# zju-pi/diff-sampler

Measured on NVIDIA H100. Metric: images/sec at fixed NFE, higher is better.
Workload: dtype fp16 operands, fp32 accumulate (split-precision: fp16 hi x hi + two e4m3 correction MMAs per product); 1 GPU; EDM cifar10 U-Net, heun num_steps=10 (NFE=18), batch 512/GPU; net=cifar10, solver=heun, nfe=18, batch_per_gpu=512, global_batch=512, weights=random init (reference constructors, seed 0), init_zero layers de-zeroed, parallelism=dp1, l2=per-forward activation working set (GBs) >> 50 MB L2

## Files before the change

diff-sampler_b200/_cstructs.py:

```python
import ctypes as C

P = C.c_uint64
I32 = C.c_int32
I64 = C.c_int64
F32 = C.c_float

DS_OP_GEMM, DS_OP_GN_STATS, DS_OP_GN_APPLY, DS_OP_SOFTMAX, DS_OP_POSEMB, DS_OP_LINEAR = 1, 2, 3, 4, 5, 6
DS_OP_PREP_INPUT, DS_OP_CHANMEAN, DS_OP_MEMSET, DS_OP_LAYERNORM, DS_OP_GEGLU, DS_OP_GN_FINALIZE, DS_OP_ATTN, DS_OP_EMBED = 7, 8, 9, 10, 11, 12, 13, 14
DS_OP_OPT_PREP, DS_OP_OPT_SOFTMAX, DS_OP_OPT_REDUCE, DS_OP_OPT_KNN = 15, 16, 17, 18
DS_IO_X, DS_IO_D, DS_IO_SIGMA, DS_IO_LABELS, DS_IO_BOTTLENECK, DS_IO_CTX, DS_IO_COUNT = 0, 1, 2, 3, 4, 5, 6
DS_M_X0, DS_M_EPS, DS_M_DIV, DS_M_NONE = 0, 1, 2, 3
DS_F8_SH_A16, DS_F8_SH_LO8, DS_F8_SH_HI8 = 6, 13, 2
DS_OPT_CAP, DS_OPT_P_SHIFT, DS_OPT_BAND_NATS, DS_OPT_TAU, DS_OPT_EPS = 1024, 15, 40, 0.01, 2.0 ** -17
DS_OPT_PLAIN, DS_OPT_RESCORED, DS_OPT_UNREFINED = 0, 1, 2
DS_KNN_MAX, DS_KNN_CAND = 64, 256

SPACE_ABS, SPACE_ARENA, SPACE_WEIGHTS, SPACE_IO = 0, 1, 2, 3


def ref(space, offset):
    return (space << 60) | int(offset)


class GemmDesc(C.Structure):
    _fields_ = [
        ('a_ptr', P), ('a_dims', I64 * 4), ('a_strides', I64 * 3), ('a_box', I32 * 4), ('a_plane_n', I32),
        ('a2_ptr', P), ('a2_c', I64), ('a2_plane_n', I32), ('nkb_aux', I32),
        ('b_ptr', P), ('b_dims', I64 * 3), ('b_strides', I64 * 2), ('b_plane_batch', I32),
        ('BN', I32), ('m_tiles', I32), ('n_tiles', I32), ('num_z', I32), ('nh', I32),
        ('taps', I32), ('cpb', I32), ('npass', I32), ('a_mode', I32), ('conv_H', I32), ('conv_W', I32),
        ('a_c_per_zh', I32), ('a_n_per_zb', I32), ('a_n_per_zh', I32),
        ('b_k0', I32), ('b_k_per_zh', I32), ('b_row_per_zh', I32), ('b_z_per_zb', I32), ('b_z_per_zh', I32),
        ('m_valid', I32), ('n_valid', I32),
        ('out_f32', P), ('out_h16', P), ('o_zb', I64), ('o_zh', I64), ('ldo', I64), ('o_plane', I64),
        ('bias_n', P), ('bias_m', P), ('rowvec', P), ('rowvec_stride', I64), ('rows_per_sample', I32), ('f8', I32),
        ('residual', P), ('ldr', I64), ('scale', F32),
        ('edm_out', I32), ('edm_x', P), ('edm_coef', P), ('edm_coef_stride', I32), ('edm_C', I32), ('edm_D', P),
        ('st_quads', P),
        ('tap_dh', I32 * 9), ('tap_dw', I32 * 9), ('tap_cb', I32 * 9), ('acc_scale', F32), ('st_unit', I32),
    ]


class GnStatsDesc(C.Structure):
    _fields_ = [('src0', P), ('src1', P), ('C0', I32), ('C1', I32), ('HW', I32), ('B', I32), ('groups', I32), ('pad0', I32),
                ('sums', P)]


class GnApplyDesc(C.Structure):
    _fields_ = [('src0', P), ('src1', P), ('C0', I32), ('C1', I32), ('H', I32), ('W', I32), ('B', I32), ('groups', I32),
                ('sums', P), ('gamma', P), ('beta', P), ('eps', F32), ('silu', I32), ('ada', P), ('ada_stride', I64),
                ('resample', I32), ('nplanes', I32), ('out_act', P), ('out_raw', P), ('out_raw_f32', P), ('fmt', I32), ('pad0', I32), ('coef', P)]


class SoftmaxDesc(C.Structure):
    _fields_ = [('S', P), ('P', P), ('rows', I64), ('L', I32), ('nplanes', I32), ('pitch_in', I32), ('pitch_out', I32)]


class PosembDesc(C.Structure):
    _fields_ = [('sigma', P), ('nsig', I32), ('num_channels', I32), ('endpoint', I32), ('swap_sincos', I32),
                ('sigma_data', F32), ('mode', I32), ('coef', P), ('emb', P), ('noise_scale', F32), ('pad0', I32)]


class LinearDesc(C.Structure):
    _fields_ = [('in_', P), ('in_stride', I64), ('W', P), ('b', P), ('add', P), ('add_stride', I64), ('out', P),
                ('n_rows', I32), ('in_f', I32), ('out_f', I32), ('act', I32), ('in_scale', F32), ('pad0', I32)]


class PrepInputDesc(C.Structure):
    _fields_ = [('x', P), ('coef', P), ('coef_stride', I32), ('B', I32), ('C', I32), ('HW', I32), ('nplanes', I32),
                ('x_batch', I32), ('out', P), ('codebook', P), ('idx', P), ('n_embed', I32), ('pad0', I32)]


class ChanmeanDesc(C.Structure):
    _fields_ = [('src', P), ('out', P), ('rows', I64), ('C', I32), ('pad0', I32)]


class LayernormDesc(C.Structure):
    _fields_ = [('src', P), ('gamma', P), ('beta', P), ('out', P), ('rows', I64), ('C', I32), ('nplanes', I32), ('eps', F32), ('fmt', I32)]


class GegluDesc(C.Structure):
    _fields_ = [('src', P), ('out', P), ('rows', I64), ('I', I32), ('nplanes', I32), ('fmt', I32), ('mode', I32)]


class GnFinalizeDesc(C.Structure):
    _fields_ = [('quads0', P), ('quads1', P), ('C0', I32), ('C1', I32), ('slabs_per_sample', I32), ('B', I32), ('groups', I32),
                ('unit0', I32), ('sums', P), ('gamma', P), ('beta', P), ('ada', P), ('ada_stride', I64), ('eps', F32), ('HW', I32), ('coef', P),
                ('unit1', I32), ('pad1', I32)]


class AttnDesc(C.Structure):
    _fields_ = [('q', P), ('k', P), ('vt', P), ('out', P), ('B', I32), ('nh', I32), ('L', I32), ('Lk', I32),
                ('q_pitch', I32), ('q_c0', I32), ('k_pitch', I32), ('k_c0', I32), ('vt_pitch', I32), ('o_pitch', I32),
                ('nplanes', I32), ('scale', F32), ('causal', I32), ('pad0', I32)]


class EmbedDesc(C.Structure):
    _fields_ = [('ids', P), ('tok', P), ('pos', P), ('out', P), ('rows', I64), ('T', I32), ('C', I32), ('vocab', I32), ('pad0', I32)]


class OptPrepDesc(C.Structure):
    _fields_ = [('x', P), ('planes', P), ('xn2', P), ('B', I32), ('D', I32), ('pitch', I32), ('pad0', I32)]


class OptSoftmaxDesc(C.Structure):
    _fields_ = [('part', P), ('hy2', P), ('xn2', P), ('sigma', P), ('x', P), ('y', P), ('P', P), ('status', P), ('ldp', I64), ('ldP', I64),
                ('B', I32), ('N', I32), ('D', I32), ('nslice', I32), ('nsig', I32), ('ymax', F32)]


class OptReduceDesc(C.Structure):
    _fields_ = [('part', P), ('out', P), ('rows', I64), ('cols', I32), ('ld', I32), ('nsplit', I32), ('scale', F32)]


class OptKnnDesc(C.Structure):
    _fields_ = [('part', P), ('hy2', P), ('xn2', P), ('x', P), ('y', P), ('dist', P), ('idx', P), ('ldp', I64),
                ('B', I32), ('N', I32), ('D', I32), ('nslice', I32), ('k', I32), ('ymax', F32)]


class MemsetDesc(C.Structure):
    _fields_ = [('ptr', P), ('bytes', I64)]


class _OpUnion(C.Union):
    _fields_ = [('gemm', GemmDesc), ('gn_stats', GnStatsDesc), ('gn_apply', GnApplyDesc), ('softmax', SoftmaxDesc),
                ('posemb', PosembDesc), ('linear', LinearDesc), ('prep_input', PrepInputDesc), ('chanmean', ChanmeanDesc),
                ('memset', MemsetDesc), ('layernorm', LayernormDesc), ('geglu', GegluDesc), ('gn_finalize', GnFinalizeDesc), ('attn', AttnDesc),
                ('embed', EmbedDesc), ('opt_prep', OptPrepDesc), ('opt_softmax', OptSoftmaxDesc), ('opt_reduce', OptReduceDesc),
                ('opt_knn', OptKnnDesc)]


class PlanOp(C.Structure):
    _fields_ = [('type', I32), ('tag', I32), ('u', _OpUnion)]


SIZEOF_CHECKS = {
    0: PlanOp, DS_OP_GEMM: GemmDesc, DS_OP_GN_STATS: GnStatsDesc, DS_OP_GN_APPLY: GnApplyDesc, DS_OP_SOFTMAX: SoftmaxDesc,
    DS_OP_POSEMB: PosembDesc, DS_OP_LINEAR: LinearDesc, DS_OP_PREP_INPUT: PrepInputDesc, DS_OP_CHANMEAN: ChanmeanDesc,
    DS_OP_MEMSET: MemsetDesc, DS_OP_LAYERNORM: LayernormDesc, DS_OP_GEGLU: GegluDesc, DS_OP_GN_FINALIZE: GnFinalizeDesc, DS_OP_ATTN: AttnDesc,
    DS_OP_EMBED: EmbedDesc, DS_OP_OPT_PREP: OptPrepDesc, DS_OP_OPT_SOFTMAX: OptSoftmaxDesc, DS_OP_OPT_REDUCE: OptReduceDesc,
    DS_OP_OPT_KNN: OptKnnDesc,
}

UNION_FIELD = {
    DS_OP_GEMM: 'gemm', DS_OP_GN_STATS: 'gn_stats', DS_OP_GN_APPLY: 'gn_apply', DS_OP_SOFTMAX: 'softmax', DS_OP_POSEMB: 'posemb',
    DS_OP_LINEAR: 'linear', DS_OP_PREP_INPUT: 'prep_input', DS_OP_CHANMEAN: 'chanmean', DS_OP_MEMSET: 'memset',
    DS_OP_LAYERNORM: 'layernorm', DS_OP_GEGLU: 'geglu', DS_OP_GN_FINALIZE: 'gn_finalize', DS_OP_ATTN: 'attn', DS_OP_EMBED: 'embed',
}
OPT_UNION_FIELD = {DS_OP_OPT_PREP: 'opt_prep', DS_OP_OPT_SOFTMAX: 'opt_softmax', DS_OP_OPT_REDUCE: 'opt_reduce', DS_OP_OPT_KNN: 'opt_knn'}
ALL_UNION_FIELD = {**UNION_FIELD, **OPT_UNION_FIELD}
OP_TYPE_OF = {GemmDesc: DS_OP_GEMM, GnStatsDesc: DS_OP_GN_STATS, GnApplyDesc: DS_OP_GN_APPLY, SoftmaxDesc: DS_OP_SOFTMAX,
              PosembDesc: DS_OP_POSEMB, LinearDesc: DS_OP_LINEAR, PrepInputDesc: DS_OP_PREP_INPUT, ChanmeanDesc: DS_OP_CHANMEAN,
              MemsetDesc: DS_OP_MEMSET, LayernormDesc: DS_OP_LAYERNORM, GegluDesc: DS_OP_GEGLU, GnFinalizeDesc: DS_OP_GN_FINALIZE, AttnDesc: DS_OP_ATTN,
              EmbedDesc: DS_OP_EMBED, OptPrepDesc: DS_OP_OPT_PREP, OptSoftmaxDesc: DS_OP_OPT_SOFTMAX, OptReduceDesc: DS_OP_OPT_REDUCE,
              OptKnnDesc: DS_OP_OPT_KNN}
```

diff-sampler_b200/_lib.py:

```python
import ctypes as C
import os

import torch

from . import _cstructs as S

_HERE = os.path.dirname(os.path.abspath(__file__))
LIB_PATH = os.path.join(_HERE, 'libdiffsampler_b200.so')

EXPORTS = [
    'ds_version', 'ds_last_error', 'ds_weights_create', 'ds_weights_destroy', 'ds_unet_create', 'ds_unet_destroy',
    'ds_unet_forward', 'ds_unet_debug_read', 'ds_unet_last_launch_count', 'ds_solver_update', 'ds_dyn_threshold',
    'ds_op_launch', 'ds_sizeof', 'ds_unet_set_profiling', 'ds_unet_get_profile', 'ds_unet_op_type', 'ds_gits_cost', 'ds_unet_forward_io', 'ds_images_to_uint8', 'ds_solver_update_u8', 'ds_unet_enable_graph', 'ds_amed_predict',
    'ds_gemm_config', 'ds_op_check',
]

_lib = None


class DsError(RuntimeError):
    pass


def load():
    global _lib
    if _lib is not None:
        return _lib
    if not os.path.exists(LIB_PATH):
        raise DsError(f'{LIB_PATH} not found: build it with `python diff-sampler_b200/build.py` '
                      '(there is no CPU fallback for the CUDA path)')
    lib = C.CDLL(LIB_PATH)
    vp, cp, sz = C.c_void_p, C.c_char_p, C.c_size_t
    lib.ds_version.restype = cp
    lib.ds_last_error.restype = cp
    lib.ds_weights_create.argtypes = [vp, sz, C.POINTER(vp)]
    lib.ds_weights_destroy.argtypes = [vp]
    lib.ds_weights_destroy.restype = None
    lib.ds_unet_create.argtypes = [vp, vp, C.c_int, sz, sz, C.POINTER(vp)]
    lib.ds_unet_destroy.argtypes = [vp]
    lib.ds_unet_destroy.restype = None
    lib.ds_unet_forward.argtypes = [vp, vp, vp, vp, vp, vp, vp]
    lib.ds_unet_forward_io.argtypes = [vp, C.POINTER(vp), C.c_int, vp]
    lib.ds_unet_enable_graph.argtypes = [vp, C.POINTER(sz), C.c_int]
    lib.ds_unet_debug_read.argtypes = [vp, sz, vp, sz, vp]
    lib.ds_unet_last_launch_count.argtypes = [vp]
    lib.ds_unet_set_profiling.argtypes = [vp, C.c_int]
    lib.ds_unet_get_profile.argtypes = [vp, C.POINTER(C.c_float), C.c_int]
    lib.ds_unet_op_type.argtypes = [vp, C.c_int]
    lib.ds_solver_update.argtypes = [vp, vp, vp, vp, vp, C.POINTER(vp), C.c_int, vp, C.c_int, C.c_float, vp,
                                     C.POINTER(C.c_float), vp, C.c_int64, C.c_int, vp]
    lib.ds_solver_update_u8.argtypes = [vp, vp, vp, C.c_int, C.c_int, vp, vp, vp, C.POINTER(vp), C.c_int, vp, C.c_int, C.c_float, vp,
                                        C.POINTER(C.c_float), vp, C.c_int64, C.c_int, vp]
    lib.ds_amed_predict.argtypes = [vp, C.POINTER(C.c_int), vp, vp, vp, C.c_float, C.c_float, vp, C.c_int, vp]
    lib.ds_dyn_threshold.argtypes = [vp, vp, C.c_int, C.c_int, C.c_float, C.c_float, vp]
    lib.ds_gits_cost.argtypes = [vp, vp, vp, vp, C.c_int, C.c_int, C.c_int64, vp]
    lib.ds_images_to_uint8.argtypes = [vp, vp, C.c_int, C.c_int, C.c_int, vp]
    lib.ds_op_launch.argtypes = [C.c_int, vp, sz, vp]
    lib.ds_op_check.argtypes = [C.c_int, vp, sz]
    lib.ds_sizeof.argtypes = [C.c_int]
    lib.ds_sizeof.restype = sz
    lib.ds_gemm_config.argtypes = [vp, C.POINTER(C.c_int)]
    for which, cls in S.SIZEOF_CHECKS.items():
        got, want = C.sizeof(cls), lib.ds_sizeof(which)
        if got != want:
            raise DsError(f'struct mirror {cls.__name__}: ctypes size {got} != library size {want}')
    _lib = lib
    return lib


def check(rc, what=''):
    if rc != 0:
        msg = load().ds_last_error().decode()
        raise DsError(f'{what} failed (rc={rc}): {msg}')


def version():
    return load().ds_version().decode()


def op_launch(desc, stream=0):
    lib = load()
    check(lib.ds_op_launch(S.OP_TYPE_OF[type(desc)], C.byref(desc), C.sizeof(desc), C.c_void_p(stream)), type(desc).__name__)


def op_check(desc):
    lib = load()
    if lib.ds_op_check(S.OP_TYPE_OF[type(desc)], C.byref(desc), C.sizeof(desc)) == 0:
        return None
    return lib.ds_last_error().decode()


def gemm_config(desc):
    info = (C.c_int * 2)()
    check(load().ds_gemm_config(C.byref(desc), info), 'ds_gemm_config')
    return dict(stages=info[0], grid=info[1])


class NativePlans:

    def __init__(self, blob, device):
        self.lib = load()
        self.device = device
        self.plans = {}
        self._wh = C.c_void_p()
        with torch.cuda.device(device):
            check(self.lib.ds_weights_create(blob, len(blob), C.byref(self._wh)), 'ds_weights_create')

    def get(self, key, compile_fn, io_bytes=None):
        ent = self.plans.get(key)
        if ent is None:
            pl = compile_fn()
            h = C.c_void_p()
            with torch.cuda.device(self.device):
                check(self.lib.ds_unet_create(self._wh, C.cast(pl.ops_array, C.c_void_p), pl.n_ops, C.sizeof(S.PlanOp), pl.arena_bytes,
                                              C.byref(h)), 'ds_unet_create')
                if io_bytes is not None:
                    check(self.lib.ds_unet_enable_graph(h, (C.c_size_t * S.DS_IO_COUNT)(*io_bytes(pl)), S.DS_IO_COUNT),
                          'ds_unet_enable_graph')
            ent = self.plans[key] = (h, pl)
        return ent

    def run(self, h, io, stream):
        check(self.lib.ds_unet_forward_io(h, (C.c_void_p * S.DS_IO_COUNT)(*io), S.DS_IO_COUNT, C.c_void_p(stream)), 'ds_unet_forward_io')
        return self.lib.ds_unet_last_launch_count(h)

    def debug_read(self, key, name, numel, dtype=torch.float32):
        h, pl = self.plans[key]
        t = torch.empty(numel, dtype=dtype)
        stream = torch.cuda.current_stream(self.device).cuda_stream
        check(self.lib.ds_unet_debug_read(h, pl.arena_offsets[name], t.data_ptr(), t.numel() * t.element_size(), C.c_void_p(stream)),
              'ds_unet_debug_read')
        return t

    def __del__(self):
        try:
            for h, _ in self.plans.values():
                self.lib.ds_unet_destroy(h)
            self.lib.ds_weights_destroy(self._wh)
        except Exception:
            pass
```

diff-sampler_b200/csrc/elementwise.cu:

```cuda
#include "ops.h"
#include "operand.cuh"
#include <cuda_fp16.h>
#include <math.h>

namespace dsb {

__device__ __forceinline__ float silu_f(float v) { return __fdividef(v, 1.0f + __expf(-v)); }

__global__ void gn_stats_kernel(ds_gn_stats_desc d, int pix_per_cta) {
    __shared__ double s_sum[64];
    __shared__ double s_sq[64];
    const int tid = threadIdx.y * blockDim.x + threadIdx.x;
    if (tid < 64) { s_sum[tid] = 0.0; s_sq[tid] = 0.0; }
    __syncthreads();
    const int C = d.C0 + d.C1;
    const int cpg = C / d.groups;
    const int n = blockIdx.y;
    const int ncol4 = C / 4;
    const int p_begin = blockIdx.x * pix_per_cta;
    int p_end = p_begin + pix_per_cta;
    if (p_end > d.HW) p_end = d.HW;
    for (int col = threadIdx.x; col < ncol4; col += blockDim.x) {
        const int c = col * 4;
        const float* base;
        int pitch, cc;
        if (c < d.C0) { base = d.src0; pitch = d.C0; cc = c; }
        else { base = d.src1; pitch = d.C1; cc = c - d.C0; }
        const int gA = c / cpg;
        const int gB = (c + 3) / cpg;
        const int nA = (gA == gB) ? 4 : ((gA + 1) * cpg - c);
        float sA = 0.f, qA = 0.f, sB = 0.f, qB = 0.f;
#pragma unroll 8
        for (int p = p_begin + threadIdx.y; p < p_end; p += blockDim.y) {
            const float4 v = __ldcs(reinterpret_cast<const float4*>(base + ((long long)n * d.HW + p) * pitch + cc));
            const float e[4] = {v.x, v.y, v.z, v.w};
#pragma unroll
            for (int j = 0; j < 4; ++j) {
                if (j < nA) { sA += e[j]; qA += e[j] * e[j]; }
                else { sB += e[j]; qB += e[j] * e[j]; }
            }
        }
        atomicAdd(&s_sum[gA], (double)sA);
        atomicAdd(&s_sq[gA], (double)qA);
        if (gB != gA) {
            atomicAdd(&s_sum[gB], (double)sB);
            atomicAdd(&s_sq[gB], (double)qB);
        }
    }
    __syncthreads();
    if (tid < d.groups) {
        atomicAdd(&d.sums[((long long)n * d.groups + tid) * 2 + 0], s_sum[tid]);
        atomicAdd(&d.sums[((long long)n * d.groups + tid) * 2 + 1], s_sq[tid]);
    }
}

template <class D>
__device__ __forceinline__ float2 gn_group_stats(const D& d, int n, int g, double cnt) {
    const double s = d.sums[((long long)n * d.groups + g) * 2 + 0];
    const double q = d.sums[((long long)n * d.groups + g) * 2 + 1];
    const double mu = s / cnt;
    double var = q / cnt - mu * mu;
    if (var < 0.0) var = 0.0;
    const float rstd = (float)(1.0 / sqrt(var + (double)d.eps));
    return make_float2((float)mu, rstd);
}

template <class D>
__device__ __forceinline__ void gn_channel_coef(const D& d, int n, int C, int c, int j, float rstd, float& a, float& b) {
    float aa = rstd * __ldg(d.gamma + c + j);
    float bb = __ldg(d.beta + c + j);
    if (d.ada) {
        const float sc = d.ada[(long long)n * d.ada_stride + c + j] + 1.0f;
        const float sh = d.ada[(long long)n * d.ada_stride + C + c + j];
        aa *= sc;
        bb = bb * sc + sh;
    }
    a = aa;
    b = bb;
}

__global__ void __launch_bounds__(1024) gn_finalize_kernel(ds_gn_finalize_desc d) {
    extern __shared__ double s_cols[];
    __shared__ float s_mu[64], s_rstd[64];
    const int n = blockIdx.x;
    const int C = d.C0 + d.C1;
    if (d.quads0) {
        const int u0 = d.unit0 == 2 ? 2 : 4, u1 = d.unit1 == 2 ? 2 : 4;
        const int w0 = d.C0 / u0 * 2, w1 = d.C1 / u1 * 2;
        const int cols = w0 + w1;
        int SG = blockDim.x / cols;
        if (SG < 1) SG = 1;
        if (SG > d.slabs_per_sample) SG = d.slabs_per_sample;
        double* part = s_cols + cols;
        for (int idx = threadIdx.x; idx < cols * SG; idx += blockDim.x) {
            const int t = idx % cols, sg = idx / cols;
            const float* src = (t < w0) ? d.quads0 + (long long)n * d.slabs_per_sample * w0 + t
                                        : d.quads1 + (long long)n * d.slabs_per_sample * w1 + (t - w0);
            const int pitch = (t < w0) ? w0 : w1;
            double acc = 0.0;
#pragma unroll 4
            for (int sl = sg; sl < d.slabs_per_sample; sl += SG) acc += (double)__ldg(src + (long long)sl * pitch);
            part[(long long)sg * cols + t] = acc;
        }
        __syncthreads();
        for (int t = threadIdx.x; t < cols; t += blockDim.x) {
            double acc = 0.0;
            for (int sg = 0; sg < SG; ++sg) acc += part[(long long)sg * cols + t];
            s_cols[t] = acc;
        }
        __syncthreads();
        const int cpg = C / d.groups;
        for (int j = threadIdx.x; j < 2 * d.groups; j += blockDim.x) {
            const int g = j >> 1, k = j & 1;
            double acc = 0.0;
            int c = g * cpg;
            const int c_end = c + cpg;
            while (c < c_end) {
                if (c < d.C0) { acc += s_cols[(c / u0) * 2 + k]; c += u0; }
                else { acc += s_cols[w0 + ((c - d.C0) / u1) * 2 + k]; c += u1; }
            }
            d.sums[((long long)n * d.groups + g) * 2 + k] = acc;
        }
        __syncthreads();
    }
    if (!d.coef) return;
    const double cnt = (double)(C / d.groups) * d.HW;
    for (int g = threadIdx.x; g < d.groups; g += blockDim.x) {
        const float2 st = gn_group_stats(d, n, g, cnt);
        s_mu[g] = st.x;
        s_rstd[g] = st.y;
    }
    __syncthreads();
    const int cpg = C / d.groups;
    for (int c = threadIdx.x; c < C; c += blockDim.x) {
        const int g = c / cpg;
        float aa, bb;
        gn_channel_coef(d, n, C, c, 0, s_rstd[g], aa, bb);
        reinterpret_cast<float2*>(d.coef)[(long long)n * C + c] = make_float2(aa, fmaf(-s_mu[g], aa, bb));
    }
}

template <int RESAMPLE>
__global__ void __launch_bounds__(512) gn_apply_kernel(ds_gn_apply_desc d, int pix_per_cta, int nc8, int rows) {
    const int C = d.C0 + d.C1;
    const int n = blockIdx.y;
    const int c8 = threadIdx.x % nc8;
    const int prow = threadIdx.x / nc8;
    const int c = c8 * 8;
    const bool norm = d.sums != nullptr;
    float mean[8], a[8], b[8];
    if (norm) {
        const int cpg = C / d.groups;
// ... 487 lines not shown
    for (int o = 16; o > 0; o >>= 1) sum += __shfl_xor_sync(0xffffffffu, sum, o);
    const float mean = sum / (float)d.C;
    float sq = 0.f;
#pragma unroll
    for (int k = 0; k < MAXV; ++k) {
        const int j = lane + 32 * k;
        if (j < nv) {
            const float a = v[k].x - mean, b = v[k].y - mean, c = v[k].z - mean, e = v[k].w - mean;
            sq += a * a + b * b + c * c + e * e;
        }
    }
#pragma unroll
    for (int o = 16; o > 0; o >>= 1) sq += __shfl_xor_sync(0xffffffffu, sq, o);
    const float rstd = rsqrtf(sq / (float)d.C + d.eps);
#pragma unroll
    for (int k = 0; k < MAXV; ++k) {
        const int j = lane + 32 * k;
        if (j < nv) {
            const float4 g = *reinterpret_cast<const float4*>(d.gamma + 4 * j);
            const float4 b = *reinterpret_cast<const float4*>(d.beta + 4 * j);
            const float y[4] = {(v[k].x - mean) * rstd * g.x + b.x, (v[k].y - mean) * rstd * g.y + b.y,
                                (v[k].z - mean) * rstd * g.z + b.z, (v[k].w - mean) * rstd * g.w + b.w};
            if (FMT == 2) *reinterpret_cast<float4*>(reinterpret_cast<float*>(d.out) + row * d.C + 4 * j) = make_float4(y[0], y[1], y[2], y[3]);
            else store_operand<4>(reinterpret_cast<__half*>(d.out), d.rows * d.C, row * d.C + 4 * j, y, d.nplanes, FMT);
        }
    }
}

__global__ void embed_kernel(ds_embed_desc d) {
    const long long idx = (long long)blockIdx.x * blockDim.x + threadIdx.x;
    const int c4 = d.C / 4;
    if (idx >= d.rows * c4) return;
    const long long row = idx / c4;
    const int j = (int)(idx - row * c4) * 4;
    int id = d.ids[row];
    id = id < 0 ? 0 : (id >= d.vocab ? d.vocab - 1 : id);
    const float4 t = *reinterpret_cast<const float4*>(d.tok + (long long)id * d.C + j);
    const float4 p = *reinterpret_cast<const float4*>(d.pos + (long long)(row % d.T) * d.C + j);
    *reinterpret_cast<float4*>(d.out + row * d.C + j) = make_float4(t.x + p.x, t.y + p.y, t.z + p.z, t.w + p.w);
}

template <int MODE, int FMT>
__global__ void gate_kernel(ds_geglu_desc d) {
    const long long idx = (long long)blockIdx.x * blockDim.x + threadIdx.x;
    const int i4 = d.I / 4;
    if (idx >= d.rows * i4) return;
    float y[4];
    if (MODE == 0) {
        const long long row = idx / i4;
        const int j = (int)(idx - row * i4) * 4;
        const float4 a = *reinterpret_cast<const float4*>(d.src + row * 2 * d.I + j);
        const float4 g = *reinterpret_cast<const float4*>(d.src + row * 2 * d.I + d.I + j);
        const float av[4] = {a.x, a.y, a.z, a.w}, gv[4] = {g.x, g.y, g.z, g.w};
#pragma unroll
        for (int q = 0; q < 4; ++q) y[q] = av[q] * (0.5f * gv[q] * (1.0f + erff(gv[q] * 0.70710678118654752f)));
    } else {
        const float4 a = *reinterpret_cast<const float4*>(d.src + idx * 4);
        const float av[4] = {a.x, a.y, a.z, a.w};
#pragma unroll
        for (int q = 0; q < 4; ++q) y[q] = av[q] / (1.0f + expf(-1.702f * av[q]));
    }
    store_operand<4>(reinterpret_cast<__half*>(d.out), d.rows * d.I, idx * 4, y, d.nplanes, FMT);
}

__global__ void chanmean_kernel(ds_chanmean_desc d) {
    const long long row = (long long)blockIdx.x * (blockDim.x >> 5) + (threadIdx.x >> 5);
    if (row >= d.rows) return;
    const int lane = threadIdx.x & 31;
    float s = 0.f;
    for (int c = lane; c < d.C; c += 32) s += d.src[row * d.C + c];
#pragma unroll
    for (int o = 16; o > 0; o >>= 1) s += __shfl_xor_sync(0xffffffffu, s, o);
    if (lane == 0) d.out[row] = s / (float)d.C;
}

static inline int ok() { return cudaGetLastError() == cudaSuccess ? 0 : -1; }

}

using namespace dsb;

OpCheck dsb::gn_stats_check(const ds_gn_stats_desc& d) {
    const int C = d.C0 + d.C1;
    if (C % 4 || d.groups <= 0 || d.groups > 64 || C % d.groups || (d.C0 % 4)) return {-2, "gn_stats: channels"};
    if (C / d.groups < 2) return {-2, "gn_stats: one-channel groups"};
    return {0, nullptr};
}

extern "C" int ds_gn_stats_launch(const ds_gn_stats_desc* d, cudaStream_t stream) {
    if (const int rc = gn_stats_check(*d).rc) return rc;
    const int C = d->C0 + d->C1;
    const int ncol4 = C / 4;
    int bx = ncol4 < 256 ? ncol4 : 256;
    int by = 256 / bx; if (by < 1) by = 1;
    int pix_per_cta = 8 * by;
    if (pix_per_cta < 64) pix_per_cta = 64;
    const int min_pix = by > 8 ? by : 8;
    while (pix_per_cta > min_pix && (long long)((d->HW + pix_per_cta - 1) / pix_per_cta) * d->B < 132 * 4) pix_per_cta /= 2;
    const int chunks = (d->HW + pix_per_cta - 1) / pix_per_cta;
    gn_stats_kernel<<<dim3(chunks, d->B), dim3(bx, by), 0, stream>>>(*d, pix_per_cta);
    return ok();
}

static size_t gn_finalize_shape(const ds_gn_finalize_desc& d, int* threads) {
    *threads = 256;
    if (!d.quads0) return (size_t)(d.C0 + d.C1 + 2) * sizeof(double);
    const int u0 = d.unit0 == 2 ? 2 : 4, u1 = d.unit1 == 2 ? 2 : 4;
    const int cols = d.C0 / u0 * 2 + d.C1 / u1 * 2;
    *threads = 1024;
    const int sg = cols >= *threads ? 1 : *threads / cols;
    return (size_t)(cols + (size_t)sg * cols + 2) * sizeof(double);
}

OpCheck dsb::gn_finalize_check(const ds_gn_finalize_desc& d) {
    const int C = d.C0 + d.C1;
    if (d.groups <= 0 || d.groups > 64 || C % d.groups) return {-2, "gn_finalize: groups"};
    if (d.quads0) {
        const int u0 = d.unit0 == 2 ? 2 : 4, u1 = d.unit1 == 2 ? 2 : 4;
        const int cpg = C / d.groups;
        if (d.C0 % u0 || d.C1 % u1 || (d.C1 > 0 && !d.quads1)) return {-2, "gn_finalize: source units"};
        const int rem = d.C0 % cpg;
        if (cpg % u0 || rem % u0) return {-2, "gn_finalize: group units"};
        if (d.C1 > 0 && (cpg % u1 || (rem ? (cpg - rem) % u1 : 0))) return {-2, "gn_finalize: group units"};
    }
    if (!d.quads0 && !d.coef) return {-2, "gn_finalize: nothing to do"};
    if (d.coef && (!d.gamma || !d.beta || d.HW <= 0)) return {-2, "gn_finalize: coef inputs"};
    int threads;
    if (gn_finalize_shape(d, &threads) > 48 * 1024) return {-2, "gn_finalize: shared memory"};
    return {0, nullptr};
}

extern "C" int ds_gn_finalize_launch(const ds_gn_finalize_desc* d, cudaStream_t stream) {
    if (const int rc = gn_finalize_check(*d).rc) return rc;
    int threads;
    const size_t smem = gn_finalize_shape(*d, &threads);
    gn_finalize_kernel<<<d->B, threads, smem, stream>>>(*d);
    return ok();
}

OpCheck dsb::gn_apply_check(const ds_gn_apply_desc& d) {
    const int C = d.C0 + d.C1;
    if (C % 8 || (d.C0 % 8)) return {-2, "gn_apply: channels"};
    if (d.fmt != 0 && (d.fmt != 1 || d.resample == 3 || d.nplanes != 2)) return {-2, "gn_apply: fmt"};
    if (d.coef && d.resample != 0) return {-2, "gn_apply: coef with resample"};
    if (d.out_act && !d.sums && !d.coef) return {-2, "gn_apply: statistics"};
    if ((d.resample == 1 || d.resample == 3) && (d.H % 2 || d.W % 2)) return {-2, "gn_apply: resample parity"};
    if (d.pad0 && (d.resample != 3 || d.pad0 < C || d.pad0 % 8 || d.out_raw_f32)) return {-2, "gn_apply: phase pitch"};
    const int nc8 = C / 8;
    if (nc8 > 512) return {-2, "gn_apply: width"};
    if (d.coef && d.resample == 0 && d.sums == nullptr && nc8 > 256) return {-2, "gn_apply: coef width"};
    return {0, nullptr};
}

extern "C" int ds_gn_apply_launch(const ds_gn_apply_desc* d, cudaStream_t stream) {
    if (const int rc = gn_apply_check(*d).rc) return rc;
    const int C = d->C0 + d->C1;
    const int nc8 = C / 8;
    int rows = 256 / nc8;
    if (rows < 1) rows = 1;
    const int threads = nc8 * rows;
    const int Ho = d->resample == 1 ? d->H / 2 : (d->resample == 2 ? d->H * 2 : d->H);
    const int Wo = d->resample == 1 ? d->W / 2 : (d->resample == 2 ? d->W * 2 : d->W);
    const int npix = Ho * Wo;
    int pix_per_cta = rows * 16;
    while (pix_per_cta > rows && (long long)((npix + pix_per_cta - 1) / pix_per_cta) * d->B < 132 * 4) pix_per_cta /= 2;
    const int chunks = (npix + pix_per_cta - 1) / pix_per_cta;
    dim3 grid(chunks, d->B);
    if (d->coef && d->resample == 0 && d->sums == nullptr) {
        static int occ[64][17] = {};
        static int sms[64] = {};
        int dev = 0;
        cudaGetDevice(&dev);
        if (dev < 0 || dev >= 64) dev = 0;
        const int slot = threads / 32;
        if (!sms[dev]) cudaDeviceGetAttribute(&sms[dev], cudaDevAttrMultiProcessorCount, dev);
        if (!occ[dev][slot]) {
            int nb = 0;
            if (cudaOccupancyMaxActiveBlocksPerMultiprocessor(&nb, gn_apply_v3_kernel, threads, 0) != cudaSuccess || nb < 1) nb = 1;
            occ[dev][slot] = nb;
        }
        const int ups = (npix + rows - 1) / rows;
        const long long total_units = (long long)ups * d->B;
        long long g3 = (long long)sms[dev] * occ[dev][slot];
        const long long total_chunks = (long long)((ups + 7) / 8) * d->B;
        if (g3 > total_chunks) g3 = total_chunks;
        if (g3 < 1) g3 = 1;
        gn_apply_v3_kernel<<<(unsigned)g3, threads, 0, stream>>>(*d, nc8, rows, ups, total_units);
        return ok();
    }
    if (d->resample == 1) gn_apply_kernel<1><<<grid, threads, 0, stream>>>(*d, pix_per_cta, nc8, rows);
    else if (d->resample == 3 && d->pad0 && d->pad0 != C) gn_apply_kernel<4><<<grid, threads, 0, stream>>>(*d, pix_per_cta, nc8, rows);
    else if (d->resample == 3) gn_apply_kernel<3><<<grid, threads, 0, stream>>>(*d, pix_per_cta, nc8, rows);
    else if (d->resample == 2) gn_apply_kernel<2><<<grid, threads, 0, stream>>>(*d, pix_per_cta, nc8, rows);
    else gn_apply_v2_kernel<<<grid, threads, 0, stream>>>(*d, pix_per_cta, nc8, rows);
    return ok();
}

OpCheck dsb::embed_check(const ds_embed_desc& d) {
    if (d.C % 4 || d.rows <= 0 || d.T <= 0 || d.vocab <= 0) return {-2, "embed: shape"};
    return {0, nullptr};
}

extern "C" int ds_embed_launch(const ds_embed_desc* d, cudaStream_t stream) {
    if (const int rc = embed_check(*d).rc) return rc;
    const long long total = d->rows * (d->C / 4);
    embed_kernel<<<(unsigned)((total + 255) / 256), 256, 0, stream>>>(*d);
    return ok();
}

OpCheck dsb::layernorm_check(const ds_layernorm_desc& d) {
    if (d.C % 4 || d.C > 2048) return {-2, "layernorm: C"};
    if (d.fmt == 1 && d.nplanes != 2) return {-2, "layernorm: f8 planes"};
    return {0, nullptr};
}

extern "C" int ds_layernorm_launch(const ds_layernorm_desc* d, cudaStream_t stream) {
    if (const int rc = layernorm_check(*d).rc) return rc;
    const int wpb = 8;
    const unsigned blocks = (unsigned)((d->rows + wpb - 1) / wpb);
    if (d->fmt == 1) {
        layernorm_kernel<1><<<blocks, wpb * 32, 0, stream>>>(*d);
    } else if (d->fmt == 2) {
        layernorm_kernel<2><<<blocks, wpb * 32, 0, stream>>>(*d);
    } else {
        layernorm_kernel<0><<<blocks, wpb * 32, 0, stream>>>(*d);
    }
    return ok();
}

OpCheck dsb::geglu_check(const ds_geglu_desc& d) {
    if (d.I % 4) return {-2, "geglu: I"};
    if (d.mode == 1 && d.fmt != 0) return {-2, "geglu: quick-GELU fmt"};
    if (d.mode != 1 && d.fmt == 1 && d.nplanes != 2) return {-2, "geglu: f8 planes"};
    return {0, nullptr};
}

extern "C" int ds_geglu_launch(const ds_geglu_desc* d, cudaStream_t stream) {
    if (const int rc = geglu_check(*d).rc) return rc;
    const unsigned blocks = (unsigned)((d->rows * (d->I / 4) + 255) / 256);
    if (d->mode == 1) {
        gate_kernel<1, 0><<<blocks, 256, 0, stream>>>(*d);
    } else if (d->fmt == 1) {
        gate_kernel<0, 1><<<blocks, 256, 0, stream>>>(*d);
    } else {
        gate_kernel<0, 0><<<blocks, 256, 0, stream>>>(*d);
    }
    return ok();
}

extern "C" int ds_softmax_launch(const ds_softmax_desc* d, cudaStream_t stream) {
    const bool dense = (d->pitch_in == 0 || d->pitch_in == d->L) && (d->pitch_out == 0 || d->pitch_out == d->L) && (d->L % 4 == 0);
    if (dense && d->L <= 1024) {
        const unsigned blocks = (unsigned)((d->rows + 7) / 8);
        if (d->L <= 256) softmax_reg_kernel<2, false><<<blocks, 256, 0, stream>>>(*d);
        else softmax_reg_kernel<8, false><<<blocks, 256, 0, stream>>>(*d);
        return ok();
    }
    if (dense && d->L <= 8192) {
        if (d->L <= 4096) softmax_reg_kernel<4, true><<<(unsigned)d->rows, 256, 0, stream>>>(*d);
        else softmax_reg_kernel<8, true><<<(unsigned)d->rows, 256, 0, stream>>>(*d);
        return ok();
    }
    const int wpb = 8;
    const long long blocks = (d->rows + wpb - 1) / wpb;
    softmax_kernel<<<(unsigned)blocks, wpb * 32, 0, stream>>>(*d);
    return ok();
}

extern "C" int ds_posemb_launch(const ds_posemb_desc* d, cudaStream_t stream) {
    posemb_kernel<<<d->nsig, 128, 0, stream>>>(*d);
    return ok();
}

OpCheck dsb::linear_check(const ds_linear_desc& d) {
    if (d.in_f > 2048) return {-2, "linear: in_f"};
    return {0, nullptr};
}

extern "C" int ds_linear_launch(const ds_linear_desc* d, cudaStream_t stream) {
    if (const int rc = linear_check(*d).rc) return rc;
    const int wpb = 4;
    const int bx = (d->out_f + wpb - 1) / wpb;
    int by = d->n_rows < 16 ? d->n_rows : 16;
    if (by < 1) by = 1;
    if (d->in_f <= 256) linear_kernel<256><<<dim3(bx, by), wpb * 32, 0, stream>>>(*d);
    else if (d->in_f <= 512) linear_kernel<512><<<dim3(bx, by), wpb * 32, 0, stream>>>(*d);
    else if (d->in_f <= 1024) linear_kernel<1024><<<dim3(bx, by), wpb * 32, 0, stream>>>(*d);
    else linear_kernel<2048><<<dim3(bx, by), wpb * 32, 0, stream>>>(*d);
    return ok();
}

OpCheck dsb::prep_input_check(const ds_prep_input_desc& d) {
    if (d.C > 64) return {-2, "prep_input: C"};
    if (d.codebook && (d.C > 8 || d.n_embed < 1)) return {-2, "prep_input: codebook"};
    return {0, nullptr};
}

extern "C" int ds_prep_input_launch(const ds_prep_input_desc* d, cudaStream_t stream) {
    if (const int rc = prep_input_check(*d).rc) return rc;
    if (d->codebook) {
        const unsigned blocks = (unsigned)(((long long)d->B * d->HW + 255) / 256);
        if (d->C <= 4) vq_prep_input_kernel<4><<<blocks, 256, 0, stream>>>(*d);
        else vq_prep_input_kernel<8><<<blocks, 256, 0, stream>>>(*d);
        return ok();
    }
    const long long total = (long long)d->B * d->HW * 8;
    prep_input_kernel<<<(unsigned)((total + 255) / 256), 256, 0, stream>>>(*d);
    return ok();
}

extern "C" int ds_chanmean_launch(const ds_chanmean_desc* d, cudaStream_t stream) {
    const int wpb = 8;
    chanmean_kernel<<<(unsigned)((d->rows + wpb - 1) / wpb), wpb * 32, 0, stream>>>(*d);
    return ok();
}
```

diff-sampler_b200/csrc/engine.cu:

```cuda
#include "../../include/diffsampler_b200.h"
#include "ops.h"
#include "ptx.cuh"
#include <cuda_fp16.h>
#include <nvtx3/nvToolsExt.h>
#include <stdio.h>
#include <stdlib.h>
#include <string.h>
#include <string>
#include <vector>

namespace dsb {
struct GemmKernelParams;
int gemm_build(const ds_gemm_desc* d, GemmKernelParams* kp);
int gemm_run(const GemmKernelParams* kp, cudaStream_t stream);
size_t gemm_params_size();
void gemm_patch_edm(GemmKernelParams* kp, const float* x, float* D);
struct AttnKernelParams;
int attn_build(const ds_attn_desc* d, AttnKernelParams* kp);
int attn_run(const AttnKernelParams* kp, cudaStream_t stream);
size_t attn_params_size();
}

static thread_local std::string g_err;

struct NvtxRange {
    explicit NvtxRange(const char* name) { nvtxRangePushA(name); }
    ~NvtxRange() { nvtxRangePop(); }
};
static int fail(int code, const std::string& msg) {
    g_err = msg;
    return code;
}

struct ds_weights {
    void* dev = nullptr;
    size_t bytes = 0;
};

struct IoFix {
    int op;
    size_t field_off;
    int slot;
};

struct ds_unet {
    const ds_weights* w = nullptr;
    void* arena = nullptr;
    size_t arena_bytes = 0;
    std::vector<ds_plan_op> ops;
    std::vector<std::vector<unsigned char>> gemm_params;
    std::vector<IoFix> fixes;
    int last_launches = 0;
    bool profiling = false;
    std::vector<cudaEvent_t> ev0, ev1;
    std::vector<char> ev_used;
    bool graph_on = false;
    void* stage[DS_IO_COUNT] = {nullptr, nullptr, nullptr, nullptr, nullptr, nullptr};
    size_t stage_bytes[DS_IO_COUNT] = {0, 0, 0, 0, 0, 0};
    cudaGraphExec_t gexec[2] = {nullptr, nullptr};
    int gnodes[2] = {0, 0};
    int warm_runs = 0;
    cudaStream_t cap_stream = nullptr;
};

template <class F>
static void visit_ptrs(ds_plan_op& op, F f) {
#define P(field) f((void**)(void*)(&(field)))
    switch (op.type) {
        case DS_OP_GEMM: {
            ds_gemm_desc& g = op.u.gemm;
            P(g.a_ptr); P(g.a2_ptr); P(g.b_ptr); P(g.out_f32); P(g.out_h16); P(g.bias_n); P(g.bias_m); P(g.rowvec);
            P(g.residual); P(g.edm_x); P(g.edm_coef); P(g.edm_D); P(g.st_quads);
            break;
        }
        case DS_OP_GN_STATS: { auto& d = op.u.gn_stats; P(d.src0); P(d.src1); P(d.sums); break; }
        case DS_OP_GN_APPLY: {
            auto& d = op.u.gn_apply;
            P(d.src0); P(d.src1); P(d.sums); P(d.gamma); P(d.beta); P(d.ada); P(d.out_act); P(d.out_raw); P(d.out_raw_f32); P(d.coef);
            break;
        }
        case DS_OP_SOFTMAX: { auto& d = op.u.softmax; P(d.S); P(d.P); break; }
        case DS_OP_POSEMB: { auto& d = op.u.posemb; P(d.sigma); P(d.coef); P(d.emb); break; }
        case DS_OP_LINEAR: { auto& d = op.u.linear; P(d.in); P(d.W); P(d.b); P(d.add); P(d.out); break; }
        case DS_OP_PREP_INPUT: { auto& d = op.u.prep_input; P(d.x); P(d.coef); P(d.out); P(d.codebook); P(d.idx); break; }
        case DS_OP_CHANMEAN: { auto& d = op.u.chanmean; P(d.src); P(d.out); break; }
        case DS_OP_MEMSET: { auto& d = op.u.memset; P(d.ptr); break; }
        case DS_OP_LAYERNORM: { auto& d = op.u.layernorm; P(d.src); P(d.gamma); P(d.beta); P(d.out); break; }
        case DS_OP_GEGLU: { auto& d = op.u.geglu; P(d.src); P(d.out); break; }
        case DS_OP_GN_FINALIZE: { auto& d = op.u.gn_finalize; P(d.quads0); P(d.quads1); P(d.sums); P(d.gamma); P(d.beta); P(d.ada); P(d.coef); break; }
        case DS_OP_ATTN: { auto& d = op.u.attn; P(d.q); P(d.k); P(d.vt); P(d.out); break; }
        case DS_OP_EMBED: { auto& d = op.u.embed; P(d.ids); P(d.tok); P(d.pos); P(d.out); break; }
        case DS_OP_OPT_PREP: { auto& d = op.u.opt_prep; P(d.x); P(d.planes); P(d.xn2); break; }
        case DS_OP_OPT_SOFTMAX: { auto& d = op.u.opt_softmax; P(d.part); P(d.hy2); P(d.xn2); P(d.sigma); P(d.x); P(d.y); P(d.P); P(d.status); break; }
        case DS_OP_OPT_REDUCE: { auto& d = op.u.opt_reduce; P(d.part); P(d.out); break; }
        case DS_OP_OPT_KNN: { auto& d = op.u.opt_knn; P(d.part); P(d.hy2); P(d.xn2); P(d.x); P(d.y); P(d.dist); P(d.idx); break; }
        default: break;
    }
#undef P
}

static dsb::OpCheck check_op(const ds_plan_op& op) {
    switch (op.type) {
        case DS_OP_GEMM: return dsb::gemm_check(op.u.gemm);
        case DS_OP_GN_STATS: return dsb::gn_stats_check(op.u.gn_stats);
        case DS_OP_GN_APPLY: return dsb::gn_apply_check(op.u.gn_apply);
        case DS_OP_LINEAR: return dsb::linear_check(op.u.linear);
        case DS_OP_PREP_INPUT: return dsb::prep_input_check(op.u.prep_input);
        case DS_OP_LAYERNORM: return dsb::layernorm_check(op.u.layernorm);
        case DS_OP_GEGLU: return dsb::geglu_check(op.u.geglu);
        case DS_OP_GN_FINALIZE: return dsb::gn_finalize_check(op.u.gn_finalize);
        case DS_OP_ATTN: return dsb::attn_check(op.u.attn);
        case DS_OP_EMBED: return dsb::embed_check(op.u.embed);
        case DS_OP_OPT_PREP: return dsb::opt_prep_check(op.u.opt_prep);
        case DS_OP_OPT_SOFTMAX: return dsb::opt_softmax_check(op.u.opt_softmax);
        case DS_OP_OPT_REDUCE: return dsb::opt_reduce_check(op.u.opt_reduce);
        case DS_OP_OPT_KNN: return dsb::opt_knn_check(op.u.opt_knn);
        case DS_OP_SOFTMAX: case DS_OP_POSEMB: case DS_OP_CHANMEAN: case DS_OP_MEMSET: return {0, nullptr};
        default: return {-100, "unknown op type"};
    }
}

static int launch_op(const ds_plan_op& op, const unsigned char* gemm_kp, cudaStream_t s) {
    switch (op.type) {
        case DS_OP_GEMM:
            if (gemm_kp) return dsb::gemm_run(reinterpret_cast<const dsb::GemmKernelParams*>(gemm_kp), s);
            return ds_gemm_launch(&op.u.gemm, s);
        case DS_OP_GN_STATS: return ds_gn_stats_launch(&op.u.gn_stats, s);
        case DS_OP_GN_APPLY: return ds_gn_apply_launch(&op.u.gn_apply, s);
        case DS_OP_SOFTMAX: return ds_softmax_launch(&op.u.softmax, s);
        case DS_OP_POSEMB: return ds_posemb_launch(&op.u.posemb, s);
        case DS_OP_LINEAR: return ds_linear_launch(&op.u.linear, s);
        case DS_OP_PREP_INPUT: return ds_prep_input_launch(&op.u.prep_input, s);
        case DS_OP_CHANMEAN: return ds_chanmean_launch(&op.u.chanmean, s);
        case DS_OP_LAYERNORM: return ds_layernorm_launch(&op.u.layernorm, s);
        case DS_OP_GEGLU: return ds_geglu_launch(&op.u.geglu, s);
        case DS_OP_GN_FINALIZE: return ds_gn_finalize_launch(&op.u.gn_finalize, s);
        case DS_OP_EMBED: return ds_embed_launch(&op.u.embed, s);
        case DS_OP_OPT_PREP: return ds_opt_prep_launch(&op.u.opt_prep, s);
        case DS_OP_OPT_SOFTMAX: return ds_opt_softmax_launch(&op.u.opt_softmax, s);
        case DS_OP_OPT_REDUCE: return ds_opt_reduce_launch(&op.u.opt_reduce, s);
        case DS_OP_OPT_KNN: return ds_opt_knn_launch(&op.u.opt_knn, s);
        case DS_OP_ATTN:
            if (gemm_kp) return dsb::attn_run(reinterpret_cast<const dsb::AttnKernelParams*>(gemm_kp), s);
            return ds_attn_launch(&op.u.attn, s);
        case DS_OP_MEMSET:
            return cudaMemsetAsync(op.u.memset.ptr, 0, (size_t)op.u.memset.bytes, s) == cudaSuccess ? 0 : -1;
        default: return -100;
    }
}

extern "C" {

const char* ds_version(void) { return "diffsampler_b200 0.1 (sm_90a, wgmma/TMA)"; }
const char* ds_last_error(void) { return g_err.c_str(); }

int ds_weights_create(const void* host_blob, size_t bytes, ds_weights** out) {
    if (!host_blob || !out) return fail(-1, "ds_weights_create: null argument");
    ds_weights* w = new ds_weights();
    if (cudaMalloc(&w->dev, bytes ? bytes : 16) != cudaSuccess) {
        delete w;
        return fail(-2, std::string("ds_weights_create: cudaMalloc failed: ") + cudaGetErrorString(cudaGetLastError()));
    }
    if (cudaMemcpy(w->dev, host_blob, bytes, cudaMemcpyHostToDevice) != cudaSuccess) {
        cudaFree(w->dev);
        delete w;
        return fail(-3, "ds_weights_create: cudaMemcpy failed");
    }
    w->bytes = bytes;
    *out = w;
    return 0;
}

void ds_weights_destroy(ds_weights* w) {
    if (!w) return;
    cudaFree(w->dev);
    delete w;
}

int ds_unet_create(const ds_weights* w, const void* plan_ops, int n_ops, size_t op_size, size_t arena_bytes, ds_unet** out) {
    if (!w || !plan_ops || !out) return fail(-1, "ds_unet_create: null argument");
    if (op_size != sizeof(ds_plan_op)) {
        char buf[128];
        snprintf(buf, sizeof buf, "ds_unet_create: ds_plan_op size mismatch (caller %zu, library %zu)", op_size, sizeof(ds_plan_op));
        return fail(-4, buf);
    }
    for (int i = 0; i < n_ops; ++i) {
        const ds_plan_op& op = reinterpret_cast<const ds_plan_op*>(plan_ops)[i];
        const dsb::OpCheck c = check_op(op);
        if (c.rc) {
            char buf[160];
            snprintf(buf, sizeof buf, "ds_unet_create: op %d (type %d tag %d) refused (rc %d): %s", i, op.type, op.tag, c.rc, c.rule);
            return fail(-6, buf);
        }
    }
    ds_unet* u = new ds_unet();
    u->w = w;
    u->arena_bytes = arena_bytes;
    if (cudaMalloc(&u->arena, arena_bytes ? arena_bytes : 16) != cudaSuccess) {
        delete u;
        return fail(-2, std::string("ds_unet_create: cudaMalloc(arena) failed: ") + cudaGetErrorString(cudaGetLastError()));
    }
    cudaMemset(u->arena, 0, arena_bytes);
    u->ops.assign(reinterpret_cast<const ds_plan_op*>(plan_ops), reinterpret_cast<const ds_plan_op*>(plan_ops) + n_ops);
    u->gemm_params.resize(n_ops);
    int bad = 0;
    for (int i = 0; i < n_ops; ++i) {
        ds_plan_op& op = u->ops[i];
        visit_ptrs(op, [&](void** field) {
            const uint64_t ref = reinterpret_cast<uint64_t>(*field);
            const uint64_t space = ref >> 60;
            const uint64_t off = ref & ((1ull << 60) - 1);
            if (space == 0) return;
            if (space == 1) {
                if (off >= arena_bytes) bad = i + 1;
                *field = static_cast<char*>(u->arena) + off;
            } else if (space == 2) {
                if (off >= w->bytes) bad = i + 1;
                *field = static_cast<char*>(w->dev) + off;
            } else if (space == 3) {
                IoFix fx;
                fx.op = i;
                fx.field_off = reinterpret_cast<char*>(field) - reinterpret_cast<char*>(&op);
                fx.slot = (int)off;
                u->fixes.push_back(fx);
                *field = nullptr;
            } else {
                bad = i + 1;
            }
        });
    }
    if (bad) {
        char buf[96];
        snprintf(buf, sizeof buf, "ds_unet_create: bad pointer reference in op %d", bad - 1);
        ds_unet_destroy(u);
        return fail(-5, buf);
    }
    for (int i = 0; i < n_ops; ++i) {
        const int type = u->ops[i].type;
        if (type != DS_OP_GEMM && type != DS_OP_ATTN) continue;
        u->gemm_params[i].resize((type == DS_OP_GEMM ? dsb::gemm_params_size() : dsb::attn_params_size()) + 64);
        unsigned char* p = u->gemm_params[i].data();
        unsigned char* al = reinterpret_cast<unsigned char*>((reinterpret_cast<uintptr_t>(p) + 63) & ~uintptr_t(63));
        int rc = type == DS_OP_GEMM ? dsb::gemm_build(&u->ops[i].u.gemm, reinterpret_cast<dsb::GemmKernelParams*>(al))
                                    : dsb::attn_build(&u->ops[i].u.attn, reinterpret_cast<dsb::AttnKernelParams*>(al));
        if (rc) {
            char buf[96];
            snprintf(buf, sizeof buf, "ds_unet_create: %s failed (rc %d) for op %d tag %d", type == DS_OP_GEMM ? "gemm_build" : "attn_build", rc, i,
                     u->ops[i].tag);
            ds_unet_destroy(u);
            return fail(-6, buf);
        }
    }
    *out = u;
    return 0;
}

void ds_unet_destroy(ds_unet* u) {
    if (!u) return;
    for (auto e : u->ev0) cudaEventDestroy(e);
    for (auto e : u->ev1) cudaEventDestroy(e);
    for (int v = 0; v < 2; ++v) if (u->gexec[v]) cudaGraphExecDestroy(u->gexec[v]);
    for (int k = 0; k < DS_IO_COUNT; ++k) if (u->stage[k]) cudaFree(u->stage[k]);
    if (u->cap_stream) cudaStreamDestroy(u->cap_stream);
    cudaFree(u->arena);
    delete u;
}

int ds_unet_forward_io(ds_unet* u, const void* const* io_in, int n_io, void* stream);

int ds_unet_forward(ds_unet* u, const float* x, const float* sigma, const float* labels, float* out_D, float* out_bottleneck,
                    void* stream) {
    const void* io[DS_IO_COUNT] = {x, out_D, sigma, labels, out_bottleneck, nullptr};
    return ds_unet_forward_io(u, io, DS_IO_COUNT, stream);
}

static int run_ops(ds_unet* u, const void* const* io, cudaStream_t s, bool profiling) {
    for (const IoFix& fx : u->fixes) {
        if (fx.slot < 0 || fx.slot >= DS_IO_COUNT) return fail(-7, "ds_unet_forward: bad io slot");
        void** field = reinterpret_cast<void**>(reinterpret_cast<char*>(&u->ops[fx.op]) + fx.field_off);
        *field = const_cast<void*>(io[fx.slot]);
    }
    int launches = 0;
    for (size_t i = 0; i < u->ops.size(); ++i) {
        ds_plan_op& op = u->ops[i];
        const unsigned char* kp = nullptr;
        if (op.type == DS_OP_GEMM || op.type == DS_OP_ATTN) {
            unsigned char* p = u->gemm_params[i].data();
            unsigned char* al = reinterpret_cast<unsigned char*>((reinterpret_cast<uintptr_t>(p) + 63) & ~uintptr_t(63));
            if (op.type == DS_OP_GEMM && op.u.gemm.edm_out)
                dsb::gemm_patch_edm(reinterpret_cast<dsb::GemmKernelParams*>(al), op.u.gemm.edm_x, op.u.gemm.edm_D);
            kp = al;
        }
        if (op.type == DS_OP_CHANMEAN && op.u.chanmean.out == nullptr) continue;
        if (profiling) { cudaEventRecord(u->ev0[i], s); u->ev_used[i] = 1; }
        int rc = launch_op(op, kp, s);
        if (profiling) cudaEventRecord(u->ev1[i], s);
        if (rc) {
            char buf[160];
            snprintf(buf, sizeof buf, "ds_unet_forward: op %zu (type %d tag %d) failed rc=%d cuda=%s", i, op.type, op.tag, rc,
                     cudaGetErrorString(cudaGetLastError()));
            return fail(-8, buf);
        }
        ++launches;
    }
    return launches;
}

static int build_graph(ds_unet* u, int variant, const void* const* staged_io) {
    if (!u->cap_stream && cudaStreamCreateWithFlags(&u->cap_stream, cudaStreamNonBlocking) != cudaSuccess)
        return fail(-20, "ds_unet_forward: cannot create the capture stream");
    if (cudaStreamBeginCapture(u->cap_stream, cudaStreamCaptureModeThreadLocal) != cudaSuccess)
        return fail(-21, std::string("ds_unet_forward: cudaStreamBeginCapture failed: ") + cudaGetErrorString(cudaGetLastError()));
    const int n = run_ops(u, staged_io, u->cap_stream, false);
    cudaGraph_t g = nullptr;
    const cudaError_t e = cudaStreamEndCapture(u->cap_stream, &g);
    if (n < 0 || e != cudaSuccess || !g) {
        if (g) cudaGraphDestroy(g);
        if (n < 0) return n;
        return fail(-22, std::string("ds_unet_forward: stream capture failed: ") + cudaGetErrorString(e));
    }
    cudaGraphExec_t ex = nullptr;
    const cudaError_t ei = cudaGraphInstantiate(&ex, g, 0);
    cudaGraphDestroy(g);
    if (ei != cudaSuccess) return fail(-23, std::string("ds_unet_forward: cudaGraphInstantiate failed: ") + cudaGetErrorString(ei));
    u->gexec[variant] = ex;
    u->gnodes[variant] = n;
    return 0;
}

int ds_unet_forward_io(ds_unet* u, const void* const* io_in, int n_io, void* stream) {
    if (!u) return fail(-1, "ds_unet_forward: null handle");
    NvtxRange nvtx_range("ds_unet_forward");
    cudaStream_t s = static_cast<cudaStream_t>(stream);
    const void* io[DS_IO_COUNT] = {nullptr, nullptr, nullptr, nullptr, nullptr, nullptr};
    for (int k = 0; k < n_io && k < DS_IO_COUNT; ++k) io[k] = io_in[k];
    if (!u->graph_on || u->profiling) {
        const int n = run_ops(u, io, s, u->profiling);
        if (n < 0) return n;
        u->last_launches = n;
        return 0;
    }
    static const bool is_input[DS_IO_COUNT] = {true, false, true, true, false, true};
    const void* staged[DS_IO_COUNT];
    for (int k = 0; k < DS_IO_COUNT; ++k) {
        staged[k] = (io[k] && u->stage[k]) ? u->stage[k] : nullptr;
        if (io[k] && !u->stage[k]) return fail(-24, "ds_unet_forward: io slot used without a staging buffer (ds_unet_enable_graph sizes)");
        if (io[k] && is_input[k] &&
            cudaMemcpyAsync(u->stage[k], io[k], u->stage_bytes[k], cudaMemcpyDeviceToDevice, s) != cudaSuccess)
            return fail(-25, "ds_unet_forward: staging copy failed");
    }
    const int variant = io[DS_IO_BOTTLENECK] ? 1 : 0;
    int launches = 0;
    if (!u->gexec[variant]) {
        if (u->warm_runs < 1) {
            launches = run_ops(u, staged, s, false);
            if (launches < 0) return launches;
            ++u->warm_runs;
        } else {
            const int rc = build_graph(u, variant, staged);
            if (rc) return rc;
        }
    }
    if (u->gexec[variant]) {
        if (cudaGraphLaunch(u->gexec[variant], s) != cudaSuccess)
            return fail(-26, std::string("ds_unet_forward: cudaGraphLaunch failed: ") + cudaGetErrorString(cudaGetLastError()));
        launches = u->gnodes[variant];
    }
    for (int k = 0; k < DS_IO_COUNT; ++k)
        if (io[k] && !is_input[k] &&
            cudaMemcpyAsync(const_cast<void*>(io[k]), u->stage[k], u->stage_bytes[k], cudaMemcpyDeviceToDevice, s) != cudaSuccess)
            return fail(-25, "ds_unet_forward: staging copy failed");
    u->last_launches = launches;
    return 0;
}

int ds_unet_enable_graph(ds_unet* u, const size_t* io_bytes, int n_io) {
    if (!u || !io_bytes) return fail(-1, "ds_unet_enable_graph: null argument");
    if (u->graph_on) return 0;
    for (int k = 0; k < n_io && k < DS_IO_COUNT; ++k) {
        if (!io_bytes[k]) continue;
        if (cudaMalloc(&u->stage[k], io_bytes[k]) != cudaSuccess)
            return fail(-2, std::string("ds_unet_enable_graph: cudaMalloc failed: ") + cudaGetErrorString(cudaGetLastError()));
        u->stage_bytes[k] = io_bytes[k];
    }
    u->graph_on = true;
    return 0;
}

int ds_unet_debug_read(ds_unet* u, size_t arena_offset, void* host_dst, size_t bytes, void* stream) {
    if (!u || arena_offset + bytes > u->arena_bytes) return fail(-1, "ds_unet_debug_read: out of range");
    cudaStream_t s = static_cast<cudaStream_t>(stream);
    if (cudaStreamSynchronize(s) != cudaSuccess) return fail(-2, std::string("ds_unet_debug_read: ") + cudaGetErrorString(cudaGetLastError()));
    if (cudaMemcpy(host_dst, static_cast<char*>(u->arena) + arena_offset, bytes, cudaMemcpyDeviceToHost) != cudaSuccess)
        return fail(-3, "ds_unet_debug_read: memcpy failed");
    return 0;
}

int ds_unet_last_launch_count(const ds_unet* u) { return u ? u->last_launches : 0; }

int ds_unet_set_profiling(ds_unet* u, int enable) {
    if (!u) return fail(-1, "ds_unet_set_profiling: null handle");
    if (enable && u->ev0.empty()) {
        u->ev0.resize(u->ops.size());
        u->ev1.resize(u->ops.size());
        u->ev_used.assign(u->ops.size(), 0);
        for (size_t i = 0; i < u->ops.size(); ++i) {
            cudaEventCreate(&u->ev0[i]);
            cudaEventCreate(&u->ev1[i]);
        }
    }
    u->profiling = enable != 0;
    return 0;
}

int ds_unet_get_profile(ds_unet* u, float* ms_per_op, int n) {
    if (!u || u->ev0.empty()) return fail(-1, "ds_unet_get_profile: profiling was not enabled");
    if (cudaDeviceSynchronize() != cudaSuccess) return fail(-2, "ds_unet_get_profile: sync failed");
    for (int i = 0; i < n && i < (int)u->ops.size(); ++i) {
        float ms = 0.f;
        if (u->ev_used[i]) cudaEventElapsedTime(&ms, u->ev0[i], u->ev1[i]);
        ms_per_op[i] = ms;
    }
    return (int)u->ops.size();
}

int ds_unet_op_type(const ds_unet* u, int i) { return (u && i >= 0 && i < (int)u->ops.size()) ? u->ops[i].type : -1; }

static int solver_update_impl(float* out_x, float* out_m, unsigned char* out_u8, int u8_C, int u8_HW, const float* xb, const float* xs,
                              const float* D, const float* const* hist, int nhist, const float* thr, int mode, float t, const float* t_dev,
                              const float* coef6, const float* coef_dev, int64_t n_per_sample, int B, void* stream) {
    if (!xb || nhist < 0 || nhist > 4) return fail(-1, "ds_solver_update: bad argument");
    NvtxRange nvtx_range("ds_solver_update");
    ds_update_desc d;
    memset(&d, 0, sizeof d);
    d.out_x = out_x; d.out_m = out_m; d.xb = xb; d.xs = xs; d.D = D;
    for (int k = 0; k < nhist; ++k) d.h[k] = hist[k];
    d.thr = thr; d.coef_dev = coef_dev; d.t_dev = t_dev;
    if (coef6) for (int k = 0; k < 6; ++k) d.coef[k] = coef6[k];
    d.t = t; d.mode = mode; d.nhist = nhist; d.B = B; d.n_per_sample = n_per_sample;
    d.out_u8 = out_u8; d.u8_C = u8_C; d.u8_HW = u8_HW;
    if ((mode == DS_M_X0 || mode == DS_M_EPS) && !D) return fail(-1, "ds_solver_update: mode needs D");
    int rc = ds_update_launch(&d, static_cast<cudaStream_t>(stream));
    if (rc) return fail(rc, std::string("ds_solver_update: launch failed: ") + cudaGetErrorString(cudaGetLastError()));
    return 0;
}

int ds_solver_update(float* out_x, float* out_m, const float* xb, const float* xs, const float* D, const float* const* hist, int nhist,
                     const float* thr, int mode, float t, const float* t_dev, const float* coef6, const float* coef_dev,
                     int64_t n_per_sample, int B, void* stream) {
    return solver_update_impl(out_x, out_m, nullptr, 0, 0, xb, xs, D, hist, nhist, thr, mode, t, t_dev, coef6, coef_dev, n_per_sample, B, stream);
}

int ds_solver_update_u8(float* out_x, float* out_m, unsigned char* out_u8, int C, int HW, const float* xb, const float* xs, const float* D,
                        const float* const* hist, int nhist, const float* thr, int mode, float t, const float* t_dev, const float* coef6,
                        const float* coef_dev, int64_t n_per_sample, int B, void* stream) {
    if (!out_u8 || C <= 0 || HW <= 0) return fail(-1, "ds_solver_update_u8: bad image geometry");
    return solver_update_impl(out_x, out_m, out_u8, C, HW, xb, xs, D, hist, nhist, thr, mode, t, t_dev, coef6, coef_dev, n_per_sample, B, stream);
}

int ds_dyn_threshold(const float* x0, float* thr, int B, int row_len, float q, float floor_val, void* stream) {
    ds_threshold_desc d;
    d.x0 = x0; d.thr = thr; d.B = B; d.row_len = row_len; d.q = q; d.floor_val = floor_val;
    int rc = ds_threshold_launch(&d, static_cast<cudaStream_t>(stream));
    if (rc) return fail(rc, std::string("ds_dyn_threshold: launch failed: ") + cudaGetErrorString(cudaGetLastError()));
    return 0;
}

size_t ds_sizeof(int which) {
    switch (which) {
        case 0: return sizeof(ds_plan_op);
        case DS_OP_GEMM: return sizeof(ds_gemm_desc);
        case DS_OP_GN_STATS: return sizeof(ds_gn_stats_desc);
        case DS_OP_GN_APPLY: return sizeof(ds_gn_apply_desc);
        case DS_OP_SOFTMAX: return sizeof(ds_softmax_desc);
        case DS_OP_POSEMB: return sizeof(ds_posemb_desc);
        case DS_OP_LINEAR: return sizeof(ds_linear_desc);
        case DS_OP_PREP_INPUT: return sizeof(ds_prep_input_desc);
        case DS_OP_CHANMEAN: return sizeof(ds_chanmean_desc);
        case DS_OP_MEMSET: return sizeof(ds_memset_desc);
        case DS_OP_LAYERNORM: return sizeof(ds_layernorm_desc);
        case DS_OP_GEGLU: return sizeof(ds_geglu_desc);
        case DS_OP_GN_FINALIZE: return sizeof(ds_gn_finalize_desc);
        case DS_OP_ATTN: return sizeof(ds_attn_desc);
        case DS_OP_EMBED: return sizeof(ds_embed_desc);
        case DS_OP_OPT_PREP: return sizeof(ds_opt_prep_desc);
        case DS_OP_OPT_SOFTMAX: return sizeof(ds_opt_softmax_desc);
        case DS_OP_OPT_REDUCE: return sizeof(ds_opt_reduce_desc);
        case DS_OP_OPT_KNN: return sizeof(ds_opt_knn_desc);
        default: return 0;
    }
}

int ds_gits_cost(const float* traj, const float* eps, const float* t_steps, double* out, int N, int B, int64_t n_per_sample, void* stream) {
    ds_gits_cost_desc d;
    d.traj = traj; d.eps = eps; d.t = t_steps; d.out = out; d.N = N; d.B = B; d.n = n_per_sample;
    int rc = ds_gits_cost_launch(&d, static_cast<cudaStream_t>(stream));
    if (rc) return fail(rc, std::string("ds_gits_cost: launch failed: ") + cudaGetErrorString(cudaGetLastError()));
    return 0;
}

int ds_amed_predict(const float* weights, const int* dims6, const float* bottleneck, const float* t_cur, const float* t_next,
                    float scale_dir, float scale_time, float* out4, int B, void* stream) {
    if (!weights || !dims6 || !t_cur || !t_next || !out4) return fail(-1, "ds_amed_predict: null argument");
    NvtxRange nvtx_range("ds_amed_predict");
    int rc = ds_amed_predict_launch(weights, dims6, bottleneck, t_cur, t_next, scale_dir, scale_time, out4, B, static_cast<cudaStream_t>(stream));
    if (rc) return fail(rc, std::string("ds_amed_predict: launch failed: ") + cudaGetErrorString(cudaGetLastError()));
    return 0;
}

int ds_images_to_uint8(const float* images, unsigned char* out, int B, int C, int HW, void* stream) {
    if (!images || !out) return fail(-1, "ds_images_to_uint8: null argument");
    int rc = ds_to_uint8_launch(images, out, B, C, HW, static_cast<cudaStream_t>(stream));
    if (rc) return fail(rc, std::string("ds_images_to_uint8: launch failed: ") + cudaGetErrorString(cudaGetLastError()));
    return 0;
}

int ds_op_launch(int op_type, const void* desc, size_t desc_size, void* stream) {
    ds_plan_op op;
    memset(&op, 0, sizeof op);
    op.type = op_type;
    if (desc_size > sizeof(op.u)) return fail(-1, "ds_op_launch: descriptor too large");
    memcpy(&op.u, desc, desc_size);
    int rc = launch_op(op, nullptr, static_cast<cudaStream_t>(stream));
    if (rc) {
        char buf[128];
        snprintf(buf, sizeof buf, "ds_op_launch: op type %d failed rc=%d cuda=%s", op_type, rc, cudaGetErrorString(cudaGetLastError()));
        return fail(rc, buf);
    }
    return 0;
}

int ds_op_check(int op_type, const void* desc, size_t desc_size) {
    ds_plan_op op;
    memset(&op, 0, sizeof op);
    op.type = op_type;
    if (desc_size > sizeof(op.u)) return fail(-1, "ds_op_check: descriptor too large");
    memcpy(&op.u, desc, desc_size);
    const dsb::OpCheck c = check_op(op);
// ... 5 lines not shown
```

diff-sampler_b200/csrc/gemm_tc.cu:

```cuda
#include "ops.h"
#include "ptx.cuh"
#include <cuda_fp16.h>
#include <stdio.h>
#include <stdlib.h>
#include <string.h>

namespace dsb {

static constexpr int kMaxStages = 8;
static constexpr int kATileBytes = 128 * 128;
static constexpr int kThreads = 384;
static constexpr int kStgPitch = 64;
static constexpr int kStgBytes = 2 * 64 * kStgPitch * 4;
static constexpr int kSmemLimit = 227 * 1024;

struct alignas(64) GemmKernelParams {
    CUtensorMap tmA, tmA2, tmB;
    CUtensorMap tmA8, tmA2_8, tmB8;
    int f8, cpb8, nkb8_main, nkb8_aux, a8_plane_n;
    float acc_scale;
    int BN, m_tiles, n_tiles, num_z, nh;
    int taps, cpb, nkb_main, nkb_aux, npass;
    int a_mode, conv_H, conv_W, a_bn_dummy;
    int a_plane_n, a2_plane_n, b_plane_batch;
    int a_c_per_zh, a_n_per_zb, a_n_per_zh;
    int b_k0, b_k_per_zh, b_row_per_zh, b_z_per_zb, b_z_per_zh;
    int m_valid, n_valid;
    int num_stages;
    float* out_f32;
    __half* out_h16;
    long long o_zb, o_zh, ldo, o_plane;
    const float* bias_n;
    const float* bias_m;
    const float* rowvec;
    long long rowvec_stride;
    int rows_per_sample;
    const float* residual;
    long long ldr;
    float scale;
    int edm_out;
    const float* edm_x;
    const float* edm_coef;
    int edm_coef_stride;
    int edm_C;
    float* edm_D;
    float* st_quads;
    int st_unit;
    int tap_dh[9], tap_dw[9], tap_cb[9];
    int f8_last_steps;
};

struct SmemCtl {
    uint64_t full[kMaxStages];
    uint64_t empty[kMaxStages];
};

template <int N>
__device__ __forceinline__ void warp_sum_levels(float* v, int lane, int off) {
    if constexpr (N >= 1) {
        const bool up = (lane & off) != 0;
#pragma unroll
        for (int i = 0; i < N; ++i) {
            const float send = up ? v[i] : v[i + N];
            const float keep = up ? v[i + N] : v[i];
            v[i] = keep + __shfl_xor_sync(0xffffffffu, send, off);
        }
        warp_sum_levels<N / 2>(v, lane, off >> 1);
    } else {
        for (; off >= 1; off >>= 1) v[0] += __shfl_xor_sync(0xffffffffu, v[0], off);
    }
}
template <int NV>
__device__ __forceinline__ void warp_sum_multi(float (&v)[NV], int lane) {
    static_assert(NV == 32 || NV == 16 || NV == 8, "NV");
    warp_sum_levels<NV / 2>(v, lane, 16);
}

template <int W>
__device__ __forceinline__ void epilogue_chunk(const GemmKernelParams& p, const float* v, long long grow_in_z, int col0, bool row_ok,
                                               int zb, int zh) {
    const bool warp_rows_ok = __all_sync(0xffffffffu, row_ok);
    if (!row_ok) return;
    float r[W];
#pragma unroll
    for (int j = 0; j < W; ++j) r[j] = v[j] * p.acc_scale;
    const bool full = (col0 + W <= p.n_valid);
    if (p.bias_n) {
        if (full) {
#pragma unroll
            for (int j = 0; j < W; j += 4) {
                const float4 t = __ldg(reinterpret_cast<const float4*>(p.bias_n + col0 + j));
                r[j] += t.x; r[j + 1] += t.y; r[j + 2] += t.z; r[j + 3] += t.w;
            }
        } else {
#pragma unroll
            for (int j = 0; j < W; ++j)
                if (col0 + j < p.n_valid) r[j] += __ldg(p.bias_n + col0 + j);
        }
    }
    if (p.bias_m) {
        const float bm = __ldg(p.bias_m + grow_in_z);
#pragma unroll
        for (int j = 0; j < W; ++j) r[j] += bm;
    }
    if (p.rowvec) {
        const long long s = (p.rowvec_stride == 0) ? 0 : (grow_in_z / p.rows_per_sample) * p.rowvec_stride;
        const float* rv = p.rowvec + s + col0;
        if (full) {
#pragma unroll
            for (int j = 0; j < W; j += 4) {
                const float4 t = __ldg(reinterpret_cast<const float4*>(rv + j));
                r[j] += t.x; r[j + 1] += t.y; r[j + 2] += t.z; r[j + 3] += t.w;
            }
        } else {
#pragma unroll
            for (int j = 0; j < W; ++j)
                if (col0 + j < p.n_valid) r[j] += __ldg(rv + j);
        }
    }
    if (p.residual) {
        const float* rs = p.residual + grow_in_z * p.ldr + col0;
        if (full) {
#pragma unroll
            for (int j = 0; j < W; j += 4) {
                const float4 t = *reinterpret_cast<const float4*>(rs + j);
                r[j] += t.x; r[j + 1] += t.y; r[j + 2] += t.z; r[j + 3] += t.w;
            }
        } else {
#pragma unroll
            for (int j = 0; j < W; ++j)
                if (col0 + j < p.n_valid) r[j] += rs[j];
        }
    }
#pragma unroll
    for (int j = 0; j < W; ++j) r[j] *= p.scale;

    if (p.st_quads) {
        const int lane = threadIdx.x & 31;
        if (p.st_unit == 2) {
            float q[W];
#pragma unroll
            for (int j = 0; j < W; j += 2) {
                q[j] = r[j] + r[j + 1];
                q[j + 1] = fmaf(r[j], r[j], r[j + 1] * r[j + 1]);
            }
            warp_sum_multi<W>(q, lane);
            constexpr int kShift = (W == 32) ? 0 : 1;
            const int vi = lane >> kShift;
            if ((lane & ((1 << kShift) - 1)) == 0 && col0 + 2 * (vi >> 1) < p.n_valid)
                p.st_quads[(grow_in_z >> 5) * (long long)p.n_valid + col0 + vi] = q[0];
        } else {
            float q[W / 2];
#pragma unroll
            for (int j = 0; j < W; j += 4) {
                q[j / 2] = (r[j] + r[j + 1]) + (r[j + 2] + r[j + 3]);
                q[j / 2 + 1] = fmaf(r[j], r[j], r[j + 1] * r[j + 1]) + fmaf(r[j + 2], r[j + 2], r[j + 3] * r[j + 3]);
            }
            warp_sum_multi<W / 2>(q, lane);
            constexpr int kShift = (W == 32) ? 1 : 2;
            const int vi = lane >> kShift;
            if ((lane & ((1 << kShift) - 1)) == 0 && col0 + 4 * (vi >> 1) < p.n_valid)
                p.st_quads[((grow_in_z >> 5) * (long long)(p.n_valid >> 2)) * 2 + (col0 >> 1) + vi] = q[0];
        }
    }

    if (p.edm_out) {
        const int HW = p.rows_per_sample;
        const long long n = grow_in_z / HW;
        const long long hw = grow_in_z % HW;
        if (p.edm_out == 2) {
#pragma unroll
            for (int j = 0; j < W; ++j) {
                const int c = col0 + j;
                if (c < p.edm_C) p.edm_D[(n * p.edm_C + c) * HW + hw] = r[j];
            }
            return;
        }
        const float cskip = __ldg(p.edm_coef + n * p.edm_coef_stride + 0);
        const float cout = __ldg(p.edm_coef + n * p.edm_coef_stride + 1);
#pragma unroll
        for (int j = 0; j < W; ++j) {
            const int c = col0 + j;
            if (c < p.edm_C) {
                const long long idx = (n * p.edm_C + c) * HW + hw;
                p.edm_D[idx] = cskip * __ldg(p.edm_x + idx) + cout * r[j];
            }
        }
        return;
    }

    const long long obase = (long long)zb * p.o_zb + (long long)zh * p.o_zh + grow_in_z * p.ldo + col0;
    const int odd = threadIdx.x & 1;
    if (p.out_f32) {
        float* o = p.out_f32 + obase;
        if (full && warp_rows_ok) {
            float* oe = o - odd * p.ldo + odd * 4;
#pragma unroll
            for (int j = 0; j < W; j += 8) {
                float x[4];
#pragma unroll
                for (int k = 0; k < 4; ++k) x[k] = __shfl_xor_sync(0xffffffffu, odd ? r[j + k] : r[j + 4 + k], 1);
                const float4 s1 = odd ? make_float4(x[0], x[1], x[2], x[3]) : make_float4(r[j], r[j + 1], r[j + 2], r[j + 3]);
// ... 270 lines not shown
                    ah0 = 0;
                    an0 = tc.zb * p.a_n_per_zb + tc.zh * p.a_n_per_zh;
                }
                const int a_c_off = tc.zh * p.a_c_per_zh;
                const int b_k_off = p.b_k0 + tc.zh * p.b_k_per_zh;
                const int b_row = tc.nt * BN + tc.zh * p.b_row_per_zh;
                const int b_z = tc.zb * p.b_z_per_zb + tc.zh * p.b_z_per_zh;
                producer_tile(p, smem, ctl, ring, block_bytes, aw0, ah0, an0, a_c_off, b_k_off, b_row, b_z);
            }
        }
    } else {
        asm volatile("setmaxnreg.inc.sync.aligned.u32 232;");
        const int cw = wg - 1;
        float* my_stg = stg + cw * 64 * kStgPitch;
        RingPos ring{0, 0u};
        for (int tile = blockIdx.x; tile < total_tiles; tile += gridDim.x) {
            const TileCoord tc = tile_coord(p, tile);
            float acc[BN / 2];
            mma_tile<BN>(p, smem, ctl, ring, block_bytes, cw, acc);
            epilogue_tile<BN>(p, my_stg, cw, tc, acc);
        }
    }
}

typedef CUresult (*EncodeTiledFn)(CUtensorMap*, CUtensorMapDataType, cuuint32_t, void*, const cuuint64_t*, const cuuint64_t*,
                                  const cuuint32_t*, const cuuint32_t*, CUtensorMapInterleave, CUtensorMapSwizzle,
                                  CUtensorMapL2promotion, CUtensorMapFloatOOBfill);

static EncodeTiledFn get_encode_fn() {
    static EncodeTiledFn fn = nullptr;
    if (!fn) {
        void* p = nullptr;
        cudaDriverEntryPointQueryResult q;
        if (cudaGetDriverEntryPoint("cuTensorMapEncodeTiled", &p, cudaEnableDefault, &q) != cudaSuccess || q != cudaDriverEntryPointSuccess)
            return nullptr;
        fn = reinterpret_cast<EncodeTiledFn>(p);
    }
    return fn;
}

static int encode_map_typed(CUtensorMap* m, const void* ptr, int rank, const int64_t* dims, const int64_t* strides_bytes,
                            const int32_t* box, bool bytes8) {
    EncodeTiledFn fn = get_encode_fn();
    if (!fn) return -1;
    cuuint64_t gd[5];
    cuuint64_t gs[4];
    cuuint32_t bx[5];
    cuuint32_t es[5];
    for (int i = 0; i < rank; ++i) { gd[i] = (cuuint64_t)dims[i]; bx[i] = (cuuint32_t)box[i]; es[i] = 1; }
    for (int i = 0; i + 1 < rank; ++i) gs[i] = (cuuint64_t)strides_bytes[i];
    CUresult r = fn(m, bytes8 ? CU_TENSOR_MAP_DATA_TYPE_UINT8 : CU_TENSOR_MAP_DATA_TYPE_FLOAT16, (cuuint32_t)rank, const_cast<void*>(ptr), gd, gs, bx, es, CU_TENSOR_MAP_INTERLEAVE_NONE,
                    CU_TENSOR_MAP_SWIZZLE_128B, CU_TENSOR_MAP_L2_PROMOTION_L2_256B, CU_TENSOR_MAP_FLOAT_OOB_FILL_NONE);
    if (r != CUDA_SUCCESS) {
        fprintf(stderr, "[dsb] cuTensorMapEncodeTiled failed: %d (rank %d dims %lld %lld %lld %lld box %d %d %d %d)\n", (int)r, rank,
                (long long)dims[0], (long long)dims[1], (long long)dims[2], rank > 3 ? (long long)dims[3] : 0LL, box[0], box[1], box[2],
                rank > 3 ? box[3] : 0);
        return -2;
    }
    return 0;
}

int encode_map(CUtensorMap* m, const void* ptr, int rank, const int64_t* dims, const int64_t* strides_bytes, const int32_t* box) {
    return encode_map_typed(m, ptr, rank, dims, strides_bytes, box, false);
}

OpCheck gemm_check(const ds_gemm_desc& d) {
    if (d.BN < 16 || d.BN > 256 || (d.BN % 16) != 0) return {-10, "gemm: BN"};
    if (d.a_box[0] != 64 || d.a_box[1] * d.a_box[2] * d.a_box[3] != 128) return {-11, "gemm: a_box"};
    if (d.npass != 1 && d.npass != 3) return {-12, "gemm: npass"};
    for (int i = 0; i < 4; ++i) if (d.a_dims[i] > (int64_t(1) << 32)) return {-1, "gemm: A tensor map"};
    for (int i = 0; i < 3; ++i) if (d.a_strides[i] % 16 || d.a_strides[i] >= (int64_t(1) << 40)) return {-1, "gemm: A tensor map"};
    if (d.st_unit != 0 && d.st_unit != 2 && d.st_unit != 4) return {-14, "gemm: st_unit"};
    if (d.f8 & 1) {
        if (d.a_mode != 0 || d.num_z != 1 || d.npass != 3 || d.a_plane_n <= 0) return {-16, "gemm: f8"};
        for (int t = 0; t < 9; ++t) if (d.tap_cb[t]) return {-16, "gemm: f8 with tap_cb"};
        if (d.a_dims[0] % 64 || d.a2_c % 64) return {-16, "gemm: f8 channel remainder"};
    }
    if (d.taps != 1 && d.taps != 9) return {-15, "gemm: taps"};
    if (d.a_mode == 0 && d.conv_W > 128 && (d.conv_W % 128 != 0 || d.a_box[1] != 128)) return {-13, "gemm: row segment"};
    if (d.st_quads && (d.num_z != 1 || d.m_valid % 32 != 0 || d.n_valid % (d.st_unit == 2 ? 2 : 4) != 0 || d.edm_out != 0))
        return {-14, "gemm: st_quads"};
    return {0, nullptr};
}

int gemm_build(const ds_gemm_desc* d, GemmKernelParams* kp) {
    memset(kp, 0, sizeof(*kp));
    if (const int rc = gemm_check(*d).rc) return rc;
    if (encode_map(&kp->tmA, d->a_ptr, 4, d->a_dims, d->a_strides, d->a_box)) return -1;
    if (d->a2_c > 0) {
        int64_t dims2[4] = {d->a2_c, d->a_dims[1], d->a_dims[2], d->a_dims[3]};
        int64_t st2[3] = {d->a2_c * 2, d->a2_c * 2 * d->a_dims[1], d->a2_c * 2 * d->a_dims[1] * d->a_dims[2]};
        if (encode_map(&kp->tmA2, d->a2_ptr, 4, dims2, st2, d->a_box)) return -2;
    }
    int32_t bbox[3] = {64, d->BN, 1};
    if (encode_map(&kp->tmB, d->b_ptr, 3, d->b_dims, d->b_strides, bbox)) return -3;

    kp->BN = d->BN; kp->m_tiles = d->m_tiles; kp->n_tiles = d->n_tiles; kp->num_z = d->num_z; kp->nh = d->nh > 0 ? d->nh : 1;
    kp->taps = d->taps; kp->cpb = d->cpb; kp->nkb_main = d->taps * d->cpb; kp->nkb_aux = d->a2_c > 0 ? (int)((d->a2_c + 63) / 64) : 0;
    kp->npass = d->npass; kp->a_mode = d->a_mode; kp->conv_H = d->conv_H; kp->conv_W = d->conv_W;
    kp->a_plane_n = d->a_plane_n; kp->a2_plane_n = d->a2_plane_n; kp->b_plane_batch = d->b_plane_batch;
    kp->a_c_per_zh = d->a_c_per_zh; kp->a_n_per_zb = d->a_n_per_zb; kp->a_n_per_zh = d->a_n_per_zh;
    kp->b_k0 = d->b_k0; kp->b_k_per_zh = d->b_k_per_zh; kp->b_row_per_zh = d->b_row_per_zh;
    kp->b_z_per_zb = d->b_z_per_zb; kp->b_z_per_zh = d->b_z_per_zh;
    kp->m_valid = d->m_valid; kp->n_valid = d->n_valid;
    kp->out_f32 = d->out_f32; kp->out_h16 = reinterpret_cast<__half*>(d->out_h16);
    kp->o_zb = d->o_zb; kp->o_zh = d->o_zh; kp->ldo = d->ldo; kp->o_plane = d->o_plane;
    kp->bias_n = d->bias_n; kp->bias_m = d->bias_m; kp->rowvec = d->rowvec; kp->rowvec_stride = d->rowvec_stride;
    kp->rows_per_sample = d->rows_per_sample > 0 ? d->rows_per_sample : 1;
    kp->residual = d->residual; kp->ldr = d->ldr; kp->scale = d->scale;
    kp->edm_out = d->edm_out; kp->edm_x = d->edm_x; kp->edm_coef = d->edm_coef; kp->edm_coef_stride = d->edm_coef_stride;
    kp->edm_C = d->edm_C; kp->edm_D = d->edm_D;
    kp->st_quads = d->st_quads;
    kp->st_unit = d->st_unit == 2 ? 2 : 4;
    kp->acc_scale = d->acc_scale == 0.f ? 1.f : d->acc_scale;
    if (d->f8 & 1) {
        const int64_t C = d->a_dims[0], Wd = d->a_dims[1], Hd = d->a_dims[2], Bn = d->a_plane_n;
        const int32_t box8[4] = {128, d->a_box[1], d->a_box[2], d->a_box[3]};
        const int64_t dims8[4] = {C, Wd, Hd, 2 * Bn};
        const int64_t st8[3] = {C, Wd * C, Hd * Wd * C};
        const char* a8 = static_cast<const char*>(d->a_ptr) + Bn * Hd * Wd * C * 2;
        if (encode_map_typed(&kp->tmA8, a8, 4, dims8, st8, box8, true)) return -17;
        kp->f8 = 1;
        kp->f8_last_steps = (d->cpb & 1) ? 2 : 4;
        kp->a8_plane_n = (int)Bn;
        kp->cpb8 = (d->cpb + 1) / 2;
        kp->nkb8_main = d->taps * kp->cpb8;
        kp->nkb8_aux = 0;
        if (d->a2_c > 0) {
            const int64_t C2 = d->a2_c;
            const int64_t dims28[4] = {C2, Wd, Hd, 2 * Bn};
            const int64_t st28[3] = {C2, Wd * C2, Hd * Wd * C2};
            const char* a28 = static_cast<const char*>(d->a2_ptr) + Bn * Hd * Wd * C2 * 2;
            if (encode_map_typed(&kp->tmA2_8, a28, 4, dims28, st28, box8, true)) return -18;
            kp->nkb8_aux = (int)((C2 + 127) / 128);
        }
        const int64_t ktot8 = (int64_t)(kp->nkb8_main + kp->nkb8_aux) * 128;
        const int64_t rows = d->b_dims[1];
        const int64_t bd8[3] = {ktot8, rows, 2};
        const int64_t bs8[2] = {ktot8, rows * ktot8};
        const int32_t bbox8[3] = {128, d->BN, 1};
        const char* b8 = static_cast<const char*>(d->b_ptr) + rows * d->b_dims[0] * 2;
        if (encode_map_typed(&kp->tmB8, b8, 3, bd8, bs8, bbox8, true)) return -19;
    }
    for (int t = 0; t < 9; ++t) { kp->tap_dh[t] = d->tap_dh[t]; kp->tap_dw[t] = d->tap_dw[t]; kp->tap_cb[t] = d->tap_cb[t]; }
    const int stage_bytes = kATileBytes + d->BN * 128;
    int ns = (kSmemLimit - 1024 - kStgBytes - (int)sizeof(SmemCtl)) / stage_bytes;
    if (ns > kMaxStages) ns = kMaxStages;
    kp->num_stages = ns;
    return 0;
}

size_t gemm_params_size() { return sizeof(GemmKernelParams); }
void gemm_patch_edm(GemmKernelParams* kp, const float* x, float* D) { kp->edm_x = x; kp->edm_D = D; }

static int g_num_sms[64] = {};
static bool g_attr_set[64][17] = {};

template <int BN>
static int gemm_launch(const GemmKernelParams* kp, cudaStream_t stream, int slot) {
    if (!g_attr_set[slot][BN / 16]) {
        if (cudaFuncSetAttribute(gemm_tc_kernel<BN>, cudaFuncAttributeMaxDynamicSharedMemorySize, kSmemLimit) != cudaSuccess) return -20;
        g_attr_set[slot][BN / 16] = true;
    }
    const size_t smem = (size_t)kp->num_stages * (kATileBytes + BN * 128) + kStgBytes + sizeof(SmemCtl) + 1024;
    const int tiles = kp->num_z * kp->m_tiles * kp->n_tiles;
    const int grid = tiles < g_num_sms[slot] ? tiles : g_num_sms[slot];
    if (grid <= 0) return 0;
    gemm_tc_kernel<BN><<<grid, kThreads, smem, stream>>>(*kp);
    return cudaGetLastError() == cudaSuccess ? 0 : -21;
}

int gemm_run(const GemmKernelParams* kp, cudaStream_t stream) {
    int dev = 0;
    cudaGetDevice(&dev);
    const int slot = (dev < 0 || dev >= 64) ? 0 : dev;
    if (!g_num_sms[slot]) cudaDeviceGetAttribute(&g_num_sms[slot], cudaDevAttrMultiProcessorCount, slot);
    switch (kp->BN / 16) {
        case 1: return gemm_launch<16>(kp, stream, slot);
        case 2: return gemm_launch<32>(kp, stream, slot);
        case 3: return gemm_launch<48>(kp, stream, slot);
        case 4: return gemm_launch<64>(kp, stream, slot);
        case 5: return gemm_launch<80>(kp, stream, slot);
        case 6: return gemm_launch<96>(kp, stream, slot);
        case 7: return gemm_launch<112>(kp, stream, slot);
        case 8: return gemm_launch<128>(kp, stream, slot);
        case 9: return gemm_launch<144>(kp, stream, slot);
        case 10: return gemm_launch<160>(kp, stream, slot);
        case 11: return gemm_launch<176>(kp, stream, slot);
        case 12: return gemm_launch<192>(kp, stream, slot);
        case 13: return gemm_launch<208>(kp, stream, slot);
        case 14: return gemm_launch<224>(kp, stream, slot);
        case 15: return gemm_launch<240>(kp, stream, slot);
        case 16: return gemm_launch<256>(kp, stream, slot);
        default: return -10;
    }
}

}

extern "C" int ds_gemm_launch(const ds_gemm_desc* d, cudaStream_t stream) {
    dsb::GemmKernelParams kp;
    int rc = dsb::gemm_build(d, &kp);
    if (rc) return rc;
    return dsb::gemm_run(&kp, stream);
}

extern "C" int ds_gemm_config(const void* desc, int* info) {
    dsb::GemmKernelParams kp;
    int rc = dsb::gemm_build(static_cast<const ds_gemm_desc*>(desc), &kp);
    if (rc) return rc;
    int dev = 0, sms = 0;
    cudaGetDevice(&dev);
    if (cudaDeviceGetAttribute(&sms, cudaDevAttrMultiProcessorCount, dev) != cudaSuccess) return -20;
    const int tiles = kp.num_z * kp.m_tiles * kp.n_tiles;
    info[0] = kp.num_stages;
    info[1] = tiles < sms ? tiles : sms;
    return 0;
}
```

diff-sampler_b200/csrc/ops.h:

```cpp
#pragma once
#include <stdint.h>
#include <cuda_runtime.h>

#ifdef __cplusplus
extern "C" {
#endif

enum { DS_F8_SH_A16 = 6, DS_F8_SH_LO8 = 13, DS_F8_SH_HI8 = 2 };
typedef struct ds_gemm_desc {
    const void* a_ptr;
    int64_t a_dims[4];
    int64_t a_strides[3];
    int32_t a_box[4];
    int32_t a_plane_n;
    const void* a2_ptr;
    int64_t a2_c;
    int32_t a2_plane_n;
    int32_t nkb_aux;
    const void* b_ptr;
    int64_t b_dims[3];
    int64_t b_strides[2];
    int32_t b_plane_batch;
    int32_t BN;
    int32_t m_tiles, n_tiles, num_z, nh;
// ... 210 lines not shown
    const float* t_dev;
    float coef[6];
    float t;
    int32_t mode;
    int32_t nhist;
    int32_t B;
    int64_t n_per_sample;
    unsigned char* out_u8;
    int32_t u8_C, u8_HW;
} ds_update_desc;

typedef struct ds_threshold_desc {
    const float* x0;
    float* thr;
    int32_t B;
    int32_t row_len;
    float q;
    float floor_val;
} ds_threshold_desc;

typedef struct ds_gits_cost_desc {
    const float* traj;
    const float* eps;
    const float* t;
    double* out;
    int32_t N, B;
    int64_t n;
} ds_gits_cost_desc;

int ds_gits_cost_launch(const ds_gits_cost_desc* d, cudaStream_t stream);

typedef struct ds_opt_prep_desc {
    const float* x;
    void* planes;
    double* xn2;
    int32_t B, D;
    int32_t pitch, pad0;
} ds_opt_prep_desc;

enum { DS_OPT_CAP = 1024, DS_OPT_P_SHIFT = 15, DS_OPT_BAND_NATS = 40 };
#define DS_OPT_TAU 0.01f
#define DS_OPT_EPS 7.62939453125e-06
enum { DS_OPT_PLAIN = 0, DS_OPT_RESCORED = 1, DS_OPT_UNREFINED = 2 };
typedef struct ds_opt_softmax_desc {
    float* part;
    const double* hy2;
    const double* xn2;
    const float* sigma;
    const float* x;
    const float* y;
    void* P;
    int32_t* status;
    int64_t ldp, ldP;
    int32_t B, N, D, nslice;
    int32_t nsig;
    float ymax;
} ds_opt_softmax_desc;

typedef struct ds_opt_reduce_desc {
    const float* part;
    float* out;
    int64_t rows;
    int32_t cols, ld;
    int32_t nsplit;
    float scale;
} ds_opt_reduce_desc;

enum { DS_KNN_MAX = 64, DS_KNN_CAND = 256 };
typedef struct ds_opt_knn_desc {
    float* part;
    const double* hy2;
    const double* xn2;
    const float* x;
    const float* y;
    float* dist;
    int32_t* idx;
    int64_t ldp;
    int32_t B, N, D, nslice;
    int32_t k;
    float ymax;
} ds_opt_knn_desc;

int ds_opt_prep_launch(const ds_opt_prep_desc* d, cudaStream_t stream);
int ds_opt_softmax_launch(const ds_opt_softmax_desc* d, cudaStream_t stream);
int ds_opt_reduce_launch(const ds_opt_reduce_desc* d, cudaStream_t stream);
int ds_opt_knn_launch(const ds_opt_knn_desc* d, cudaStream_t stream);
int ds_amed_predict_launch(const float* w, const int* dims6, const float* bott, const float* t_cur, const float* t_next, float scale_dir,
                           float scale_time, float* out, int B, cudaStream_t stream);
int ds_to_uint8_launch(const float* x, unsigned char* out, int B, int Cc, int HW, cudaStream_t stream);
int ds_update_launch(const ds_update_desc* d, cudaStream_t stream);
int ds_threshold_launch(const ds_threshold_desc* d, cudaStream_t stream);
int ds_gn_stats_launch(const ds_gn_stats_desc* d, cudaStream_t stream);
int ds_gn_apply_launch(const ds_gn_apply_desc* d, cudaStream_t stream);
int ds_gn_finalize_launch(const ds_gn_finalize_desc* d, cudaStream_t stream);
int ds_attn_launch(const ds_attn_desc* d, cudaStream_t stream);
int ds_softmax_launch(const ds_softmax_desc* d, cudaStream_t stream);
int ds_posemb_launch(const ds_posemb_desc* d, cudaStream_t stream);
int ds_linear_launch(const ds_linear_desc* d, cudaStream_t stream);
int ds_prep_input_launch(const ds_prep_input_desc* d, cudaStream_t stream);
int ds_chanmean_launch(const ds_chanmean_desc* d, cudaStream_t stream);
int ds_layernorm_launch(const ds_layernorm_desc* d, cudaStream_t stream);
int ds_geglu_launch(const ds_geglu_desc* d, cudaStream_t stream);
int ds_embed_launch(const ds_embed_desc* d, cudaStream_t stream);

enum { DS_OP_GEMM = 1, DS_OP_GN_STATS = 2, DS_OP_GN_APPLY = 3, DS_OP_SOFTMAX = 4, DS_OP_POSEMB = 5, DS_OP_LINEAR = 6,
       DS_OP_PREP_INPUT = 7, DS_OP_CHANMEAN = 8, DS_OP_MEMSET = 9, DS_OP_LAYERNORM = 10, DS_OP_GEGLU = 11,
       DS_OP_GN_FINALIZE = 12, DS_OP_ATTN = 13, DS_OP_EMBED = 14, DS_OP_OPT_PREP = 15, DS_OP_OPT_SOFTMAX = 16,
       DS_OP_OPT_REDUCE = 17, DS_OP_OPT_KNN = 18 };
enum { DS_IO_X = 0, DS_IO_D = 1, DS_IO_SIGMA = 2, DS_IO_LABELS = 3, DS_IO_BOTTLENECK = 4, DS_IO_CTX = 5, DS_IO_COUNT = 6 };

typedef struct ds_memset_desc {
    void* ptr;
    int64_t bytes;
} ds_memset_desc;

typedef struct ds_plan_op {
    int32_t type;
    int32_t tag;
    union {
        ds_gemm_desc gemm;
        ds_gn_stats_desc gn_stats;
        ds_gn_apply_desc gn_apply;
        ds_softmax_desc softmax;
        ds_posemb_desc posemb;
        ds_linear_desc linear;
        ds_prep_input_desc prep_input;
        ds_chanmean_desc chanmean;
        ds_memset_desc memset;
        ds_layernorm_desc layernorm;
        ds_geglu_desc geglu;
        ds_gn_finalize_desc gn_finalize;
        ds_attn_desc attn;
        ds_embed_desc embed;
        ds_opt_prep_desc opt_prep;
        ds_opt_softmax_desc opt_softmax;
        ds_opt_reduce_desc opt_reduce;
        ds_opt_knn_desc opt_knn;
    } u;
} ds_plan_op;

#ifdef __cplusplus
}

namespace dsb {
struct OpCheck {
    int rc;
    const char* rule;
};
OpCheck gemm_check(const ds_gemm_desc& d);
OpCheck attn_check(const ds_attn_desc& d);
OpCheck gn_stats_check(const ds_gn_stats_desc& d);
OpCheck gn_finalize_check(const ds_gn_finalize_desc& d);
OpCheck gn_apply_check(const ds_gn_apply_desc& d);
OpCheck embed_check(const ds_embed_desc& d);
OpCheck layernorm_check(const ds_layernorm_desc& d);
OpCheck geglu_check(const ds_geglu_desc& d);
OpCheck linear_check(const ds_linear_desc& d);
OpCheck prep_input_check(const ds_prep_input_desc& d);
OpCheck opt_prep_check(const ds_opt_prep_desc& d);
OpCheck opt_softmax_check(const ds_opt_softmax_desc& d);
OpCheck opt_reduce_check(const ds_opt_reduce_desc& d);
OpCheck opt_knn_check(const ds_opt_knn_desc& d);
}
#endif
```

diff-sampler_b200/gemm_desc.py:

```python
from . import _cstructs as S

H16 = 2


NUM_SMS = 132


def _tile_cost(bn):
    return 690.0 + bn


def pick_bn(n):
    for bn in (32, 64):
        if n <= bn:
            return bn, 1
    best = None
    for bn in range(256, 63, -16):
        tiles = -(-n // bn)
        key = (tiles * _tile_cost(bn), tiles * bn - n, -bn)
        if best is None or key < best[0]:
            best = (key, bn, tiles)
    return best[1], best[2]


def fill_bn(n, m_tiles, num_z=1):
    bn, tiles = pick_bn(n)
    if m_tiles * tiles * num_z >= 4 * NUM_SMS or bn <= 64:
        return bn, tiles
    best = None
    for cand in range(256, 63, -16):
        nt = -(-n // cand)
        waves = -(-(m_tiles * nt * num_z) // NUM_SMS)
        key = (waves * _tile_cost(cand), nt * cand - n, -cand)
        if best is None or key < best[0]:
            best = (key, cand, nt)
    return best[1], best[2]


def padded_rows(n):
    bn, tiles = pick_bn(n)
    return bn * tiles


def split_planes_rows(n_valid, bn):
    tiles = -(-n_valid // bn)
    return tiles, tiles * bn


def conv_box(H, W):
    if W > 128:
        assert W % 128 == 0, f'unsupported width {W}'
        return 128, 1, 1
    assert 128 % W == 0, f'unsupported width {W}'
    bw = W
    bh = min(H, 128 // W)
    bn = 128 // (bw * bh)
    assert bw * bh * bn == 128
    return bw, bh, bn


def conv_gemm(a_ptr, Bn, H, W, C, w_ptr, Cout, *, taps=9, npass=3, a_planes=2, w_planes=2, a2_ptr=0, C2=0,
              out_f32=0, out_h16=0, o_planes=2, ldo=None, bias=0, rowvec=0, rowvec_stride=0, residual=0, ldr=None, scale=1.0,
              edm=None, nchw_out=None, bn=None, s2d=False, f8=False, acc_scale=1.0):
    assert C % 8 == 0 and C2 % 8 == 0
    cpad, c2pad = -(-C // 64) * 64, -(-C2 // 64) * 64
    if f8:
        assert npass == 3 and not s2d
        a_planes = w_planes = 1
    elif npass == 3:
        assert a_planes == 2 and w_planes == 2
    d = S.GemmDesc()
    bw, bh, bnn = conv_box(H, W)
    BN, n_tiles = (bn, -(-Cout // bn)) if bn else fill_bn(Cout, -(-(Bn * H * W) // 128))
    cout_pad = padded_rows(Cout)
    ktot = taps * cpad + c2pad
    d.a_ptr = a_ptr
    cphys = 4 * cpad if s2d else C
    d.a_dims[:] = [cphys, W, H, a_planes * Bn]
    d.a_strides[:] = [cphys * H16, W * cphys * H16, H * W * cphys * H16]
    d.a_box[:] = [64, bw, bh, bnn]
    d.a_plane_n = Bn
    d.a2_ptr = a2_ptr
    d.a2_c = C2
    d.a2_plane_n = Bn
    d.nkb_aux = c2pad // 64
    d.b_ptr = w_ptr
    d.b_dims[:] = [ktot, cout_pad, w_planes]
    d.b_strides[:] = [ktot * H16, cout_pad * ktot * H16]
    d.b_plane_batch = 1
    d.BN = BN
    d.m_tiles = -(-(Bn * H * W) // 128)
    d.n_tiles = n_tiles
    d.num_z = 1
    d.nh = 1
    d.taps = taps
    d.cpb = cpad // 64
    d.npass = npass
    d.a_mode = 0
    d.conv_H, d.conv_W = H, W
    if taps == 9:
        for t in range(9):
            kh, kw = t // 3, t % 3
            if s2d:
                sh, ph = [(-1, 1), (0, 0), (0, 1)][kh]
                sw, pw = [(-1, 1), (0, 0), (0, 1)][kw]
                d.tap_dh[t], d.tap_dw[t], d.tap_cb[t] = sh, sw, (ph * 2 + pw) * cpad
            else:
                d.tap_dh[t], d.tap_dw[t], d.tap_cb[t] = kh - 1, kw - 1, 0
    d.m_valid = Bn * H * W
    d.n_valid = Cout
    d.out_f32 = out_f32
    d.out_h16 = out_h16
    d.ldo = ldo if ldo is not None else Cout
    d.o_plane = (Bn * H * W * d.ldo) if (out_h16 and o_planes == 2) else 0
    d.bias_n = bias
    d.rowvec = rowvec
    d.rowvec_stride = rowvec_stride
    d.rows_per_sample = H * W
    d.residual = residual
    d.ldr = ldr if ldr is not None else Cout
    d.scale = scale
    d.f8 = 1 if f8 else 0
    d.acc_scale = acc_scale
    if edm is not None:
        d.edm_out = 1
        d.edm_x, d.edm_coef, d.edm_coef_stride, d.edm_C, d.edm_D = edm
    if nchw_out is not None:
        d.edm_out = 2
        d.edm_C, d.edm_D = nchw_out
    return d, dict(BN=BN, n_tiles=n_tiles, cout_pad=cout_pad, ktot=ktot)


def rows_gemm(a_ptr, a_rows, a_pitch, a_batches, b_ptr, b_rows, b_pitch, b_batches, K, *, num_z, nh=1, m_valid, n_valid,
              npass=3, a_planes=2, b_planes=2, a_c_per_zh=0, a_n_per_zb=0, a_n_per_zh=0, b_k0=0, b_k_per_zh=0, b_row_per_zh=0,
              b_z_per_zb=0, b_z_per_zh=0, out_f32=0, out_h16=0, o_zb=0, o_zh=0, ldo=0, o_plane=0, bias_n=0, bias_m=0,
              residual=0, ldr=0, scale=1.0, bn=None, a_k_valid=None, b_k_valid=None):
    assert K % 64 == 0
    d = S.GemmDesc()
    BN, n_tiles = (bn, -(-n_valid // bn)) if bn else fill_bn(n_valid, -(-m_valid // 128), num_z)
    d.a_ptr = a_ptr
    d.a_dims[:] = [a_k_valid or a_pitch, a_rows, 1, a_planes * a_batches]
    d.a_strides[:] = [a_pitch * H16, a_rows * a_pitch * H16, a_rows * a_pitch * H16]
    d.a_box[:] = [64, 128, 1, 1]
    d.a_plane_n = a_batches
    d.b_ptr = b_ptr
    d.b_dims[:] = [b_k_valid or b_pitch, b_rows, b_planes * b_batches]
    d.b_strides[:] = [b_pitch * H16, b_rows * b_pitch * H16]
    d.b_plane_batch = b_batches
    d.BN = BN
    d.m_tiles = -(-m_valid // 128)
    d.n_tiles = n_tiles
    d.num_z = num_z
    d.nh = nh
    d.taps = 1
    d.cpb = K // 64
    d.npass = npass
    d.a_mode = 1
    d.conv_H = d.conv_W = 1
    d.a_c_per_zh, d.a_n_per_zb, d.a_n_per_zh = a_c_per_zh, a_n_per_zb, a_n_per_zh
    d.b_k0, d.b_k_per_zh, d.b_row_per_zh, d.b_z_per_zb, d.b_z_per_zh = b_k0, b_k_per_zh, b_row_per_zh, b_z_per_zb, b_z_per_zh
    d.m_valid, d.n_valid = m_valid, n_valid
    d.out_f32, d.out_h16 = out_f32, out_h16
    d.o_zb, d.o_zh, d.ldo, d.o_plane = o_zb, o_zh, ldo, o_plane
    d.bias_n, d.bias_m = bias_n, bias_m
    d.rows_per_sample = 1
    d.residual, d.ldr = residual, ldr
    d.scale = scale
    return d, dict(BN=BN, n_tiles=n_tiles)


def pack_conv_weight(weight, skip_weight=None, cin_pad=None, bn=None):
    import torch
    cout, cin, kh, kw = weight.shape
    cin_pad = cin_pad or -(-cin // 64) * 64
    w = torch.zeros(cout, kh, kw, cin_pad, dtype=torch.float32)
    w[..., :cin] = weight.detach().float().permute(0, 2, 3, 1)
    w = w.reshape(cout, kh * kw * cin_pad)
    if skip_weight is not None:
        c2 = skip_weight.shape[1]
        c2_pad = -(-c2 // 64) * 64
        sk = torch.zeros(cout, c2_pad, dtype=torch.float32)
        sk[:, :c2] = skip_weight.detach().float().reshape(cout, c2)
        w = torch.cat([w, sk], dim=1)
    BN, n_tiles = (bn, -(-cout // bn)) if bn else pick_bn(cout)
    cout_pad = BN * n_tiles
    wp = torch.zeros(cout_pad, w.shape[1], dtype=torch.float32)
    wp[:cout] = w
    hi = wp.half()
    lo = (wp - hi.float()).half()
    return torch.stack([hi, lo]).contiguous()


def describe(d):
    m, n, z = int(d.m_valid), int(d.n_valid), max(int(d.num_z), 1)
    k_main = int(d.taps) * int(d.cpb) * 64
    k_aux = int(d.a2_c)
    k = k_main + k_aux
    flops = 2.0 * m * n * k * z
    a_bytes = 4 * m * (int(d.cpb) * 64 + k_aux) * z if d.a_mode == 0 else 4 * m * k * z
    w_bytes = 4 * n * k * (z if d.a_mode == 1 else 1)
    out_bytes = m * n * z * ((4 if d.out_f32 else 0) + (4 if d.out_h16 and d.o_plane else (2 if d.out_h16 else 0)))
    if d.edm_out:
        out_bytes = 2 * 4 * m * int(d.edm_C)
    res_bytes = 4 * m * n * z if d.residual else 0
    if d.a_mode == 0:
        label = f"conv{'3x3' if d.taps == 9 else '1x1'} {int(d.cpb) * 64}{'+' + str(k_aux) if k_aux else ''}->{n} @{int(d.conv_H)}x{int(d.conv_W)} x{m // max(int(d.conv_H) * int(d.conv_W), 1)}"
    else:
        label = f'gemm {m}x{n}x{k} z{z}'
    return dict(label=label + (' f8' if d.f8 & 1 else ''), flops=flops, bytes=float(a_bytes + w_bytes + out_bytes + res_bytes),
                m=m, n=n, k=k, z=z, f8=bool(d.f8 & 1))


E4M3_MAX = 448.0


def _e4m3_bytes(x, shift):
    import torch
    return (x * 2.0 ** shift).clamp(-E4M3_MAX, E4M3_MAX).to(torch.float8_e4m3fn).view(torch.uint8)


def f8_weight_shift(*weights):
    import math
    wmax = max(float(w.detach().abs().max()) for w in weights if w is not None)
    b1 = int(math.floor(math.log2(E4M3_MAX / wmax))) if wmax > 0 else 0
    return S.DS_F8_SH_LO8 + b1


def pack_conv_weight_f8(weight, skip_weight=None, bn=None):
    import torch
    cout, cin, kh, kw = weight.shape
    Sh = f8_weight_shift(weight, skip_weight)
    b, b1, b2 = Sh - S.DS_F8_SH_A16, Sh - S.DS_F8_SH_LO8, Sh - S.DS_F8_SH_HI8
    BN, n_tiles = (bn, -(-cout // bn)) if bn else pick_bn(cout)
    cout_pad = BN * n_tiles

    def kmajor(t, pad):
        cp = -(-cin // pad) * pad
        w = torch.zeros(cout, kh, kw, cp, dtype=torch.float32)
        w[..., :cin] = t.permute(0, 2, 3, 1)
        w = w.reshape(cout, kh * kw * cp)
        return w

    def with_skip(main, skip, pad):
        w = kmajor(main, pad)
        if skip is not None:
            c2 = skip.shape[1]
            c2p = -(-c2 // pad) * pad
            sk = torch.zeros(cout, c2p, dtype=torch.float32)
            sk[:, :c2] = skip.reshape(cout, c2)
            w = torch.cat([w, sk], dim=1)
        out = torch.zeros(cout_pad, w.shape[1], dtype=torch.float32)
        out[:cout] = w
        return out

    wf = weight.detach().float()
    sf = skip_weight.detach().float() if skip_weight is not None else None
    hi16 = lambda t: (t * 2.0 ** b).clamp(-65504.0, 65504.0).half()
    w_hi = hi16(wf)
    s_hi = hi16(sf) if sf is not None else None
    w_hi_f = w_hi.float() / 2.0 ** b
    s_hi_f = s_hi.float() / 2.0 ** b if sf is not None else None
    plane16 = with_skip(w_hi.float(), s_hi.float() if sf is not None else None, 64).half()
    hi8 = _e4m3_bytes(with_skip(w_hi_f, s_hi_f, 128), b1)
    lo8 = _e4m3_bytes(with_skip(wf - w_hi_f, (sf - s_hi_f) if sf is not None else None, 128), b2)
    blob = torch.cat([plane16.contiguous().view(torch.uint8).reshape(-1), hi8.reshape(-1), lo8.reshape(-1)]).contiguous()
    return blob, Sh


def act_planes_f8(x):
    import torch
    hi = (x * 2.0 ** S.DS_F8_SH_A16).clamp(-65504.0, 65504.0).half()
    hf = hi.float() / 2.0 ** S.DS_F8_SH_A16
    lo8 = _e4m3_bytes(x - hf, S.DS_F8_SH_LO8)
    hi8 = _e4m3_bytes(hf, S.DS_F8_SH_HI8)
    return torch.cat([hi.contiguous().view(torch.uint8).reshape(-1), lo8.reshape(-1), hi8.reshape(-1)]).contiguous()


def decode_act_planes_f8(buf, shape):
    import torch
    n = 1
    for d in shape:
        n *= d
    hi = buf[:2 * n].view(torch.float16).float().reshape(shape) / 2.0 ** S.DS_F8_SH_A16
    lo8 = buf[2 * n:3 * n].view(torch.float8_e4m3fn).float().reshape(shape) / 2.0 ** S.DS_F8_SH_LO8
    hi8 = buf[3 * n:4 * n].view(torch.float8_e4m3fn).float().reshape(shape) / 2.0 ** S.DS_F8_SH_HI8
    return hi, lo8, hi8


def decode_conv_weight_f8(blob, shift, cout, cin, taps, c2=0, bn=None):
    import torch
    BN, n_tiles = (bn, -(-cout // bn)) if bn else pick_bn(cout)
    cout_pad = BN * n_tiles
# ... 21 lines not shown
```

diff-sampler_b200/net.py:

```python
import ctypes as C
from collections import OrderedDict

import torch

from . import _lib
from . import edm_nets
from . import plan as planner

PRECISIONS = {'fp16x3': 3, 'fp16': 1, 'fp16f8': 3}


def default_precision():
    import os
    p = os.environ.get('DSB_PRECISION', 'fp16x3')
    if p not in PRECISIONS:
        raise ValueError(f'DSB_PRECISION={p!r}: expected one of {sorted(PRECISIONS)}')
    return p


def default_cuda_graph():
    import os
    return os.environ.get('DSB_CUDA_GRAPH', '1') != '0'


class B200Net:
    def __init__(self, params, img_resolution, img_channels, label_dim=0, sigma_min=0.002, sigma_max=80.0, sigma_data=0.5,
                 precision=None, device='cuda', fuse_stats=True, flash_attn=True, f8_min_channels=None, cuda_graph=None, spec=None):
        self.device = torch.device(device)
        precision = precision or default_precision()
        if self.device.type != 'cuda':
            raise _lib.DsError('B200Net needs a CUDA device (no CPU fallback)')
        self.lib = _lib.load()
        self.img_resolution, self.img_channels, self.label_dim = img_resolution, img_channels, label_dim
        self.sigma_min, self.sigma_max, self.sigma_data = sigma_min, sigma_max, sigma_data
        self.precision = precision
        self.npass = PRECISIONS[precision]
        self.f8 = precision == 'fp16f8'
        if f8_min_channels is None:
            import os
            f8_min_channels = int(os.environ.get('DSB_F8_MIN_CHANNELS', '0'))
        self.f8_min_channels = int(f8_min_channels)
        self.fuse_stats = bool(fuse_stats)
        self.flash_attn = bool(flash_attn)
        self.cuda_graph = default_cuda_graph() if cuda_graph is None else bool(cuda_graph)
        self.spec = spec if spec is not None else edm_nets.spec_from_params(params, img_resolution, img_channels, label_dim)
        self.spec.sigma_data = sigma_data
        self.wb, self.winfo = planner.pack_weights(self.spec, params, f8=self.f8, f8_min_channels=self.f8_min_channels)
        blob = self.wb.bytes()
        self.native = _lib.NativePlans(blob, self.device)
        self.weight_bytes = len(blob)
        self.launches_last_forward = 0
        self.total_launches = 0

    @classmethod
    def from_config(cls, name, seed=0, dezero=False, **kw):
        params, cfg = edm_nets.init_params(name, seed=seed)
        if dezero:
            edm_nets.dezero_(params, cfg['kind'], seed=seed)
        return cls(params, cfg['img_resolution'], cfg['img_channels'], cfg.get('label_dim', 0), **kw)

    @classmethod
    def from_reference(cls, net, **kw):
        sd = OrderedDict((k, v) for k, v in net.state_dict().items() if 'resample_filter' not in k)
        return cls(sd, net.img_resolution, net.img_channels, net.label_dim, sigma_min=float(net.sigma_min),
                   sigma_max=float(net.sigma_max), sigma_data=float(getattr(net, 'sigma_data', 0.5)), **kw)

    @classmethod
    def from_pickle(cls, f, key='ema', **kw):
        from . import checkpoint
        params, meta = checkpoint.load_edm_pickle(f, key=key)
        kw.setdefault('sigma_min', 0.002)
        kw.setdefault('sigma_max', 80.0)
        kw.setdefault('sigma_data', meta['sigma_data'])
        net = cls(params, meta['img_resolution'], meta['img_channels'], meta['label_dim'], **kw)
        net.checkpoint_meta = meta
        return net

    @classmethod
    def from_cm(cls, net, setting=None, **kw):
        from . import cm_net
        if getattr(net, 'label_dim', 0):
            raise ValueError('label_dim: class-conditional CM nets are not lowered')
        spec, params = cm_net.convert(net.state_dict(), setting, prefix='model.')
        if int(net.img_resolution) != spec.img_resolution:
            raise ValueError(f'img_resolution={net.img_resolution} does not match the settings ({spec.img_resolution})')
        return cls(params, spec.img_resolution, spec.img_channels, 0, sigma_min=float(net.sigma_min), sigma_max=float(net.sigma_max),
                   sigma_data=float(net.sigma_data), spec=spec, **kw)

    @classmethod
    def from_cm_checkpoint(cls, f, setting=None, **kw):
        from . import cm_net
        sd = torch.load(f, map_location='cpu', weights_only=True)
        spec, params = cm_net.convert(sd, setting)
        for k, v in (('sigma_min', 0.002), ('sigma_max', 80.0), ('sigma_data', 0.5)):
            kw.setdefault(k, v)
        return cls(params, spec.img_resolution, spec.img_channels, 0, spec=spec, **kw)

    @property
    def _plans(self):
        return self.native.plans

    def _plan(self, B, nsig, nlab):
        img = B * self.img_channels * self.img_resolution ** 2 * 4
        return self.native.get((B, nsig, nlab),
                               lambda: planner.compile_plan(self.spec, self.wb, self.winfo, B, nsig, nlab, npass=self.npass,
                                                            fuse_stats=self.fuse_stats, flash_attn=self.flash_attn, f8=self.f8),
                               (lambda pl: (img, img, nsig * 4, nlab * self.label_dim * 4, B * 64 * 4, 0)) if self.cuda_graph else None)

    def __call__(self, x, sigma, class_labels=None, out=None, bottleneck=None, **_):
        if x.device.type != 'cuda':
            raise _lib.DsError('B200Net: input must live on the CUDA device (no CPU fallback)')
        x = x.to(torch.float32).contiguous()
        B = x.shape[0]
        sig = torch.as_tensor(sigma, dtype=torch.float32, device=x.device).reshape(-1)
        if not sig.is_contiguous():
            sig = sig.contiguous()
        if sig.numel() not in (1, B):
            raise ValueError(f'sigma must have 1 or {B} elements, got {sig.numel()}')
        nsig = sig.numel() if sig.numel() == B and B > 1 else 1
        lab = None
        nlab = 0
        if self.label_dim:
            if class_labels is None:
                lab = torch.zeros([1, self.label_dim], device=x.device)
            else:
                lab = class_labels.to(torch.float32).reshape(-1, self.label_dim).contiguous()
            nlab = lab.shape[0]
            if nlab not in (1, B):
                raise ValueError('class_labels batch mismatch')
        h, pl = self._plan(B, nsig, nlab)
        if out is None:
            out = torch.empty_like(x)
        stream = torch.cuda.current_stream(x.device).cuda_stream
        self.launches_last_forward = self.native.run(h, (x.data_ptr(), out.data_ptr(), sig.data_ptr(), lab.data_ptr() if lab is not None else None,
                                                         bottleneck.data_ptr() if bottleneck is not None else None, None), stream)
        self.total_launches += self.launches_last_forward
        return out

    def profile_forward(self, x, sigma, class_labels=None):
        B = x.shape[0]
        self(x, sigma, class_labels)
        sig = torch.as_tensor(sigma).reshape(-1)
        nsig = sig.numel() if sig.numel() == B and B > 1 else 1
        nlab = 0 if not self.label_dim else (1 if class_labels is None else class_labels.reshape(-1, self.label_dim).shape[0])
        h, pl = self._plan(B, nsig, nlab)
        _lib.check(self.lib.ds_unet_set_profiling(h, 1), 'ds_unet_set_profiling')
        self(x, sigma, class_labels)
        buf = (C.c_float * pl.n_ops)()
        n = self.lib.ds_unet_get_profile(h, buf, pl.n_ops)
        self.lib.ds_unet_set_profiling(h, 0)
        out = {}
        for i in range(n):
            t = self.lib.ds_unet_op_type(h, i)
            c, ms = out.get(t, (0, 0.0))
            out[t] = (c + 1, ms + buf[i])
        self.last_profile = ([float(buf[i]) for i in range(n)], pl)
        return out

    def round_sigma(self, sigma):
        return torch.as_tensor(sigma)

    def debug_read(self, B, nsig, nlab, name, numel, dtype=torch.float32):
        self._plan(B, nsig, nlab)
        return self.native.debug_read((B, nsig, nlab), name, numel, dtype)

    def eval(self):
        return self

    def to(self, *_a, **_k):
        return self

    def requires_grad_(self, *_a, **_k):
        return self
```

diff-sampler_b200/plan.py:

```python
import math

import torch

from . import _cstructs as S
from . import gemm_desc as G

ALIGN = 1024
F4, H2 = 4, 2
NPL = 2


def _groups(c):
    return min(32, c // 4)


def _align(n, a=ALIGN):
    return (n + a - 1) // a * a


def io(slot):
    return S.ref(S.SPACE_IO, slot)


class WeightBlob:
    def __init__(self):
        self.chunks = []
        self.off = {}
        self.size = 0

    def add(self, name, t):
        t = t.detach().contiguous().cpu()
        raw = t.numpy().tobytes() if t.dtype != torch.float16 else t.view(torch.int16).numpy().tobytes()
        o = _align(self.size)
        if o > self.size:
            self.chunks.append(b'\0' * (o - self.size))
        self.chunks.append(raw)
        self.size = o + len(raw)
        self.off[name] = o
        return o

    def add_gemm(self, key, w, skip_w=None, bias=None, f8=False):
        if w.dim() == 2:
            w = w.reshape(w.shape[0], w.shape[1], 1, 1)
        packed, shift = G.pack_conv_weight_f8(w, skip_w) if f8 else (G.pack_conv_weight(w, skip_w), None)
        self.add(key + ':w', packed)
        if bias is not None:
            self.add(key + ':b', bias)
        return packed, shift

    def add_norm(self, key, P, src=None):
        src = src or key
        self.add(key + ':g', P(src + '.weight'))
        self.add(key + ':b', P(src + '.bias'))

    def ref(self, name, extra=0):
        return S.ref(S.SPACE_WEIGHTS, self.off[name] + extra)

    def bytes(self):
        return b''.join(self.chunks)


def _resolve(R, x):
    if x is None:
        return 0
    if isinstance(x, str):
        return R(x)
    if isinstance(x, tuple):
        return R(*x)
    return x


class Plan:
    def __init__(self, ops_array, n_ops, arena_bytes, arena_offsets, meta):
        self.ops_array = ops_array
        self.n_ops = n_ops
        self.arena_bytes = arena_bytes
        self.arena_offsets = arena_offsets
        self.meta = meta


class PlanBuilder:

    def __init__(self, wb, B, npass=3, tag=0):
        self.wb, self.B, self.npass, self.tag = wb, B, npass, tag
        self.sizes = {}
        self.ops = []
        self._slots = self._n_slots = 0

    def need(self, name, nbytes):
        self.sizes[name] = max(self.sizes.get(name, 0), int(nbytes))
        return name

    def emit(self, build):
        self.ops.append((len(self.ops) if self.tag is None else self.tag, build))

    def finish(self, **meta):
        offsets, total = {}, 0
        for name, nbytes in self.sizes.items():
            offsets[name] = total
            total += _align(nbytes)

        def R(name, extra=0):
            return S.ref(S.SPACE_ARENA, offsets[name] + int(extra))
        arr = (S.PlanOp * len(self.ops))()
        for op, (tag, build) in zip(arr, self.ops):
            desc = build(R)
            op.type = S.OP_TYPE_OF[type(desc)]
            op.tag = tag
            setattr(op.u, S.ALL_UNION_FIELD[op.type], desc)
        meta.update(n_ops=len(self.ops), n_gemm=sum(1 for op in arr if op.type == S.DS_OP_GEMM))
        return Plan(arr, len(self.ops), total, offsets, meta)

    def stats(self, n_slots):
        nbytes = n_slots * self.B * 32 * 2 * 8
        self.need('stats', nbytes)
        self.emit(lambda R: S.MemsetDesc(ptr=R('stats'), bytes=nbytes))
        self._n_slots = n_slots

    def stats_slot(self):
        assert self._slots < self._n_slots
        self._slots += 1
        return (self._slots - 1) * self.B * 32 * 2 * 8

    def gn_stats(self, slot, parts, hw, groups=32):
        (n0, c0), (n1, c1) = parts[0], (parts[1] if len(parts) > 1 else (None, 0))
        self.emit(lambda R: S.GnStatsDesc(src0=R(n0), src1=_resolve(R, n1), C0=c0, C1=c1, HW=hw, B=self.B, groups=groups,
                                          sums=R('stats', slot)))

    def gn_apply(self, parts, H, norm, eps, out, *, W=None, B=None, groups=32, slot=None, coef=False, silu=1, ada=None, ada_stride=0,
                 resample=0, raw=None, raw_f32=None, fmt=0, phase_pitch=0):
        (n0, c0), (n1, c1) = parts[0], (parts[1] if len(parts) > 1 else (None, 0))
        assert norm is None or (c0 + c1) % groups == 0
        Wt = self.wb.ref
        self.emit(lambda R: S.GnApplyDesc(
            src0=_resolve(R, n0), src1=_resolve(R, n1), C0=c0, C1=c1, H=H, W=W or H, B=B or self.B, groups=groups,
            sums=R('stats', slot) if slot is not None and not coef else 0, coef=R('gncoef') if coef else 0,
            gamma=Wt(norm + ':g') if norm else 0, beta=Wt(norm + ':b') if norm else 0, eps=eps, silu=silu,
            ada=_resolve(R, ada), ada_stride=ada_stride, resample=resample, nplanes=NPL, out_act=_resolve(R, out),
            out_raw=_resolve(R, raw), out_raw_f32=_resolve(R, raw_f32), fmt=fmt, pad0=phase_pitch))

    def group_norm(self, parts, H, norm, eps, out, **apply_kw):
        slot = self.stats_slot()
        self.gn_stats(slot, parts, H * H)
        self.gn_apply(parts, H, norm, eps, out, slot=slot, **apply_kw)

    def to_planes(self, src, C, H, W, B, dst, fmt=0, resample=0, groups=32, phase_pitch=0):
        self.gn_apply([(src, C)], H, None, 0.0, None, W=W, B=B, groups=groups, silu=0, resample=resample, raw=dst, fmt=fmt,
                      phase_pitch=phase_pitch)

    def vt_gemm(self, w, src, C, N, L, pitch, bias=None):
        W = self.wb.ref
        K = -(-C // 64) * 64
        self.emit(lambda R: G.rows_gemm(W(w), N, C, 1, R(src), L, C, self.B, K, num_z=self.B, nh=1, m_valid=N, n_valid=L,
                                        npass=self.npass, b_z_per_zb=1, out_h16=R('vt'), o_zb=N * pitch, ldo=pitch,
                                        o_plane=self.B * N * pitch, bias_m=W(bias) if bias else 0)[0])

    def attention(self, fused, q, k, out, nh, L, Lk, d, scale, vt_pitch, causal=0, s_pitch=None, pairs=False):
        B, C = self.B, nh * d
        qp, kc0 = (2 * C, C) if q == k else (C, 0)
        if fused:
            self.emit(lambda R: S.AttnDesc(q=R(q), k=R(k), vt=R('vt'), out=R(out), B=B, nh=nh, L=L, Lk=Lk, q_pitch=qp, q_c0=0,
                                           k_pitch=qp, k_c0=kc0, vt_pitch=vt_pitch, o_pitch=C, nplanes=NPL, scale=scale, causal=causal,
                                           pad0=32 if pairs else 0))
            return
        sp = s_pitch or Lk
        self.need('S', B * nh * L * sp * F4)
        self.need('P', NPL * B * nh * L * vt_pitch * H2)
        self.emit(lambda R: G.rows_gemm(R(q), L, qp, B, R(k), Lk, qp, B, d, num_z=B * nh, nh=nh, m_valid=L, n_valid=Lk, npass=self.npass,
                                        a_c_per_zh=d, a_n_per_zb=1, b_k0=kc0, b_k_per_zh=d, b_z_per_zb=1, out_f32=R('S'),
                                        o_zb=nh * L * sp, o_zh=L * sp, ldo=sp, scale=scale)[0])
        self.emit(lambda R: S.SoftmaxDesc(S=R('S'), P=R('P'), rows=B * nh * L, L=Lk, nplanes=NPL, pitch_in=s_pitch or 0,
                                          pitch_out=0 if vt_pitch == Lk else vt_pitch))
        self.emit(lambda R: G.rows_gemm(R('P'), L, vt_pitch, B * nh, R('vt'), C, vt_pitch, B, vt_pitch, num_z=B * nh, nh=nh, m_valid=L,
                                        n_valid=d, npass=self.npass, a_n_per_zb=nh, a_n_per_zh=1, b_row_per_zh=d, b_z_per_zb=1,
                                        out_h16=R(out), o_zb=L * C, o_zh=d, ldo=C, o_plane=B * L * C, a_k_valid=Lk, b_k_valid=Lk)[0])


def _qkv_split(w, b, heads):
    c3 = w.shape[0]
    cc = c3 // 3
    d = cc // heads
    idx = torch.arange(c3).reshape(heads, d, 3)
    qi, ki, vi = idx[:, :, 0].reshape(-1), idx[:, :, 1].reshape(-1), idx[:, :, 2].reshape(-1)
    w2 = w.reshape(c3, -1)
    return torch.cat([w2[qi], w2[ki]]), torch.cat([b[qi], b[ki]]), w2[vi], b[vi]


def pack_weights(spec, params, f8=False, f8_min_channels=0):
    pf = spec.prefix
    P = lambda k: params[pf + k].detach().float().cpu()
    has = lambda k: (pf + k) in params
    wb = WeightBlob()
    info = {}

    def add_conv(key, w, skip_w=None, bias=None, as_f8=False):
        packed, shift = wb.add_gemm(key, w, skip_w, bias, f8=as_f8)
        info[key] = dict(cout=w.shape[0], f8_shift=shift) if as_f8 else dict(cout=w.shape[0], cout_pad=packed.shape[1], ktot=packed.shape[2])

    add_conv(spec.stem, P(spec.stem + '.weight'), bias=P(spec.stem + '.bias'))
    aff_w, aff_b = [], []
    for b in spec.enc + spec.dec:
        n = b.name
        wb.add_norm(n + '.norm0', P)
        blk_f8 = f8 and min(b.cin, b.cout) >= f8_min_channels
        add_conv(n + '.conv0', P(n + '.conv0.weight'), bias=P(n + '.conv0.bias'), as_f8=blk_f8)
        wb.add_norm(n + '.norm1', P)
        bias1 = P(n + '.conv1.bias')
        skip_w = None
        if b.skip == 'conv':
            skip_w = P(n + '.skip.weight')
            bias1 = bias1 + P(n + '.skip.bias')
        add_conv(n + '.conv1', P(n + '.conv1.weight'), skip_w, bias=bias1, as_f8=blk_f8)
        aff_w.append(P(n + '.affine.weight'))
        aff_b.append(P(n + '.affine.bias'))
        if b.heads:
            wb.add_norm(n + '.norm2', P)
            wqk, bqk, wv, bv = _qkv_split(P(n + '.qkv.weight'), P(n + '.qkv.bias'), b.heads)
            add_conv(n + '.qk', wqk.reshape(wqk.shape[0], wqk.shape[1], 1, 1), bias=bqk)
            wb.add(n + '.v:w', G.split_planes(wv))
            wb.add(n + '.v:b', bv)
            add_conv(n + '.proj', P(n + '.proj.weight'), bias=P(n + '.proj.bias'))
    wb.add('affine:w', torch.cat(aff_w, dim=0))
    wb.add('affine:w16', G.split_planes(torch.cat(aff_w, dim=0)))
    wb.add('affine:b', torch.cat(aff_b, dim=0))
    for k in ('map_layer0', 'map_layer1'):
        wb.add(k + ':w', P(k + '.weight'))
        wb.add(k + ':b', P(k + '.bias'))
    if spec.label_dim:
        wb.add('map_label:w', P('map_label.weight'))
        if has('map_label.bias'):
            wb.add('map_label:b', P('map_label.bias'))
    wb.add_norm(spec.head_norm, P)
    add_conv(spec.head_conv, P(spec.head_conv + '.weight'), bias=P(spec.head_conv + '.bias'),
             as_f8=f8 and P(spec.head_conv + '.weight').shape[1] >= f8_min_channels)
    return wb, info


def compile_plan(spec, wb, winfo, B, nsig, nlab, npass=3, fuse_stats=True, flash_attn=True, f8=False):
    assert nsig in (1, B) and nlab in (0, 1, B)
    assert not f8 or npass == 3

    def is_f8(key):
        return f8 and 'f8_shift' in winfo[key]

    def f8_args(key):
        return dict(f8=True, acc_scale=2.0 ** -winfo[key]['f8_shift']) if is_f8(key) else {}
    pb = PlanBuilder(wb, B, npass)
    emit, W = pb.emit, wb.ref
    nE = max(nsig, nlab, 1)
    R0 = spec.img_resolution

    prod_of = {}
    quads_of = {}
    unit_of = {}

    def emit_producer(name, cout, m_rows, build):
        pid = len(pb.ops)
        prod_of[name] = (pid, cout, m_rows)

        def materialise(R):
            d = build(R)
            if pid in quads_of:
                d.st_quads = R(quads_of[pid])
                d.st_unit = unit_of[pid]
            return d
        emit(materialise)

    def need_stats(slot, parts, hw, norm=None, eps=0.0, ada=None, ada_stride=0):
        assert len(parts) <= 2
        c_total = sum(c for _, c in parts)
        g = _groups(c_total)
        cpg = c_total // g
        (n0, c0), (n1, c1) = parts[0], (parts[1] if len(parts) > 1 else (None, 0))
        rem = c0 % cpg if n1 else 0
        pieces = [cpg] + ([rem, cpg - rem] if rem else [])
        unit = 4 if all(p % 4 == 0 for p in pieces) else (2 if all(p % 2 == 0 for p in pieces) else 0)
        fusable = (fuse_stats and hw % 32 == 0 and unit and all(c % unit == 0 for _, c in parts)
                   and all(name in prod_of and prod_of[name][1] == c for name, c in parts))
        want_coef = norm is not None and c_total <= 2048
        if want_coef:
            pb.need('gncoef', B * c_total * 2 * F4)

        def coef_args(R):
            if not want_coef:
                return {}
            return dict(gamma=W(norm + ':g'), beta=W(norm + ':b'), ada=_resolve(R, ada), ada_stride=ada_stride, eps=eps, HW=hw,
                        coef=R('gncoef'))
        if not fusable:
            pb.gn_stats(slot, parts, hw, groups=g)
            if want_coef:
                emit(lambda R: S.GnFinalizeDesc(quads0=0, quads1=0, C0=c0, C1=c1, slabs_per_sample=0, B=B, groups=g, sums=R('stats', slot),
                                                **coef_args(R)))
            return want_coef
        bufs, pids = [], []
        for name, c in parts:
            pid, cout, m_rows = prod_of[name]
            unit_of[pid] = min(unit_of.get(pid, 4), unit)
            quads_of[pid] = pb.need('quads:' + name, (m_rows // 32) * (cout // unit_of[pid]) * 2 * F4)
            bufs.append(quads_of[pid])
            pids.append(pid)
        emit(lambda R: S.GnFinalizeDesc(quads0=R(bufs[0]), quads1=R(bufs[1]) if len(bufs) > 1 else 0, C0=c0, C1=c1,
                                        slabs_per_sample=hw // 32, B=B, groups=g, sums=R('stats', slot), unit0=unit_of[pids[0]],
                                        unit1=unit_of[pids[1]] if len(pids) > 1 else 4, **coef_args(R)))
        return want_coef

    def group_norm(parts, H, norm, eps, silu, fmt=0, ada=None):
        slot = pb.stats_slot()
        ada_stride = aff_stride if ada else 0
        coef = need_stats(slot, parts, H * H, norm, eps, ada, ada_stride)
        pb.gn_apply(parts, H, norm, eps, 'act', groups=_groups(sum(c for _, c in parts)), slot=slot, coef=coef, silu=silu, ada=ada,
                    ada_stride=ada_stride, fmt=fmt)

    pb.need('coef', nsig * 4 * F4)
    pb.need('emb0', nsig * spec.noise_channels * F4)
    pb.need('e1', nE * spec.emb_channels * F4)
    pb.need('e2', nE * spec.emb_channels * F4)
    pb.need('e3', nE * spec.emb_channels * F4)
    pb.need('aff', nE * spec.aff_total * F4)
    pb.stats(2 * len(spec.enc + spec.dec) + sum(1 for b in spec.enc + spec.dec if b.heads) + 1)
    emit(lambda R: S.PosembDesc(sigma=io(S.DS_IO_SIGMA), nsig=nsig, num_channels=spec.noise_channels,
                                endpoint=1 if spec.kind == 'song' else 0, swap_sincos=1 if spec.kind == 'song' else 0,
                                sigma_data=spec.sigma_data, coef=R('coef'), emb=R('emb0'),
                                noise_scale=0.0 if spec.noise_scale == 1 else spec.noise_scale))
    nc, ec = spec.noise_channels, spec.emb_channels
    if spec.kind == 'song':
        src, src_rows = 'emb0', nsig
        if spec.label_dim and nlab:
            pb.need('emb0b', nE * nc * F4)
            emit(lambda R: S.LinearDesc(in_=io(S.DS_IO_LABELS), in_stride=spec.label_dim if nlab > 1 else 0, W=W('map_label:w'),
                                        b=W('map_label:b'), add=R('emb0'), add_stride=nc if nsig > 1 else 0, out=R('emb0b'),
                                        n_rows=nE, in_f=spec.label_dim, out_f=nc, act=0, in_scale=math.sqrt(spec.label_dim)))
            src, src_rows = 'emb0b', nE
        emit(lambda R: S.LinearDesc(in_=R(src), in_stride=nc if src_rows > 1 else 0, W=W('map_layer0:w'), b=W('map_layer0:b'),
                                    out=R('e1'), n_rows=src_rows, in_f=nc, out_f=ec, act=1, in_scale=1.0))
        emit(lambda R: S.LinearDesc(in_=R('e1'), in_stride=ec if src_rows > 1 else 0, W=W('map_layer1:w'), b=W('map_layer1:b'),
                                    out=R('e2'), n_rows=src_rows, in_f=ec, out_f=ec, act=1, in_scale=1.0))
        emb_buf, emb_rows = 'e2', src_rows
    else:
        with_label = bool(spec.label_dim and nlab)
        emit(lambda R: S.LinearDesc(in_=R('emb0'), in_stride=nc if nsig > 1 else 0, W=W('map_layer0:w'), b=W('map_layer0:b'),
                                    out=R('e1'), n_rows=nsig, in_f=nc, out_f=ec, act=1, in_scale=1.0))
        emit(lambda R: S.LinearDesc(in_=R('e1'), in_stride=ec if nsig > 1 else 0, W=W('map_layer1:w'), b=W('map_layer1:b'),
                                    out=R('e2'), n_rows=nsig, in_f=ec, out_f=ec, act=0 if with_label else 1, in_scale=1.0))
        emb_buf, emb_rows = 'e2', nsig
        if with_label:
            emit(lambda R: S.LinearDesc(in_=io(S.DS_IO_LABELS), in_stride=spec.label_dim if nlab > 1 else 0, W=W('map_label:w'), b=0,
                                        add=R('e2'), add_stride=ec if nsig > 1 else 0, out=R('e3'), n_rows=nE, in_f=spec.label_dim,
                                        out_f=ec, act=1, in_scale=1.0))
            emb_buf, emb_rows = 'e3', nE
    if emb_rows >= 32 and ec % 64 == 0:
        pb.need('emb_planes', NPL * emb_rows * ec * H2)
        pb.to_planes(emb_buf, ec, emb_rows, 1, 1, 'emb_planes', groups=1)
        emit(lambda R: G.rows_gemm(R('emb_planes'), emb_rows, ec, 1, W('affine:w16'), spec.aff_total, ec, 1, ec, num_z=1, nh=1,
                                   m_valid=emb_rows, n_valid=spec.aff_total, npass=npass, out_f32=R('aff'), ldo=spec.aff_total,
                                   bias_n=W('affine:b'))[0])
    else:
        emit(lambda R: S.LinearDesc(in_=R(emb_buf), in_stride=ec if emb_rows > 1 else 0, W=W('affine:w'), b=W('affine:b'), out=R('aff'),
                                    n_rows=emb_rows, in_f=ec, out_f=spec.aff_total, act=0, in_scale=1.0))
    aff_stride = spec.aff_total if emb_rows > 1 else 0

    HW0 = R0 * R0
    pb.need('in_planes', NPL * B * HW0 * 64 * H2)
    emit(lambda R: S.PrepInputDesc(x=io(S.DS_IO_X), coef=R('coef'), coef_stride=4 if nsig > 1 else 0, B=B, C=spec.img_channels,
                                   HW=HW0, nplanes=NPL, out=R('in_planes')))
    pb.need('x:' + spec.stem, B * HW0 * spec.stem_cout * F4)
    emit_producer('x:' + spec.stem, spec.stem_cout, B * HW0, lambda R: G.conv_gemm(R('in_planes'), B, R0, R0, 64, W(spec.stem + ':w'), spec.stem_cout, taps=9,
                                                          npass=npass, out_f32=R('x:' + spec.stem), bias=W(spec.stem + ':b'))[0])

    def lower_block(b, x0, c0, x1, c1):
        pb.tag += 1
        n = b.name
        Hi, Ho = b.res_in, b.res_out
        cin, cout = b.cin, b.cout
        assert c0 + c1 == cin
        resample = 1 if b.down else (2 if b.up else 0)
        Mo = B * Ho * Ho
        parts = [(x0, c0)] + ([(x1, c1)] if x1 else [])
        s0 = pb.stats_slot()
        k0 = need_stats(s0, parts, Hi * Hi, n + '.norm0' if resample == 0 else None, b.eps)
        pb.need('act', NPL * Mo * max(cin, cout) * H2)
        want_raw = b.skip == 'conv'
        want_rawf = b.skip == 'resample'
        if want_raw:
            pb.need('raw', NPL * Mo * cin * H2)
        if want_rawf:
            pb.need('rawf', Mo * cin * F4)
        pb.gn_apply(parts, Hi, n + '.norm0', b.eps, 'act', groups=_groups(cin), slot=s0, coef=k0, resample=resample,
                    raw='raw' if want_raw else None, raw_f32='rawf' if want_rawf else None, fmt=1 if is_f8(n + '.conv0') else 0)
        pb.need('y', Mo * cout * F4)
        emit_producer('y', cout, Mo, lambda R: G.conv_gemm(R('act'), B, Ho, Ho, cin, W(n + '.conv0:w'), cout, taps=9, npass=npass, out_f32=R('y'),
                                                 bias=W(n + '.conv0:b'), rowvec=0 if b.adaptive_scale else R('aff', b.aff_off * F4),
                                                 rowvec_stride=aff_stride, **f8_args(n + '.conv0'))[0])
        group_norm([('y', cout)], Ho, n + '.norm1', b.eps, 1, fmt=1 if is_f8(n + '.conv1') else 0,
                   ada=('aff', b.aff_off * F4) if b.adaptive_scale else None)
        xout = pb.need('x:' + n, Mo * cout * F4)
        mid = pb.need('xmid', Mo * cout * F4) if b.heads else xout
        if b.skip == 'identity':
            assert x1 is None
            res_name = x0
        elif b.skip == 'resample':
            res_name = 'rawf'
        else:
            res_name = None
        emit_producer(mid, cout, Mo, lambda R: G.conv_gemm(R('act'), B, Ho, Ho, cout, W(n + '.conv1:w'), cout, taps=9, npass=npass,
                                                 a2_ptr=R('raw') if want_raw else 0, C2=cin if want_raw else 0, out_f32=R(mid),
                                                 bias=W(n + '.conv1:b'), residual=R(res_name) if res_name else 0, ldr=cout,
                                                 scale=b.skip_scale, **f8_args(n + '.conv1'))[0])
        if b.heads:
            nh = b.heads
            d = cout // nh
            L = Ho * Ho
            group_norm([(mid, cout)], Ho, n + '.norm2', b.eps, 0)
            pb.need('qk', NPL * B * L * 2 * cout * H2)
            pb.need('vt', NPL * B * cout * L * H2)
            pb.need('o', NPL * B * L * cout * H2)
            emit(lambda R: G.conv_gemm(R('act'), B, Ho, Ho, cout, W(n + '.qk:w'), 2 * cout, taps=1, npass=npass, out_h16=R('qk'),
                                       bias=W(n + '.qk:b'))[0])
            pb.vt_gemm(n + '.v:w', 'act', cout, cout, L, L, bias=n + '.v:b')
            pb.attention(flash_attn and d == 64 and L % 8 == 0, 'qk', 'qk', 'o', nh, L, L, d, 1.0 / math.sqrt(d), L)
            emit_producer(xout, cout, Mo, lambda R: G.conv_gemm(R('o'), B, Ho, Ho, cout, W(n + '.proj:w'), cout, taps=1, npass=npass, out_f32=R(xout),
                                                      bias=W(n + '.proj:b'), residual=R(mid), ldr=cout, scale=b.skip_scale)[0])
        if n == spec.bottleneck_block:
            emit(lambda R: S.ChanmeanDesc(src=R(xout), out=io(S.DS_IO_BOTTLENECK), rows=B * Ho * Ho, C=cout))
        return xout

    skips = [('x:' + spec.stem, spec.stem_cout)]
    cur, cur_c = 'x:' + spec.stem, spec.stem_cout
    for b in spec.enc:
        cur = lower_block(b, cur, cur_c, None, 0)
        cur_c = b.cout
        skips.append((cur, cur_c))
    for b in spec.dec:
        if b.concat:
            sk, sc = skips.pop()
            assert sc == b.concat
            cur = lower_block(b, cur, cur_c, sk, sc)
        else:
            cur = lower_block(b, cur, cur_c, None, 0)
        cur_c = b.cout
    pb.tag += 1
    pb.need('act', NPL * B * HW0 * cur_c * H2)
    fin_c = cur_c
    group_norm([(cur, fin_c)], R0, spec.head_norm, spec.head_eps, 1, fmt=1 if is_f8(spec.head_conv) else 0)
    emit(lambda R: G.conv_gemm(R('act'), B, R0, R0, fin_c, W(spec.head_conv + ':w'), spec.img_channels, taps=9, npass=npass,
                               bias=W(spec.head_conv + ':b'),
                               edm=(io(S.DS_IO_X), R('coef'), 4 if nsig > 1 else 0, spec.img_channels, io(S.DS_IO_D)),
                               **f8_args(spec.head_conv))[0])
    return pb.finish(B=B, nsig=nsig, nlab=nlab, npass=npass, f8=bool(f8))
```

include/diffsampler_b200.h:

```cpp
#ifndef DIFFSAMPLER_B200_H
#define DIFFSAMPLER_B200_H

#include <stddef.h>
#include <stdint.h>

#ifdef __cplusplus
extern "C" {
#endif

const char* ds_version(void);
const char* ds_last_error(void);

typedef struct ds_weights ds_weights;
typedef struct ds_unet ds_unet;

int ds_weights_create(const void* host_blob, size_t bytes, ds_weights** out);
void ds_weights_destroy(ds_weights* w);

int ds_unet_create(const ds_weights* w, const void* plan_ops, int n_ops, size_t op_size, size_t arena_bytes, ds_unet** out);
void ds_unet_destroy(ds_unet* u);

int ds_unet_forward(ds_unet* u, const float* x, const float* sigma, const float* labels, float* out_D,
                    float* out_bottleneck, void* stream);

int ds_unet_forward_io(ds_unet* u, const void* const* io, int n_io, void* stream);

int ds_unet_enable_graph(ds_unet* u, const size_t* io_bytes, int n_io);

int ds_unet_debug_read(ds_unet* u, size_t arena_offset, void* host_dst, size_t bytes, void* stream);
int ds_unet_last_launch_count(const ds_unet* u);

int ds_unet_set_profiling(ds_unet* u, int enable);
int ds_unet_get_profile(ds_unet* u, float* ms_per_op, int n);
int ds_unet_op_type(const ds_unet* u, int i);

int ds_solver_update(float* out_x, float* out_m, const float* xb, const float* xs, const float* D,
                     const float* const* hist, int nhist, const float* thr, int mode, float t, const float* t_dev,
                     const float* coef6, const float* coef_dev, int64_t n_per_sample, int B, void* stream);

int ds_solver_update_u8(float* out_x, float* out_m, unsigned char* out_u8, int C, int HW, const float* xb, const float* xs, const float* D,
                        const float* const* hist, int nhist, const float* thr, int mode, float t, const float* t_dev,
                        const float* coef6, const float* coef_dev, int64_t n_per_sample, int B, void* stream);

int ds_dyn_threshold(const float* x0, float* thr, int B, int row_len, float q, float floor_val, void* stream);

int ds_gits_cost(const float* traj, const float* eps, const float* t_steps, double* out, int N, int B, int64_t n_per_sample, void* stream);

int ds_amed_predict(const float* weights, const int* dims6, const float* bottleneck, const float* t_cur, const float* t_next,
                    float scale_dir, float scale_time, float* out4, int B, void* stream);

int ds_images_to_uint8(const float* images, unsigned char* out, int B, int C, int HW, void* stream);

int ds_op_launch(int op_type, const void* desc, size_t desc_size, void* stream);
int ds_op_check(int op_type, const void* desc, size_t desc_size);
size_t ds_sizeof(int which);
int ds_gemm_config(const void* desc, int* info);

#ifdef __cplusplus
}
#endif
#endif
```

Baseline: 296.4 images/s.

## Split batch into two concurrent lanes with GEMM SM reserve and priorities

Lowers the U-Net plan as two half-batch op lists that run on two captured streams, so one lane's memory-bound normalization and elementwise ops overlap with the other lane's GEMMs. During capture GEMMs are limited to fewer SMs via an SM reserve, non-GEMM kernel nodes get high graph-node priority, and gn_apply drops its persistent grid sizing when running beside a lane. IO refs now carry byte offsets so each lane addresses its half of the inputs. The costs are smaller per-lane GEMMs with lower tile efficiency, extra event dependencies, and a plan builder whose lane setup is only partly visible.

```diff
diff --git a/diff-sampler_b200/_cstructs.py b/diff-sampler_b200/_cstructs.py
--- a/diff-sampler_b200/_cstructs.py
+++ b/diff-sampler_b200/_cstructs.py
@@ -16,6 +16,7 @@
 DS_KNN_MAX, DS_KNN_CAND = 64, 256
 
 SPACE_ABS, SPACE_ARENA, SPACE_WEIGHTS, SPACE_IO = 0, 1, 2, 3
+IO_SLOT_BITS = 8
 
 
 def ref(space, offset):
diff --git a/diff-sampler_b200/_lib.py b/diff-sampler_b200/_lib.py
--- a/diff-sampler_b200/_lib.py
+++ b/diff-sampler_b200/_lib.py
@@ -12,7 +12,7 @@
     'ds_version', 'ds_last_error', 'ds_weights_create', 'ds_weights_destroy', 'ds_unet_create', 'ds_unet_destroy',
     'ds_unet_forward', 'ds_unet_debug_read', 'ds_unet_last_launch_count', 'ds_solver_update', 'ds_dyn_threshold',
     'ds_op_launch', 'ds_sizeof', 'ds_unet_set_profiling', 'ds_unet_get_profile', 'ds_unet_op_type', 'ds_gits_cost', 'ds_unet_forward_io', 'ds_images_to_uint8', 'ds_solver_update_u8', 'ds_unet_enable_graph', 'ds_amed_predict',
-    'ds_gemm_config', 'ds_op_check',
+    'ds_gemm_config', 'ds_op_check', 'ds_unet_set_lanes',
 ]
 
 _lib = None
@@ -42,6 +42,7 @@
     lib.ds_unet_forward.argtypes = [vp, vp, vp, vp, vp, vp, vp]
     lib.ds_unet_forward_io.argtypes = [vp, C.POINTER(vp), C.c_int, vp]
     lib.ds_unet_enable_graph.argtypes = [vp, C.POINTER(sz), C.c_int]
+    lib.ds_unet_set_lanes.argtypes = [vp, C.c_int, C.c_int]
     lib.ds_unet_debug_read.argtypes = [vp, sz, vp, sz, vp]
     lib.ds_unet_last_launch_count.argtypes = [vp]
     lib.ds_unet_set_profiling.argtypes = [vp, C.c_int]
@@ -114,6 +115,8 @@
             with torch.cuda.device(self.device):
                 check(self.lib.ds_unet_create(self._wh, C.cast(pl.ops_array, C.c_void_p), pl.n_ops, C.sizeof(S.PlanOp), pl.arena_bytes,
                                               C.byref(h)), 'ds_unet_create')
+                if pl.meta.get('lanes', 1) > 1:
+                    check(self.lib.ds_unet_set_lanes(h, pl.meta['lanes'], pl.meta['gemm_sm_reserve']), 'ds_unet_set_lanes')
                 if io_bytes is not None:
                     check(self.lib.ds_unet_enable_graph(h, (C.c_size_t * S.DS_IO_COUNT)(*io_bytes(pl)), S.DS_IO_COUNT),
                           'ds_unet_enable_graph')
diff --git a/diff-sampler_b200/csrc/elementwise.cu b/diff-sampler_b200/csrc/elementwise.cu
--- a/diff-sampler_b200/csrc/elementwise.cu
+++ b/diff-sampler_b200/csrc/elementwise.cu
@@ -1,3 +1,4 @@
+#include <climits>
 #include "ops.h"
 #include "operand.cuh"
 #include <cuda_fp16.h>
@@ -791,7 +792,7 @@
     return {0, nullptr};
 }
 
-extern "C" int ds_gn_apply_launch(const ds_gn_apply_desc* d, cudaStream_t stream) {
+int dsb::gn_apply_run(const ds_gn_apply_desc* d, cudaStream_t stream, bool persistent) {
     if (const int rc = gn_apply_check(*d).rc) return rc;
     const int C = d->C0 + d->C1;
     const int nc8 = C / 8;
@@ -820,7 +821,7 @@
         }
         const int ups = (npix + rows - 1) / rows;
         const long long total_units = (long long)ups * d->B;
-        long long g3 = (long long)sms[dev] * occ[dev][slot];
+        long long g3 = persistent ? (long long)sms[dev] * occ[dev][slot] : LLONG_MAX;
         const long long total_chunks = (long long)((ups + 7) / 8) * d->B;
         if (g3 > total_chunks) g3 = total_chunks;
         if (g3 < 1) g3 = 1;
@@ -834,6 +835,8 @@
     else gn_apply_v2_kernel<<<grid, threads, 0, stream>>>(*d, pix_per_cta, nc8, rows);
     return ok();
 }
+
+extern "C" int ds_gn_apply_launch(const ds_gn_apply_desc* d, cudaStream_t stream) { return dsb::gn_apply_run(d, stream, true); }
 
 OpCheck dsb::embed_check(const ds_embed_desc& d) {
     if (d.C % 4 || d.rows <= 0 || d.T <= 0 || d.vocab <= 0) return {-2, "embed: shape"};
diff --git a/diff-sampler_b200/csrc/engine.cu b/diff-sampler_b200/csrc/engine.cu
--- a/diff-sampler_b200/csrc/engine.cu
+++ b/diff-sampler_b200/csrc/engine.cu
@@ -15,6 +15,8 @@
 int gemm_run(const GemmKernelParams* kp, cudaStream_t stream);
 size_t gemm_params_size();
 void gemm_patch_edm(GemmKernelParams* kp, const float* x, float* D);
+void gemm_set_sm_reserve(GemmKernelParams* kp, int sms);
+bool is_gemm_kernel(const void* func);
 struct AttnKernelParams;
 int attn_build(const ds_attn_desc* d, AttnKernelParams* kp);
 int attn_run(const AttnKernelParams* kp, cudaStream_t stream);
@@ -41,6 +43,7 @@
     int op;
     size_t field_off;
     int slot;
+    size_t byte_off;
 };
 
 struct ds_unet {
@@ -61,6 +64,10 @@
     int gnodes[2] = {0, 0};
     int warm_runs = 0;
     cudaStream_t cap_stream = nullptr;
+    int lanes = 1;
+    int gemm_sm_reserve = 0;
+    cudaStream_t lane_stream = nullptr;
+    cudaEvent_t lane_ev[3] = {nullptr, nullptr, nullptr};
 };
 
 template <class F>
@@ -120,13 +127,13 @@
     }
 }
 
-static int launch_op(const ds_plan_op& op, const unsigned char* gemm_kp, cudaStream_t s) {
+static int launch_op(const ds_plan_op& op, const unsigned char* gemm_kp, cudaStream_t s, bool beside_lane = false) {
     switch (op.type) {
         case DS_OP_GEMM:
             if (gemm_kp) return dsb::gemm_run(reinterpret_cast<const dsb::GemmKernelParams*>(gemm_kp), s);
             return ds_gemm_launch(&op.u.gemm, s);
         case DS_OP_GN_STATS: return ds_gn_stats_launch(&op.u.gn_stats, s);
-        case DS_OP_GN_APPLY: return ds_gn_apply_launch(&op.u.gn_apply, s);
+        case DS_OP_GN_APPLY: return dsb::gn_apply_run(&op.u.gn_apply, s, !beside_lane);
         case DS_OP_SOFTMAX: return ds_softmax_launch(&op.u.softmax, s);
         case DS_OP_POSEMB: return ds_posemb_launch(&op.u.posemb, s);
         case DS_OP_LINEAR: return ds_linear_launch(&op.u.linear, s);
@@ -221,7 +228,8 @@
                 IoFix fx;
                 fx.op = i;
                 fx.field_off = reinterpret_cast<char*>(field) - reinterpret_cast<char*>(&op);
-                fx.slot = (int)off;
+                fx.slot = (int)(off & 0xff);
+                fx.byte_off = (size_t)(off >> 8);
                 u->fixes.push_back(fx);
                 *field = nullptr;
             } else {
@@ -262,6 +270,8 @@
     for (int v = 0; v < 2; ++v) if (u->gexec[v]) cudaGraphExecDestroy(u->gexec[v]);
     for (int k = 0; k < DS_IO_COUNT; ++k) if (u->stage[k]) cudaFree(u->stage[k]);
     if (u->cap_stream) cudaStreamDestroy(u->cap_stream);
+    if (u->lane_stream) cudaStreamDestroy(u->lane_stream);
+    for (auto e : u->lane_ev) if (e) cudaEventDestroy(e);
     cudaFree(u->arena);
     delete u;
 }
@@ -274,44 +284,86 @@
     return ds_unet_forward_io(u, io, DS_IO_COUNT, stream);
 }
 
-static int run_ops(ds_unet* u, const void* const* io, cudaStream_t s, bool profiling) {
+static unsigned char* op_params(ds_unet* u, size_t i) {
+    unsigned char* p = u->gemm_params[i].data();
+    return reinterpret_cast<unsigned char*>((reinterpret_cast<uintptr_t>(p) + 63) & ~uintptr_t(63));
+}
+
+static int run_op(ds_unet* u, size_t i, cudaStream_t s, bool profiling, bool beside_lane = false) {
+    ds_plan_op& op = u->ops[i];
+    const unsigned char* kp = nullptr;
+    if (op.type == DS_OP_GEMM || op.type == DS_OP_ATTN) {
+        unsigned char* al = op_params(u, i);
+        if (op.type == DS_OP_GEMM && op.u.gemm.edm_out)
+            dsb::gemm_patch_edm(reinterpret_cast<dsb::GemmKernelParams*>(al), op.u.gemm.edm_x, op.u.gemm.edm_D);
+        kp = al;
+    }
+    if (op.type == DS_OP_CHANMEAN && op.u.chanmean.out == nullptr) return 0;
+    if (profiling) { cudaEventRecord(u->ev0[i], s); u->ev_used[i] = 1; }
+    int rc = launch_op(op, kp, s, beside_lane);
+    if (profiling) cudaEventRecord(u->ev1[i], s);
+    if (rc) {
+        char buf[160];
+        snprintf(buf, sizeof buf, "ds_unet_forward: op %zu (type %d tag %d) failed rc=%d cuda=%s", i, op.type, op.tag, rc,
+                 cudaGetErrorString(cudaGetLastError()));
+        return fail(-8, buf);
+    }
+    return 1;
+}
+
+static int run_ops(ds_unet* u, const void* const* io, cudaStream_t s, bool profiling, cudaStream_t s2 = nullptr) {
     for (const IoFix& fx : u->fixes) {
         if (fx.slot < 0 || fx.slot >= DS_IO_COUNT) return fail(-7, "ds_unet_forward: bad io slot");
         void** field = reinterpret_cast<void**>(reinterpret_cast<char*>(&u->ops[fx.op]) + fx.field_off);
-        *field = const_cast<void*>(io[fx.slot]);
+        *field = io[fx.slot] ? static_cast<char*>(const_cast<void*>(io[fx.slot])) + fx.byte_off : nullptr;
     }
     int launches = 0;
-    for (size_t i = 0; i < u->ops.size(); ++i) {
-        ds_plan_op& op = u->ops[i];
-        const unsigned char* kp = nullptr;
-        if (op.type == DS_OP_GEMM || op.type == DS_OP_ATTN) {
-            unsigned char* p = u->gemm_params[i].data();
-            unsigned char* al = reinterpret_cast<unsigned char*>((reinterpret_cast<uintptr_t>(p) + 63) & ~uintptr_t(63));
-            if (op.type == DS_OP_GEMM && op.u.gemm.edm_out)
-                dsb::gemm_patch_edm(reinterpret_cast<dsb::GemmKernelParams*>(al), op.u.gemm.edm_x, op.u.gemm.edm_D);
-            kp = al;
-        }
-        if (op.type == DS_OP_CHANMEAN && op.u.chanmean.out == nullptr) continue;
-        if (profiling) { cudaEventRecord(u->ev0[i], s); u->ev_used[i] = 1; }
-        int rc = launch_op(op, kp, s);
-        if (profiling) cudaEventRecord(u->ev1[i], s);
-        if (rc) {
-            char buf[160];
-            snprintf(buf, sizeof buf, "ds_unet_forward: op %zu (type %d tag %d) failed rc=%d cuda=%s", i, op.type, op.tag, rc,
-                     cudaGetErrorString(cudaGetLastError()));
-            return fail(-8, buf);
-        }
-        ++launches;
-    }
+    if (!s2) {
+        for (size_t i = 0; i < u->ops.size(); ++i) {
+            const int rc = run_op(u, i, s, profiling);
+            if (rc < 0) return rc;
+            launches += rc;
+        }
+        return launches;
+    }
+    const size_t n = u->ops.size() / 2;
+    cudaEvent_t* ev = u->lane_ev;
+    if (cudaEventRecord(ev[0], s) != cudaSuccess || cudaStreamWaitEvent(s2, ev[0], 0) != cudaSuccess)
+        return fail(-27, "ds_unet_forward: cannot fork the second lane");
+    for (size_t i = 0; i < n; ++i) {
+        const int r0 = run_op(u, i, s, false, true);
+        if (r0 < 0) return r0;
+        if (cudaEventRecord(ev[1], s) != cudaSuccess || cudaStreamWaitEvent(s2, ev[1], 0) != cudaSuccess)
+            return fail(-27, "ds_unet_forward: cannot order the lanes");
+        const int r1 = run_op(u, n + i, s2, false, true);
+        if (r1 < 0) return r1;
+        launches += r0 + r1;
+    }
+    if (cudaEventRecord(ev[2], s2) != cudaSuccess || cudaStreamWaitEvent(s, ev[2], 0) != cudaSuccess)
+        return fail(-27, "ds_unet_forward: cannot join the second lane");
     return launches;
+}
+
+static void set_gemm_sm_reserve(ds_unet* u, int sms) {
+    for (size_t i = 0; i < u->ops.size(); ++i)
+        if (u->ops[i].type == DS_OP_GEMM) dsb::gemm_set_sm_reserve(reinterpret_cast<dsb::GemmKernelParams*>(op_params(u, i)), sms);
 }
 
 static int build_graph(ds_unet* u, int variant, const void* const* staged_io) {
     if (!u->cap_stream && cudaStreamCreateWithFlags(&u->cap_stream, cudaStreamNonBlocking) != cudaSuccess)
         return fail(-20, "ds_unet_forward: cannot create the capture stream");
+    const bool two = u->lanes == 2;
+    if (two && !u->lane_stream) {
+        if (cudaStreamCreateWithFlags(&u->lane_stream, cudaStreamNonBlocking) != cudaSuccess)
+            return fail(-20, "ds_unet_forward: cannot create the lane stream");
+        for (auto& e : u->lane_ev)
+            if (cudaEventCreateWithFlags(&e, cudaEventDisableTiming) != cudaSuccess) return fail(-20, "ds_unet_forward: cannot create the lane events");
+    }
     if (cudaStreamBeginCapture(u->cap_stream, cudaStreamCaptureModeThreadLocal) != cudaSuccess)
         return fail(-21, std::string("ds_unet_forward: cudaStreamBeginCapture failed: ") + cudaGetErrorString(cudaGetLastError()));
-    const int n = run_ops(u, staged_io, u->cap_stream, false);
+    if (two) set_gemm_sm_reserve(u, u->gemm_sm_reserve);
+    const int n = run_ops(u, staged_io, u->cap_stream, false, two ? u->lane_stream : nullptr);
+    if (two) set_gemm_sm_reserve(u, 0);
     cudaGraph_t g = nullptr;
     const cudaError_t e = cudaStreamEndCapture(u->cap_stream, &g);
     if (n < 0 || e != cudaSuccess || !g) {
@@ -319,8 +371,27 @@
         if (n < 0) return n;
         return fail(-22, std::string("ds_unet_forward: stream capture failed: ") + cudaGetErrorString(e));
     }
+    if (two) {
+        int least = 0, greatest = 0;
+        cudaDeviceGetStreamPriorityRange(&least, &greatest);
+        size_t nn = 0;
+        cudaGraphGetNodes(g, nullptr, &nn);
+        std::vector<cudaGraphNode_t> nodes(nn);
+        cudaGraphGetNodes(g, nodes.data(), &nn);
+        for (cudaGraphNode_t node : nodes) {
+            cudaGraphNodeType t;
+            cudaKernelNodeParams kn;
+            if (cudaGraphNodeGetType(node, &t) != cudaSuccess || t != cudaGraphNodeTypeKernel) continue;
+            if (cudaGraphKernelNodeGetParams(node, &kn) != cudaSuccess || dsb::is_gemm_kernel(kn.func)) continue;
+            cudaLaunchAttributeValue v;
+            memset(&v, 0, sizeof v);
+            v.priority = greatest;
+            cudaGraphKernelNodeSetAttribute(node, cudaLaunchAttributePriority, &v);
+        }
+        cudaGetLastError();
+    }
     cudaGraphExec_t ex = nullptr;
-    const cudaError_t ei = cudaGraphInstantiate(&ex, g, 0);
+    const cudaError_t ei = cudaGraphInstantiate(&ex, g, two ? cudaGraphInstantiateFlagUseNodePriority : 0);
     cudaGraphDestroy(g);
     if (ei != cudaSuccess) return fail(-23, std::string("ds_unet_forward: cudaGraphInstantiate failed: ") + cudaGetErrorString(ei));
     u->gexec[variant] = ex;
@@ -384,6 +455,21 @@
         u->stage_bytes[k] = io_bytes[k];
     }
     u->graph_on = true;
+    return 0;
+}
+
+int ds_unet_set_lanes(ds_unet* u, int lanes, int gemm_sm_reserve) {
+    if (!u) return fail(-1, "ds_unet_set_lanes: null handle");
+    if (lanes != 1 && lanes != 2) return fail(-1, "ds_unet_set_lanes: lanes must be 1 or 2");
+    if (gemm_sm_reserve < 0) return fail(-1, "ds_unet_set_lanes: negative SM reserve");
+    if (u->gexec[0] || u->gexec[1]) return fail(-1, "ds_unet_set_lanes: the graph is already captured");
+    const size_t n = u->ops.size() / lanes;
+    if (n * lanes != u->ops.size()) return fail(-1, "ds_unet_set_lanes: op count is not a multiple of the lane count");
+    for (size_t i = 0; i < n; ++i)
+        for (int l = 1; l < lanes; ++l)
+            if (u->ops[l * n + i].type != u->ops[i].type) return fail(-1, "ds_unet_set_lanes: the lanes' op lists differ");
+    u->lanes = lanes;
+    u->gemm_sm_reserve = gemm_sm_reserve;
     return 0;
 }
 
diff --git a/diff-sampler_b200/csrc/gemm_tc.cu b/diff-sampler_b200/csrc/gemm_tc.cu
--- a/diff-sampler_b200/csrc/gemm_tc.cu
+++ b/diff-sampler_b200/csrc/gemm_tc.cu
@@ -48,6 +48,7 @@
     int st_unit;
     int tap_dh[9], tap_dw[9], tap_cb[9];
     int f8_last_steps;
+    int sm_reserve;
 };
 
 struct SmemCtl {
@@ -624,6 +625,18 @@
 
 size_t gemm_params_size() { return sizeof(GemmKernelParams); }
 void gemm_patch_edm(GemmKernelParams* kp, const float* x, float* D) { kp->edm_x = x; kp->edm_D = D; }
+void gemm_set_sm_reserve(GemmKernelParams* kp, int sms) { kp->sm_reserve = sms; }
+
+bool is_gemm_kernel(const void* func) {
+    static const void* const k[] = {
+        (const void*)gemm_tc_kernel<16>, (const void*)gemm_tc_kernel<32>, (const void*)gemm_tc_kernel<48>, (const void*)gemm_tc_kernel<64>,
+        (const void*)gemm_tc_kernel<80>, (const void*)gemm_tc_kernel<96>, (const void*)gemm_tc_kernel<112>, (const void*)gemm_tc_kernel<128>,
+        (const void*)gemm_tc_kernel<144>, (const void*)gemm_tc_kernel<160>, (const void*)gemm_tc_kernel<176>, (const void*)gemm_tc_kernel<192>,
+        (const void*)gemm_tc_kernel<208>, (const void*)gemm_tc_kernel<224>, (const void*)gemm_tc_kernel<240>, (const void*)gemm_tc_kernel<256>};
+    for (const void* f : k)
+        if (f == func) return true;
+    return false;
+}
 
 static int g_num_sms[64] = {};
 static bool g_attr_set[64][17] = {};
@@ -636,7 +649,8 @@
     }
     const size_t smem = (size_t)kp->num_stages * (kATileBytes + BN * 128) + kStgBytes + sizeof(SmemCtl) + 1024;
     const int tiles = kp->num_z * kp->m_tiles * kp->n_tiles;
-    const int grid = tiles < g_num_sms[slot] ? tiles : g_num_sms[slot];
+    const int sms = g_num_sms[slot] - kp->sm_reserve > 0 ? g_num_sms[slot] - kp->sm_reserve : 1;
+    const int grid = tiles < sms ? tiles : sms;
     if (grid <= 0) return 0;
     gemm_tc_kernel<BN><<<grid, kThreads, smem, stream>>>(*kp);
     return cudaGetLastError() == cudaSuccess ? 0 : -21;
diff --git a/diff-sampler_b200/csrc/ops.h b/diff-sampler_b200/csrc/ops.h
--- a/diff-sampler_b200/csrc/ops.h
+++ b/diff-sampler_b200/csrc/ops.h
@@ -386,6 +386,7 @@
 OpCheck gn_stats_check(const ds_gn_stats_desc& d);
 OpCheck gn_finalize_check(const ds_gn_finalize_desc& d);
 OpCheck gn_apply_check(const ds_gn_apply_desc& d);
+int gn_apply_run(const ds_gn_apply_desc* d, cudaStream_t stream, bool persistent);
 OpCheck embed_check(const ds_embed_desc& d);
 OpCheck layernorm_check(const ds_layernorm_desc& d);
 OpCheck geglu_check(const ds_geglu_desc& d);
diff --git a/diff-sampler_b200/gemm_desc.py b/diff-sampler_b200/gemm_desc.py
--- a/diff-sampler_b200/gemm_desc.py
+++ b/diff-sampler_b200/gemm_desc.py
@@ -61,7 +61,7 @@
 
 def conv_gemm(a_ptr, Bn, H, W, C, w_ptr, Cout, *, taps=9, npass=3, a_planes=2, w_planes=2, a2_ptr=0, C2=0,
               out_f32=0, out_h16=0, o_planes=2, ldo=None, bias=0, rowvec=0, rowvec_stride=0, residual=0, ldr=None, scale=1.0,
-              edm=None, nchw_out=None, bn=None, s2d=False, f8=False, acc_scale=1.0):
+              edm=None, nchw_out=None, bn=None, s2d=False, f8=False, acc_scale=1.0, lanes=1):
     assert C % 8 == 0 and C2 % 8 == 0
     cpad, c2pad = -(-C // 64) * 64, -(-C2 // 64) * 64
     if f8:
@@ -71,7 +71,7 @@
         assert a_planes == 2 and w_planes == 2
     d = S.GemmDesc()
     bw, bh, bnn = conv_box(H, W)
-    BN, n_tiles = (bn, -(-Cout // bn)) if bn else fill_bn(Cout, -(-(Bn * H * W) // 128))
+    BN, n_tiles = (bn, -(-Cout // bn)) if bn else fill_bn(Cout, -(-(lanes * Bn * H * W) // 128))
     cout_pad = padded_rows(Cout)
     ktot = taps * cpad + c2pad
     d.a_ptr = a_ptr
@@ -134,10 +134,11 @@
 def rows_gemm(a_ptr, a_rows, a_pitch, a_batches, b_ptr, b_rows, b_pitch, b_batches, K, *, num_z, nh=1, m_valid, n_valid,
               npass=3, a_planes=2, b_planes=2, a_c_per_zh=0, a_n_per_zb=0, a_n_per_zh=0, b_k0=0, b_k_per_zh=0, b_row_per_zh=0,
               b_z_per_zb=0, b_z_per_zh=0, out_f32=0, out_h16=0, o_zb=0, o_zh=0, ldo=0, o_plane=0, bias_n=0, bias_m=0,
-              residual=0, ldr=0, scale=1.0, bn=None, a_k_valid=None, b_k_valid=None):
+              residual=0, ldr=0, scale=1.0, bn=None, a_k_valid=None, b_k_valid=None, lanes=1):
     assert K % 64 == 0
     d = S.GemmDesc()
-    BN, n_tiles = (bn, -(-n_valid // bn)) if bn else fill_bn(n_valid, -(-m_valid // 128), num_z)
+    BN, n_tiles = (bn, -(-n_valid // bn)) if bn else fill_bn(n_valid, -(-(m_valid * (lanes if num_z == 1 else 1)) // 128),
+                                                                    num_z * (lanes if num_z > 1 else 1))
     d.a_ptr = a_ptr
     d.a_dims[:] = [a_k_valid or a_pitch, a_rows, 1, a_planes * a_batches]
     d.a_strides[:] = [a_pitch * H16, a_rows * a_pitch * H16, a_rows * a_pitch * H16]
diff --git a/diff-sampler_b200/net.py b/diff-sampler_b200/net.py
--- a/diff-sampler_b200/net.py
+++ b/diff-sampler_b200/net.py
@@ -104,7 +104,8 @@
         img = B * self.img_channels * self.img_resolution ** 2 * 4
         return self.native.get((B, nsig, nlab),
                                lambda: planner.compile_plan(self.spec, self.wb, self.winfo, B, nsig, nlab, npass=self.npass,
-                                                            fuse_stats=self.fuse_stats, flash_attn=self.flash_attn, f8=self.f8),
+                                                            fuse_stats=self.fuse_stats, flash_attn=self.flash_attn, f8=self.f8,
+                                                            lanes=planner.lane_count(self.spec, B)),
                                (lambda pl: (img, img, nsig * 4, nlab * self.label_dim * 4, B * 64 * 4, 0)) if self.cuda_graph else None)
 
     def __call__(self, x, sigma, class_labels=None, out=None, bottleneck=None, **_):
diff --git a/diff-sampler_b200/plan.py b/diff-sampler_b200/plan.py
--- a/diff-sampler_b200/plan.py
+++ b/diff-sampler_b200/plan.py
@@ -18,8 +18,8 @@
     return (n + a - 1) // a * a
 
 
-def io(slot):
-    return S.ref(S.SPACE_IO, slot)
+def io(slot, byte_offset=0):
+    return S.ref(S.SPACE_IO, slot | int(byte_offset) << S.IO_SLOT_BITS)
 
 
 class WeightBlob:
@@ -81,8 +81,8 @@
 
 class PlanBuilder:
 
-    def __init__(self, wb, B, npass=3, tag=0):
-        self.wb, self.B, self.npass, self.tag = wb, B, npass, tag
+    def __init__(self, wb, B, npass=3, tag=0, lanes=1):
+        self.wb, self.B, self.npass, self.tag, self.lanes = wb, B, npass, tag, lanes
         self.sizes = {}
         self.ops = []
         self._slots = self._n_slots = 0
@@ -95,21 +95,7 @@
         self.ops.append((len(self.ops) if self.tag is None else self.tag, build))
 
     def finish(self, **meta):
-        offsets, total = {}, 0
-        for name, nbytes in self.sizes.items():
-            offsets[name] = total
-            total += _align(nbytes)
-
-        def R(name, extra=0):
-            return S.ref(S.SPACE_ARENA, offsets[name] + int(extra))
-        arr = (S.PlanOp * len(self.ops))()
-        for op, (tag, build) in zip(arr, self.ops):
-            desc = build(R)
-            op.type = S.OP_TYPE_OF[type(desc)]
-            op.tag = tag
-            setattr(op.u, S.ALL_UNION_FIELD[op.type], desc)
-        meta.update(n_ops=len(self.ops), n_gemm=sum(1 for op in arr if op.type == S.DS_OP_GEMM))
-        return Plan(arr, len(self.ops), total, offsets, meta)
+        return finish_lanes([self], **meta)
 
     def stats(self, n_slots):
         nbytes = n_slots * self.B * 32 * 2 * 8
@@ -153,7 +139,7 @@
         K = -(-C // 64) * 64
         self.emit(lambda R: G.rows_gemm(W(w), N, C, 1, R(src), L, C, self.B, K, num_z=self.B, nh=1, m_valid=N, n_valid=L,
                                         npass=self.npass, b_z_per_zb=1, out_h16=R('vt'), o_zb=N * pitch, ldo=pitch,
-                                        o_plane=self.B * N * pitch, bias_m=W(bias) if bias else 0)[0])
+                                        o_plane=self.B * N * pitch, bias_m=W(bias) if bias else 0, lanes=self.lanes)[0])
 
     def attention(self, fused, q, k, out, nh, L, Lk, d, scale, vt_pitch, causal=0, s_pitch=None, pairs=False):
         B, C = self.B, nh * d
@@ -168,12 +154,35 @@
         self.need('P', NPL * B * nh * L * vt_pitch * H2)
         self.emit(lambda R: G.rows_gemm(R(q), L, qp, B, R(k), Lk, qp, B, d, num_z=B * nh, nh=nh, m_valid=L, n_valid=Lk, npass=self.npass,
                                         a_c_per_zh=d, a_n_per_zb=1, b_k0=kc0, b_k_per_zh=d, b_z_per_zb=1, out_f32=R('S'),
-                                        o_zb=nh * L * sp, o_zh=L * sp, ldo=sp, scale=scale)[0])
+                                        o_zb=nh * L * sp, o_zh=L * sp, ldo=sp, scale=scale, lanes=self.lanes)[0])
         self.emit(lambda R: S.SoftmaxDesc(S=R('S'), P=R('P'), rows=B * nh * L, L=Lk, nplanes=NPL, pitch_in=s_pitch or 0,
                                           pitch_out=0 if vt_pitch == Lk else vt_pitch))
         self.emit(lambda R: G.rows_gemm(R('P'), L, vt_pitch, B * nh, R('vt'), C, vt_pitch, B, vt_pitch, num_z=B * nh, nh=nh, m_valid=L,
                                         n_valid=d, npass=self.npass, a_n_per_zb=nh, a_n_per_zh=1, b_row_per_zh=d, b_z_per_zb=1,
-                                        out_h16=R(out), o_zb=L * C, o_zh=d, ldo=C, o_plane=B * L * C, a_k_valid=Lk, b_k_valid=Lk)[0])
+                                        out_h16=R(out), o_zb=L * C, o_zh=d, ldo=C, o_plane=B * L * C, a_k_valid=Lk, b_k_valid=Lk,
+                                        lanes=self.lanes)[0])
+
+
+def finish_lanes(builders, **meta):
+    offsets, total, ops = {}, 0, []
+    for lane, pb in enumerate(builders):
+        own = {}
+        for name, nbytes in pb.sizes.items():
+            own[name] = total
+            total += _align(nbytes)
+
+        def R(name, extra=0, own=own):
+            return S.ref(S.SPACE_ARENA, own[name] + int(extra))
+        ops += [(tag, build, R) for tag, build in pb.ops]
+        offsets.update({(f'lane{lane}:' if lane else '') + name: off for name, off in own.items()})
+    arr = (S.PlanOp * len(ops))()
+    for op, (tag, build, R) in zip(arr, ops):
+        desc = build(R)
+        op.type = S.OP_TYPE_OF[type(desc)]
+        op.tag = tag
+        setattr(op.u, S.ALL_UNION_FIELD[op.type], desc)
+    meta.update(n_ops=len(ops), n_gemm=sum(1 for op in arr if op.type == S.DS_OP_GEMM))
+    return Plan(arr, len(ops), total, offsets, meta)
 
 
 def _qkv_split(w, b, heads):
@@ -236,19 +245,44 @@
     return wb, info
 
 
-def compile_plan(spec, wb, winfo, B, nsig, nlab, npass=3, fuse_stats=True, flash_attn=True, f8=False):
+LANE_MIN_BATCH = 256
+LANE_GEMM_SM_RESERVE = 16
+
+
+def lane_count(spec, B):
+    return 2 if spec.kind in ('song', 'adm') and B >= LANE_MIN_BATCH and B % 4 == 0 else 1
+
+
+def compile_plan(spec, wb, winfo, B, nsig, nlab, npass=3, fuse_stats=True, flash_attn=True, f8=False, lanes=1):
     assert nsig in (1, B) and nlab in (0, 1, B)
     assert not f8 or npass == 3
+    if lanes == 1:
+        return _lower(spec, wb, winfo, B, nsig, nlab, npass, fuse_stats, flash_attn, f8).finish(B=B, nsig=nsig, nlab=nlab, npass=npass,
+                                                                                              f8=bool(f8))
+    assert B % lanes == 0
+    Bl = B // lanes
+    pbs = [_lower(spec, wb, winfo, Bl, Bl if nsig == B else 1, Bl if nlab == B else nlab, npass, fuse_stats, flash_attn, f8, lanes, l * Bl)
+           for l in range(lanes)]
+    assert len({len(pb.ops) for pb in pbs}) == 1
+    return finish_lanes(pbs, B=B, nsig=nsig, nlab=nlab, npass=npass, f8=bool(f8), lanes=lanes, gemm_sm_reserve=LANE_GEMM_SM_RESERVE)
+
+
+def _lower(spec, wb, winfo, B, nsig, nlab, npass, fuse_stats, flash_attn, f8, lanes=1, b0=0):
+    def io_at(slot, per_sample):
+        return io(slot, b0 * per_sample)
 
     def is_f8(key):
         return f8 and 'f8_shift' in winfo[key]
 
     def f8_args(key):
         return dict(f8=True, acc_scale=2.0 ** -winfo[key]['f8_shift']) if is_f8(key) else {}
-    pb = PlanBuilder(wb, B, npass)
+    pb = PlanBuilder(wb, B, npass, lanes=lanes)
     emit, W = pb.emit, wb.ref
+    conv_gemm = lambda *a, **k: G.conv_gemm(*a, lanes=lanes, **k)
+    rows_gemm = lambda *a, **k: G.rows_gemm(*a, lanes=lanes, **k)
     nE = max(nsig, nlab, 1)
     R0 = spec.img_resolution
+    img_bytes = spec.img_channels * R0 * R0 * F4
 
     prod_of = {}
     quads_of = {}
@@ -318,18 +352,20 @@
     pb.need('e3', nE * spec.emb_channels * F4)
     pb.need('aff', nE * spec.aff_total * F4)
     pb.stats(2 * len(spec.enc + spec.dec) + sum(1 for b in spec.enc + spec.dec if b.heads) + 1)
-    emit(lambda R: S.PosembDesc(sigma=io(S.DS_IO_SIGMA), nsig=nsig, num_channels=spec.noise_channels,
+    emit(lambda R: S.PosembDesc(sigma=io_at(S.DS_IO_SIGMA, 4 if nsig > 1 else 0), nsig=nsig, num_channels=spec.noise_channels,
                                 endpoint=1 if spec.kind == 'song' else 0, swap_sincos=1 if spec.kind == 'song' else 0,
                                 sigma_data=spec.sigma_data, coef=R('coef'), emb=R('emb0'),
                                 noise_scale=0.0 if spec.noise_scale == 1 else spec.noise_scale))
     nc, ec = spec.noise_channels, spec.emb_channels
+    lab_stride = spec.label_dim if nlab > 1 else 0
+    labels = io_at(S.DS_IO_LABELS, lab_stride * F4)
     if spec.kind == 'song':
         src, src_rows = 'emb0', nsig
         if spec.label_dim and nlab:
             pb.need('emb0b', nE * nc * F4)
-            emit(lambda R: S.LinearDesc(in_=io(S.DS_IO_LABELS), in_stride=spec.label_dim if nlab > 1 else 0, W=W('map_label:w'),
-                                        b=W('map_label:b'), add=R('emb0'), add_stride=nc if nsig > 1 else 0, out=R('emb0b'),
-                                        n_rows=nE, in_f=spec.label_dim, out_f=nc, act=0, in_scale=math.sqrt(spec.label_dim)))
+            emit(lambda R: S.LinearDesc(in_=labels, in_stride=lab_stride, W=W('map_label:w'), b=W('map_label:b'), add=R('emb0'),
+                                        add_stride=nc if nsig > 1 else 0, out=R('emb0b'), n_rows=nE, in_f=spec.label_dim, out_f=nc, act=0,
+                                        in_scale=math.sqrt(spec.label_dim)))
             src, src_rows = 'emb0b', nE
         emit(lambda R: S.LinearDesc(in_=R(src), in_stride=nc if src_rows > 1 else 0, W=W('map_layer0:w'), b=W('map_layer0:b'),
                                     out=R('e1'), n_rows=src_rows, in_f=nc, out_f=ec, act=1, in_scale=1.0))
@@ -344,14 +380,14 @@
                                     out=R('e2'), n_rows=nsig, in_f=ec, out_f=ec, act=0 if with_label else 1, in_scale=1.0))
         emb_buf, emb_rows = 'e2', nsig
         if with_label:
-            emit(lambda R: S.LinearDesc(in_=io(S.DS_IO_LABELS), in_stride=spec.label_dim if nlab > 1 else 0, W=W('map_label:w'), b=0,
+            emit(lambda R: S.LinearDesc(in_=labels, in_stride=lab_stride, W=W('map_label:w'), b=0,
                                         add=R('e2'), add_stride=ec if nsig > 1 else 0, out=R('e3'), n_rows=nE, in_f=spec.label_dim,
                                         out_f=ec, act=1, in_scale=1.0))
             emb_buf, emb_rows = 'e3', nE
     if emb_rows >= 32 and ec % 64 == 0:
         pb.need('emb_planes', NPL * emb_rows * ec * H2)
         pb.to_planes(emb_buf, ec, emb_rows, 1, 1, 'emb_planes', groups=1)
-        emit(lambda R: G.rows_gemm(R('emb_planes'), emb_rows, ec, 1, W('affine:w16'), spec.aff_total, ec, 1, ec, num_z=1, nh=1,
+        emit(lambda R: rows_gemm(R('emb_planes'), emb_rows, ec, 1, W('affine:w16'), spec.aff_total, ec, 1, ec, num_z=1, nh=1,
                                    m_valid=emb_rows, n_valid=spec.aff_total, npass=npass, out_f32=R('aff'), ldo=spec.aff_total,
                                    bias_n=W('affine:b'))[0])
     else:
@@ -361,10 +397,10 @@
 
     HW0 = R0 * R0
     pb.need('in_planes', NPL * B * HW0 * 64 * H2)
-    emit(lambda R: S.PrepInputDesc(x=io(S.DS_IO_X), coef=R('coef'), coef_stride=4 if nsig > 1 else 0, B=B, C=spec.img_channels,
+    emit(lambda R: S.PrepInputDesc(x=io_at(S.DS_IO_X, img_bytes), coef=R('coef'), coef_stride=4 if nsig > 1 else 0, B=B, C=spec.img_channels,
                                    HW=HW0, nplanes=NPL, out=R('in_planes')))
     pb.need('x:' + spec.stem, B * HW0 * spec.stem_cout * F4)
-    emit_producer('x:' + spec.stem, spec.stem_cout, B * HW0, lambda R: G.conv_gemm(R('in_planes'), B, R0, R0, 64, W(spec.stem + ':w'), spec.stem_cout, taps=9,
+    emit_producer('x:' + spec.stem, spec.stem_cout, B * HW0, lambda R: conv_gemm(R('in_planes'), B, R0, R0, 64, W(spec.stem + ':w'), spec.stem_cout, taps=9,
                                                           npass=npass, out_f32=R('x:' + spec.stem), bias=W(spec.stem + ':b'))[0])
 
     def lower_block(b, x0, c0, x1, c1):
@@ -388,7 +424,7 @@
         pb.gn_apply(parts, Hi, n + '.norm0', b.eps, 'act', groups=_groups(cin), slot=s0, coef=k0, resample=resample,
                     raw='raw' if want_raw else None, raw_f32='rawf' if want_rawf else None, fmt=1 if is_f8(n + '.conv0') else 0)
         pb.need('y', Mo * cout * F4)
-        emit_producer('y', cout, Mo, lambda R: G.conv_gemm(R('act'), B, Ho, Ho, cin, W(n + '.conv0:w'), cout, taps=9, npass=npass, out_f32=R('y'),
+        emit_producer('y', cout, Mo, lambda R: conv_gemm(R('act'), B, Ho, Ho, cin, W(n + '.conv0:w'), cout, taps=9, npass=npass, out_f32=R('y'),
                                                  bias=W(n + '.conv0:b'), rowvec=0 if b.adaptive_scale else R('aff', b.aff_off * F4),
                                                  rowvec_stride=aff_stride, **f8_args(n + '.conv0'))[0])
         group_norm([('y', cout)], Ho, n + '.norm1', b.eps, 1, fmt=1 if is_f8(n + '.conv1') else 0,
@@ -402,7 +438,7 @@
             res_name = 'rawf'
         else:
             res_name = None
-        emit_producer(mid, cout, Mo, lambda R: G.conv_gemm(R('act'), B, Ho, Ho, cout, W(n + '.conv1:w'), cout, taps=9, npass=npass,
+        emit_producer(mid, cout, Mo, lambda R: conv_gemm(R('act'), B, Ho, Ho, cout, W(n + '.conv1:w'), cout, taps=9, npass=npass,
                                                  a2_ptr=R('raw') if want_raw else 0, C2=cin if want_raw else 0, out_f32=R(mid),
                                                  bias=W(n + '.conv1:b'), residual=R(res_name) if res_name else 0, ldr=cout,
                                                  scale=b.skip_scale, **f8_args(n + '.conv1'))[0])
@@ -414,14 +450,14 @@
             pb.need('qk', NPL * B * L * 2 * cout * H2)
             pb.need('vt', NPL * B * cout * L * H2)
             pb.need('o', NPL * B * L * cout * H2)
-            emit(lambda R: G.conv_gemm(R('act'), B, Ho, Ho, cout, W(n + '.qk:w'), 2 * cout, taps=1, npass=npass, out_h16=R('qk'),
+            emit(lambda R: conv_gemm(R('act'), B, Ho, Ho, cout, W(n + '.qk:w'), 2 * cout, taps=1, npass=npass, out_h16=R('qk'),
                                        bias=W(n + '.qk:b'))[0])
             pb.vt_gemm(n + '.v:w', 'act', cout, cout, L, L, bias=n + '.v:b')
             pb.attention(flash_attn and d == 64 and L % 8 == 0, 'qk', 'qk', 'o', nh, L, L, d, 1.0 / math.sqrt(d), L)
-            emit_producer(xout, cout, Mo, lambda R: G.conv_gemm(R('o'), B, Ho, Ho, cout, W(n + '.proj:w'), cout, taps=1, npass=npass, out_f32=R(xout),
+            emit_producer(xout, cout, Mo, lambda R: conv_gemm(R('o'), B, Ho, Ho, cout, W(n + '.proj:w'), cout, taps=1, npass=npass, out_f32=R(xout),
                                                       bias=W(n + '.proj:b'), residual=R(mid), ldr=cout, scale=b.skip_scale)[0])
         if n == spec.bottleneck_block:
-            emit(lambda R: S.ChanmeanDesc(src=R(xout), out=io(S.DS_IO_BOTTLENECK), rows=B * Ho * Ho, C=cout))
+            emit(lambda R: S.ChanmeanDesc(src=R(xout), out=io_at(S.DS_IO_BOTTLENECK, Ho * Ho * F4), rows=B * Ho * Ho, C=cout))
         return xout
 
     skips = [('x:' + spec.stem, spec.stem_cout)]
@@ -442,8 +478,8 @@
     pb.need('act', NPL * B * HW0 * cur_c * H2)
     fin_c = cur_c
     group_norm([(cur, fin_c)], R0, spec.head_norm, spec.head_eps, 1, fmt=1 if is_f8(spec.head_conv) else 0)
-    emit(lambda R: G.conv_gemm(R('act'), B, R0, R0, fin_c, W(spec.head_conv + ':w'), spec.img_channels, taps=9, npass=npass,
+    emit(lambda R: conv_gemm(R('act'), B, R0, R0, fin_c, W(spec.head_conv + ':w'), spec.img_channels, taps=9, npass=npass,
                                bias=W(spec.head_conv + ':b'),
-                               edm=(io(S.DS_IO_X), R('coef'), 4 if nsig > 1 else 0, spec.img_channels, io(S.DS_IO_D)),
+                               edm=(io_at(S.DS_IO_X, img_bytes), R('coef'), 4 if nsig > 1 else 0, spec.img_channels, io_at(S.DS_IO_D, img_bytes)),
                                **f8_args(spec.head_conv))[0])
-    return pb.finish(B=B, nsig=nsig, nlab=nlab, npass=npass, f8=bool(f8))
+    return pb
diff --git a/include/diffsampler_b200.h b/include/diffsampler_b200.h
--- a/include/diffsampler_b200.h
+++ b/include/diffsampler_b200.h
@@ -26,6 +26,8 @@
 int ds_unet_forward_io(ds_unet* u, const void* const* io, int n_io, void* stream);
 
 int ds_unet_enable_graph(ds_unet* u, const size_t* io_bytes, int n_io);
+
+int ds_unet_set_lanes(ds_unet* u, int lanes, int gemm_sm_reserve);
 
 int ds_unet_debug_read(ds_unet* u, size_t arena_offset, void* host_dst, size_t bytes, void* stream);
 int ds_unet_last_launch_count(const ds_unet* u);
```

Measured after the change: 305.4 images/s (median of 6 runs). +3.0%, better.
